# navallo/collision_avoidance

Measured on AMD Instinct MI355X. Metric: agent-steps/sec (whole node), 4096 arenas x 64 agents per GPU, higher is better.
Workload: dtype f32

## Files before the change

### collision_avoidance_amd/_lib.py

```python
import ctypes as C
import os

from . import build as _build

OBS_DIM = 64
MAX_NEIGHBORS, MAX_OBST_NEIGHBORS, MAX_AGENTS = 16, 16, 1024
DONE_XLESS, DONE_GOAL, DONE_REGOAL = 0, 1, 2
F_OBS, F_STATS, F_AUTORESET, F_NODONE, F_FREEZE = 1, 2, 4, 8, 16
SCN_CROWD, SCN_CIRCLE, SCN_DOORWAY, SCN_CONGESTED, SCN_INCOMING, SCN_BLOCKS, SCN_DEADLOCK, SCN_CROWD_SEPARATED = range(8)

(FLD_POS_X, FLD_POS_Y, FLD_VEL_X, FLD_VEL_Y, FLD_PREF_X, FLD_PREF_Y, FLD_GOAL_X, FLD_GOAL_Y,
 FLD_GOAL2_X, FLD_GOAL2_Y, FLD_REWARD, FLD_AGENT_DONE, FLD_ARRIVE_STEP, FLD_NB_COUNT, FLD_NB_IDX,
 FLD_OBST_COUNT, FLD_OBST_IDX, FLD_OBS, FLD_STEP_COUNT, FLD_ARENA_DONE, FLD_EPISODE,
 FLD_REGOAL_COUNT, FLD_ALAN_WEIGHTS, FLD_ALAN_TIMES, FLD_ALAN_ACTION, FLD_ARENA_STATS) = range(26)

EXPORTS = ("ca_create", "ca_destroy", "ca_last_error", "ca_set_stream", "ca_set_obstacles", "ca_init_scenario", "ca_set",
           "ca_get", "ca_field_ptr", "ca_bind_obs", "ca_reset", "ca_step", "ca_step_host", "ca_orca_step", "ca_observe", "ca_rollout",
           "ca_get_stats", "ca_reset_stats", "ca_sync", "ca_debug_math", "ca_profile", "ca_profile_read", "ca_launch_info",
           "ca_alan_configure", "ca_alan_step", "ca_alan_rollout", "ca_reset_masked", "ca_get_obstacles",
           "ca_set_obstacles_per_arena", "ca_get_obstacles_arena", "ca_solver_info", "ca_source_sha", "ca_host_alloc", "ca_host_free",
           "ca_step_packed", "ca_allow_obstacle_overflow", "ca_alan_configure_per_arena", "ca_alan_actions_arena")


class Config(C.Structure):
    _fields_ = [
        ("n_arenas", C.c_int32), ("n_agents", C.c_int32), ("arena_offset", C.c_int64),
        ("seed", C.c_uint64), ("reward_scale", C.c_double), ("time_step", C.c_float),
        ("neighbor_dist", C.c_float), ("max_neighbors", C.c_int32), ("time_horizon", C.c_float),
        ("time_horizon_obst", C.c_float), ("radius", C.c_float), ("max_speed", C.c_float),
        ("max_obst_neighbors", C.c_int32), ("max_step", C.c_int32), ("done_mode", C.c_int32),
        ("done_x_thresh", C.c_float), ("spawn_x0", C.c_float), ("spawn_x1", C.c_float),
        ("spawn_y0", C.c_float), ("spawn_y1", C.c_float), ("goal_x0", C.c_float),
        ("goal_x1", C.c_float), ("goal_y0", C.c_float), ("goal_y1", C.c_float),
    ]


class Stats(C.Structure):
    _fields_ = [("agent_steps", C.c_uint64), ("episodes", C.c_uint64), ("collisions", C.c_uint64),
                ("obst_collisions", C.c_uint64), ("goals_reached", C.c_uint64),
                ("obst_overflow", C.c_uint64), ("sum_reward", C.c_double)]

    def as_dict(self):
        return {k: getattr(self, k) for k, _ in self._fields_}


_lib = None


def lib_path():
    return _build.LIB_PATH


def load():
    global _lib
    if _lib is not None:
        return _lib
    path = lib_path()
    if not os.path.exists(path):
        raise RuntimeError("libcaenv.so is not built (%s); run `python -m collision_avoidance_amd.build` "
                           "-- the HIP extension is the only implementation of this path" % path)
    L = C.CDLL(path)
    vp, i32, u32, sz = C.c_void_p, C.c_int32, C.c_uint32, C.c_size_t
    L.ca_create.argtypes = [C.POINTER(Config), C.c_int, vp, C.POINTER(vp)]
    L.ca_destroy.argtypes = [vp]
    L.ca_last_error.argtypes = [vp]
    L.ca_last_error.restype = C.c_char_p
    L.ca_set_stream.argtypes = [vp, vp]
    L.ca_set_obstacles.argtypes = [vp, vp, vp, i32]
    L.ca_init_scenario.argtypes = [vp, i32]
    L.ca_get_obstacles.argtypes = [vp, vp, vp, vp, i32, C.POINTER(i32)]
    L.ca_set_obstacles_per_arena.argtypes = [vp, vp, vp, vp]
    L.ca_get_obstacles_arena.argtypes = [vp, i32, vp, vp, vp, i32, C.POINTER(i32)]
    L.ca_set.argtypes = [vp, i32, vp, sz, i32]
    L.ca_get.argtypes = [vp, i32, vp, sz, i32]
    L.ca_field_ptr.argtypes = [vp, i32, C.POINTER(vp), C.POINTER(sz)]
    L.ca_bind_obs.argtypes = [vp, vp, sz]
    L.ca_reset.argtypes = [vp, vp, vp, i32, u32]
    L.ca_reset_masked.argtypes = [vp, vp, i32, u32]
    L.ca_step.argtypes = [vp, vp, u32]
    L.ca_step_host.argtypes = [vp, vp, u32]
    L.ca_step_packed.argtypes = [vp, vp, u32, vp, sz]
    L.ca_host_alloc.argtypes = [vp, sz, C.POINTER(vp)]
    L.ca_host_free.argtypes = [vp, vp]
    L.ca_orca_step.argtypes = [vp, u32]
    L.ca_observe.argtypes = [vp]
    L.ca_rollout.argtypes = [vp, i32, u32]
    L.ca_alan_configure.argtypes = [vp, vp, i32, C.c_double, C.c_double, C.c_double]
    L.ca_alan_configure_per_arena.argtypes = [vp, vp, vp, C.c_double, C.c_double, C.c_double]
    L.ca_alan_actions_arena.argtypes = [vp, i32, vp, i32, C.POINTER(i32)]
    L.ca_alan_step.argtypes = [vp, vp, i32, u32]
    L.ca_alan_rollout.argtypes = [vp, i32, u32]
    L.ca_get_stats.argtypes = [vp, C.POINTER(Stats)]
    L.ca_reset_stats.argtypes = [vp]
    L.ca_sync.argtypes = [vp]
    L.ca_allow_obstacle_overflow.argtypes = [vp, i32]
    L.ca_debug_math.argtypes = [vp, i32, vp, vp, i32]
    L.ca_profile.argtypes = [vp, i32]
    L.ca_profile_read.argtypes = [vp, C.POINTER(i32), C.POINTER(C.c_float)]
    L.ca_launch_info.argtypes = [vp] + [C.POINTER(i32)] * 4
    L.ca_solver_info.argtypes = [vp, C.POINTER(i32), C.POINTER(i32)]
    L.ca_source_sha.argtypes = []
    L.ca_source_sha.restype = C.c_char_p
    for name in EXPORTS:
        if name not in ("ca_last_error", "ca_source_sha"):
            getattr(L, name).restype = C.c_int
    _lib = L
    return L


def check(L, handle, rc, what):
    if rc != 0:
        msg = L.ca_last_error(handle)
        raise RuntimeError("%s failed (%d): %s" % (what, rc, msg.decode() if msg else "?"))
```

### collision_avoidance_amd/csrc/ca_env.hip

```cpp
#include "../../include/ca_env.h"

#include <hip/hip_runtime.h>
#include <hip/hip_ext.h>

#include <algorithm>
#include <cmath>
#include <cstdarg>
#include <cstdlib>
#include <cstdio>
#include <cstring>
#include <string>
#include <vector>

#include "ca_kernels.h"

using namespace ca;

struct ca_env {
    ca_config cfg;
    int device = 0;
    hipStream_t stream = nullptr;
    bool own_stream = false;
    float *pos_x = nullptr, *pos_y = nullptr, *vel_x = nullptr, *vel_y = nullptr, *pref_x = nullptr,
          *pref_y = nullptr, *reward = nullptr, *orient_x = nullptr, *orient_y = nullptr;
    bool orient_valid = false;
    double *goal_x = nullptr, *goal_y = nullptr, *goal2_x = nullptr, *goal2_y = nullptr;
    int *agent_done = nullptr, *arrive_step = nullptr, *regoal_count = nullptr;
    unsigned short* counts = nullptr;
    void* nb_idx = nullptr;
    unsigned short* obst_idx = nullptr;
    int nidx16 = 0;
    int* cvt_buf = nullptr;
    size_t cvt_cap = 0;
    int *step_count = nullptr, *arena_done = nullptr, *episode = nullptr;
    unsigned long long* arena_stats = nullptr;
    unsigned long long* arena_steps = nullptr;
    float* obs = nullptr;
    bool obs_external = false;
    float* slab = nullptr;
    unsigned long long* dbg = nullptr;
    unsigned long long* dbg_obs = nullptr;
    float *tmp_x = nullptr, *tmp_y = nullptr;
    double *alan_w = nullptr, *alan_t = nullptr, *alan_dirs = nullptr, *alan_u = nullptr;
    int* alan_action = nullptr;
    AlanCold* d_alan = nullptr;
    bool alan_fused = false;
    bool alan_lane = false;
    int* mask_buf = nullptr;
    std::vector<std::pair<void*, size_t>> host_allocs;
    int n_actions = 0;
    double act_c[CA_ALAN_MAX_ACTIONS], act_s[CA_ALAN_MAX_ACTIONS];
    bool alan_per = false;
    double2* d_act_tab = nullptr;
    int* d_act_n = nullptr;
    std::vector<double> h_act_tab;
    std::vector<int> h_act_n;
    double alan_temp = 0.2, alan_window = 2.0, alan_dt = 1.0 / 60.0;
    ObstDev* d_obst = nullptr;
    std::vector<ObstDev> h_obst;
    std::vector<int> h_tab_off;
    int* d_tab_off = nullptr;
    StepCold* d_cold = nullptr;
    unsigned long long* ovf_host = nullptr;
    bool allow_overflow = false;
    int* d_order = nullptr;
    int P = 1, logP = 0, BS = 64, grid = 1, K = 0, S = 1;
    bool obs_dense_on = false;
    bool lists_trusted = true;
    int LS = 1, apb = 1, linv = 65536, dense = 0;
    struct { int reg_lines = -1, pair = -1, alan_fused = -1; } sw;
    int ST = 0, KT = 16;
    int SMX = 4;
    int max_edges = 0;
    int n_cus = 256;
    bool pair = false;
    size_t lds_p = 0;
    bool quad = false;
    bool quad_roll = false;
    int BSq = 64, grid_q = 1, SQ = 4;
    size_t lds_q = 0;
    size_t lds = 0;
    uint64_t steps_done = 0;
    float rays[32], oct[32];
    bool profiling = false;
    int prof_period = 0;
    struct Span { hipEvent_t t0, t1; int kind; int steps; };
    std::vector<Span> spans;
    std::vector<hipEvent_t> free_events;
    std::string err;
};

static thread_local std::string g_create_err;

static int fail(ca_env* e, int code, const char* fmt, ...) {
    char buf[512];
    va_list ap;
    va_start(ap, fmt);
    vsnprintf(buf, sizeof buf, fmt, ap);
    va_end(ap);
    if (e) e->err = buf;
    else g_create_err = buf;
    return code;
}
#define HIPCHK(e, call)                                                                         \
    do {                                                                                        \
        hipError_t _r = (call);                                                                 \
        if (_r != hipSuccess) return fail(e, CA_EHIP, "%s failed: %s", #call, hipGetErrorString(_r)); \
    } while (0)

static int overflow_status(ca_env* e, const char* where) {
    if (e->allow_overflow || !e->ovf_host) return CA_OK;
    const unsigned long long v = *(volatile unsigned long long*)e->ovf_host;
    if (!(v >> 63)) return CA_OK;
    return fail(e, CA_ERANGE, "%s: an obstacle-neighbour list overflowed: arena %lld, agent %d had %d%s obstacle edges in range but "
                "max_obst_neighbors=%d, so the farthest were dropped (RVO2 keeps every edge in range: collision_avoidence_env.py:249, "
                "301-318).  Raise max_obst_neighbors (at most %d), coarsen the world's polylines, or accept the truncation with "
                "ca_allow_obstacle_overflow(env, 1); ca_reset_stats clears this status", where,
                (long long)((v >> 20) & 0xFFFFFFFFFFull), (int)((v >> 8) & 0x7FF), (int)(v & 0xFF), (v & 0xFF) == 255 ? "+" : "",
                e->S, CA_MAX_OBST_NEIGHBORS);
}

enum { KIND_NBR = 0, KIND_STEP = 1, KIND_OBS = 2, KIND_RESET = 3 };
enum { CA_ROLLOUT_MAX_T = 256 };
static hipEvent_t prof_event(ca_env* e) {
    if (!e->free_events.empty()) { hipEvent_t ev = e->free_events.back(); e->free_events.pop_back(); return ev; }
    hipEvent_t ev = nullptr;
    if (hipEventCreate(&ev) != hipSuccess) return nullptr;
    return ev;
}
struct ProfScope {
    ca_env* e; hipEvent_t t0 = nullptr, t1 = nullptr; int kind; int steps;
    ProfScope(ca_env* env, int k, int n_steps = 1) : e(env), kind(k), steps(n_steps) {
        if (!e->profiling) return;
        t0 = prof_event(e);
        t1 = t0 ? prof_event(e) : nullptr;
        if (t0 && !t1) { e->free_events.push_back(t0); t0 = nullptr; }
    }
    ~ProfScope() {
        if (t0) e->spans.push_back({t0, t1, kind, steps});
    }
};
template <class... Args>
static void launch_k(const ProfScope& ps, void (*kernel)(Args...), dim3 grid, dim3 block, size_t lds, hipStream_t stream,
                     Args... args) {
    if (ps.t0) hipExtLaunchKernelGGL(kernel, grid, block, (uint32_t)lds, stream, ps.t0, ps.t1, 0, args...);
    else hipLaunchKernelGGL(kernel, grid, block, lds, stream, args...);
}

static size_t AN(const ca_env* e) { return (size_t)e->cfg.n_arenas * e->cfg.n_agents; }

struct FieldInfo {
    void* ptr;
    size_t bytes;
    bool writable;
};
static FieldInfo field_info(ca_env* e, int f) {
    const size_t an = AN(e), A = e->cfg.n_arenas;
    switch (f) {
        case CA_FLD_POS_X: return {e->pos_x, an * 4, true};
        case CA_FLD_POS_Y: return {e->pos_y, an * 4, true};
        case CA_FLD_VEL_X: return {e->vel_x, an * 4, true};
        case CA_FLD_VEL_Y: return {e->vel_y, an * 4, true};
        case CA_FLD_PREF_X: return {e->pref_x, an * 4, true};
        case CA_FLD_PREF_Y: return {e->pref_y, an * 4, true};
        case CA_FLD_GOAL_X: return {e->goal_x, an * 8, true};
        case CA_FLD_GOAL_Y: return {e->goal_y, an * 8, true};
        case CA_FLD_GOAL2_X: return {e->goal2_x, an * 8, true};
        case CA_FLD_GOAL2_Y: return {e->goal2_y, an * 8, true};
        case CA_FLD_REWARD: return {e->reward, an * 4, true};
        case CA_FLD_AGENT_DONE: return {e->agent_done, an * 4, true};
        case CA_FLD_ARRIVE_STEP: return {e->arrive_step, an * 4, true};
        case CA_FLD_NB_COUNT: return {e->counts, an * 4, true};
        case CA_FLD_NB_IDX: return {e->nb_idx, an * 4 * (size_t)(e->K > 0 ? e->K : 1), true};
        case CA_FLD_OBST_COUNT: return {e->counts, an * 4, true};
        case CA_FLD_OBST_IDX: return {e->obst_idx, an * 4 * (size_t)e->S, true};
        case CA_FLD_OBS: return {e->obs, an * CA_OBS_DIM * 4, false};
        case CA_FLD_STEP_COUNT: return {e->step_count, A * 4, true};
        case CA_FLD_ARENA_DONE: return {e->arena_done, A * 4, true};
        case CA_FLD_EPISODE: return {e->episode, A * 4, true};
        case CA_FLD_REGOAL_COUNT: return {e->regoal_count, an * 4, true};
        case CA_FLD_ALAN_WEIGHTS: return {e->alan_w, an * 8 * (size_t)e->n_actions, true};
        case CA_FLD_ALAN_TIMES: return {e->alan_t, an * 8 * (size_t)e->n_actions, true};
        case CA_FLD_ALAN_ACTION: return {e->alan_action, an * 4, true};
        case CA_FLD_ARENA_STATS: return {e->arena_stats, A * ST_STRIDE * 8, false};
        default: return {nullptr, 0, false};
    }
}

static void host_tables(ca_env* e) {
    const double nd = (double)e->cfg.neighbor_dist, r = (double)e->cfg.radius;
    for (int i = 0; i < 16; ++i) {
        const double th = i * (2.0 * M_PI / 16);
        e->rays[2 * i] = (float)(nd * std::cos(th));
        e->rays[2 * i + 1] = (float)(-nd * std::sin(th));
    }
    double first[2] = {r * std::cos(0.0), -r * std::sin(0.0)}, cur[2] = {first[0], first[1]};
    int k = 0;
    for (int i = 1; i < 8; ++i, ++k) {
        const double th = i * (2.0 * M_PI / 8);
        const double nx = r * std::cos(th), ny = -r * std::sin(th);
        e->oct[4 * k] = (float)cur[0]; e->oct[4 * k + 1] = (float)cur[1];
        e->oct[4 * k + 2] = (float)nx; e->oct[4 * k + 3] = (float)ny;
        cur[0] = nx; cur[1] = ny;
    }
    e->oct[4 * k] = (float)cur[0]; e->oct[4 * k + 1] = (float)cur[1];
    e->oct[4 * k + 2] = (float)first[0]; e->oct[4 * k + 3] = (float)first[1];
}

static void fill_cold(const ca_env* e, StepCold& c) {
    const ca_config& g = e->cfg;
    c.pos_x = e->pos_x; c.pos_y = e->pos_y; c.vel_x = e->vel_x; c.vel_y = e->vel_y;
    c.pref_x = e->pref_x; c.pref_y = e->pref_y; c.goal_x = e->goal_x; c.goal_y = e->goal_y;
    c.goal2_x = e->goal2_x; c.goal2_y = e->goal2_y; c.reward = e->reward;
    c.orient_x = e->orient_x; c.orient_y = e->orient_y;
    c.agent_done = e->agent_done; c.arrive_step = e->arrive_step; c.regoal_count = e->regoal_count;
    c.step_count = e->step_count; c.arena_done = e->arena_done; c.episode = e->episode;
    c.arena_stats = e->arena_stats; c.arena_steps = e->arena_steps; c.ovf_word = e->ovf_host;
    c.reward_scale = g.reward_scale; c.seed = g.seed; c.arena_offset = g.arena_offset;
    c.max_step = g.max_step; c.done_mode = g.done_mode; c.done_x_thresh = g.done_x_thresh;
    c.spawn_x0 = g.spawn_x0; c.spawn_x1 = g.spawn_x1; c.spawn_y0 = g.spawn_y0; c.spawn_y1 = g.spawn_y1;
    c.goal_x0 = g.goal_x0; c.goal_x1 = g.goal_x1; c.goal_y0 = g.goal_y0; c.goal_y1 = g.goal_y1;
}

static void fill_args(ca_env* e, StepArgs& a, const float* actions, uint32_t flags) {
    const ca_config& c = e->cfg;
    a.pos_x = e->pos_x; a.pos_y = e->pos_y; a.vel_x = e->vel_x; a.vel_y = e->vel_y;
    a.pref_x = e->pref_x; a.pref_y = e->pref_y; a.goal_x = e->goal_x; a.goal_y = e->goal_y;
    a.counts = e->counts; a.nb_idx = e->nb_idx; a.obst_idx = e->obst_idx;
    a.arena_done = e->arena_done; a.arena_stats = e->arena_stats; a.cold = e->d_cold;
    a.obst = e->d_obst; a.tab_off = e->d_tab_off; a.actions = actions; a.alan = nullptr; a.alan_u = nullptr;
#ifdef CA_STAMPS
    a.order = e->d_order;
#endif
    a.reset_px = nullptr; a.reset_py = nullptr; a.reset_mask = nullptr; a.dbg = e->dbg;
    a.n_obst = e->h_tab_off.empty() ? (int)e->h_obst.size() : 0; a.A = c.n_arenas; a.N = c.n_agents; a.P = e->P; a.logP = e->logP;
    a.K = e->K; a.S = e->S; a.flags = flags; a.a0 = 0; a.a1 = c.n_arenas; a.T = 1;
    a.LS = e->LS; a.apb = e->apb; a.linv = e->linv; a.dense = e->dense; a.nb_hint = e->lists_trusted ? 1 : 0;
    a.time_step = c.time_step; a.neighbor_dist = c.neighbor_dist; a.time_horizon = c.time_horizon;
    a.time_horizon_obst = c.time_horizon_obst; a.radius = c.radius; a.max_speed = c.max_speed;
}

struct SolveLaunch { const void* fn; dim3 grid, block; size_t lds; };
template <class F> static const void* fn_ptr(F* f) { return reinterpret_cast<const void*>(f); }
template <int KMAX, int ST, int SMX, bool ALAN, class... PER>
static const void* step_fn_for(int BS) {
    if constexpr (ALAN) {
        return BS == 64 ? fn_ptr(&step_kernel<KMAX, 64, ST, SMX, true, PER...>) : fn_ptr(&step_kernel<KMAX, 128, ST, SMX, true, PER...>);
    } else {
        switch (BS) {
            case 64: return fn_ptr(&step_kernel<KMAX, 64, ST, SMX>);
            case 128: return fn_ptr(&step_kernel<KMAX, 128, ST, SMX>);
            case 256: return fn_ptr(&step_kernel<KMAX, 256, ST, SMX>);
            case 512: return fn_ptr(&step_kernel<KMAX, 512, ST, SMX>);
            default: return fn_ptr(&step_kernel<KMAX, 1024, ST, SMX>);
        }
    }
}
template <int KMAX>
static const void* pair_fn_for(int BS) {
    return BS == 256 ? fn_ptr(&pair_kernel<KMAX, 256>) : fn_ptr(&pair_kernel<KMAX, 512>);
}
template <int KMAX, int SQ, bool ALAN, class... PER>
static const void* quad_fn_for(int BS) {
    switch (BS) {
        case 64: return fn_ptr(&quad_kernel<KMAX, 64, SQ, ALAN, PER...>);
        case 128: return fn_ptr(&quad_kernel<KMAX, 128, SQ, ALAN, PER...>);
        case 256: return fn_ptr(&quad_kernel<KMAX, 256, SQ, ALAN, PER...>);
        default: return fn_ptr(&quad_kernel<KMAX, 512, SQ, ALAN, PER...>);
    }
}
template <bool ALAN, class... PER>
static const void* lane_fn_for(const ca_env* e) {
    if (e->ST > 0 && e->SMX > 4) return e->KT == 5 ? step_fn_for<5, 4, 16, ALAN, PER...>(e->BS) : step_fn_for<10, 4, 16, ALAN, PER...>(e->BS);
    if (e->ST > 0) return e->KT == 5 ? step_fn_for<5, 4, 4, ALAN, PER...>(e->BS) : step_fn_for<10, 4, 4, ALAN, PER...>(e->BS);
    if (e->KT == 5) return step_fn_for<5, 0, SMAX, ALAN, PER...>(e->BS);
    if constexpr (!ALAN) { if (e->KT == 16) return step_fn_for<16, 0, SMAX, false>(e->BS); }
    return step_fn_for<10, 0, SMAX, ALAN, PER...>(e->BS);
}
template <bool ALAN, class... PER>
static const void* quad_fn_for(const ca_env* e) {
    if (e->SQ > 4) return e->KT == 5 ? quad_fn_for<5, 16, ALAN, PER...>(e->BSq) : quad_fn_for<10, 16, ALAN, PER...>(e->BSq);
    return e->KT == 5 ? quad_fn_for<5, 4, ALAN, PER...>(e->BSq) : quad_fn_for<10, 4, ALAN, PER...>(e->BSq);
}
static SolveLaunch solve_launch(const ca_env* e, bool alan, bool rollout) {
    const bool per = alan && e->alan_per;
    if (e->quad || (rollout && e->quad_roll) || (alan && !e->alan_lane)) {
        const void* f = per ? quad_fn_for<true, AlanArenaSets>(e) : (alan ? quad_fn_for<true>(e) : quad_fn_for<false>(e));
        return {f, dim3(e->grid_q), dim3(e->BSq), alan ? quad_lds_bytes(e->BSq, e->KT, e->SQ, e->n_actions) : e->lds_q};
    }
    if (e->pair)
        return {e->KT == 5 ? pair_fn_for<5>(e->BS) : pair_fn_for<10>(e->BS), dim3(e->grid), dim3(2 * e->BS), e->lds_p};
    const void* f = per ? lane_fn_for<true, AlanArenaSets>(e) : (alan ? lane_fn_for<true>(e) : lane_fn_for<false>(e));
    return {f, dim3(e->grid), dim3(e->BS), e->lds};
}
static hipError_t allow_lds(const SolveLaunch& s) {
    return s.lds > 48 * 1024 ? hipFuncSetAttribute(s.fn, hipFuncAttributeMaxDynamicSharedMemorySize, (int)s.lds) : hipSuccess;
}
static hipError_t launch_step(ca_env* e, const StepArgs& a) {
    const SolveLaunch s = solve_launch(e, a.alan != nullptr, a.T > 1);
    if (!(a.flags & CA_F_FREEZE)) e->lists_trusted = true;
    ProfScope ps(e, KIND_STEP, a.T > 1 ? a.T : 1);
    StepArgs arg = a;
    void* params[] = {&arg};
    if (ps.t0) return hipExtLaunchKernel(s.fn, s.grid, s.block, params, s.lds, e->stream, ps.t0, ps.t1, 0);
    return hipLaunchKernel(s.fn, s.grid, s.block, params, s.lds, e->stream);
}

typedef void (*obs_fn_t)(const ObsArgs);
static obs_fn_t obs_fn(int obs_bs, bool w16, bool dense = false) {
    if (dense) return obs_kernel<256, false, true>;
    switch (obs_bs) {
        case 1024: return w16 ? obs_kernel<1024, true> : obs_kernel<1024, false>;
        case 512: return w16 ? obs_kernel<512, true> : obs_kernel<512, false>;
        case 128: return w16 ? obs_kernel<128, true> : obs_kernel<128, false>;
        case 64: return w16 ? obs_kernel<64, true> : obs_kernel<64, false>;
        default: return w16 ? obs_kernel<256, true> : obs_kernel<256, false>;
    }
}

static bool obs_dense(const ca_env* e) { return e->obs_dense_on; }
static int obs_nstage(const ca_env* e) { return obs_dense(e) ? 16 + 2 * e->cfg.n_agents : e->cfg.n_agents; }

static hipError_t launch_obs(ca_env* e) {
    if (!e->orient_valid) {
        StepArgs a;
        fill_args(e, a, nullptr, 0);
        const unsigned an = (unsigned)AN(e);
        hipLaunchKernelGGL(orient_kernel, dim3((an + 255) / 256), dim3(256), 0, e->stream, a);
        hipError_t r = hipGetLastError();
        if (r != hipSuccess) return r;
        e->orient_valid = true;
    }
    ObsArgs o;
    o.pos_x = e->pos_x; o.pos_y = e->pos_y; o.vel_x = e->vel_x; o.vel_y = e->vel_y;
    o.orient_x = e->orient_x; o.orient_y = e->orient_y; o.counts = e->counts; o.nb_idx = e->nb_idx;
    o.obst_idx = e->obst_idx; o.obst = e->d_obst; o.tab_off = e->d_tab_off;
    o.obs = e->obs;
    o.A = e->cfg.n_arenas; o.N = e->cfg.n_agents; o.S = e->S;
    o.K = e->K > 0 ? e->K : 1;
    const int obs_bs = obs_block_threads(o.N), apb = obs_bs / 16;
    o.bpa = (o.N + apb - 1) / apb;
    o.paircap = 16 * (e->K + e->S);
    o.a0 = 0; o.dbg = e->dbg_obs;
    o.dense = obs_dense(e) ? 1 : 0;
    o.nstage_max = obs_nstage(e);
    o.xcd = (o.A % 8 == 0 && !o.dense) ? 1 : 0;
    o.radius = e->cfg.radius;
    memcpy(o.rays, e->rays, sizeof o.rays);
    memcpy(o.oct, e->oct, sizeof o.oct);
    const dim3 grid(o.dense ? (unsigned)(((size_t)o.A * o.N + apb - 1) / apb) : (unsigned)((size_t)o.A * o.bpa)), block(obs_bs);
    const size_t lds = obs_lds_bytes(o.nstage_max, obs_bs, o.paircap);
    ProfScope ps(e, KIND_OBS);
    launch_k(ps, obs_fn(obs_bs, e->nidx16 != 0, o.dense != 0), grid, block, lds, e->stream, o);
    return hipGetLastError();
}

static hipError_t launch_reset(ca_env* e, const StepArgs& a) {
    const unsigned an = (unsigned)AN(e);
    {
        ProfScope ps(e, KIND_RESET);
        launch_k(ps, reset_kernel, dim3((an + 255) / 256), dim3(256), 0, e->stream, a);
    }
    hipError_t r = hipGetLastError();
    if (r != hipSuccess) return r;
    {
        ProfScope ps(e, KIND_RESET);
        launch_k(ps, reset_arena_kernel, dim3((e->cfg.n_arenas + 255) / 256), dim3(256), 0, e->stream, a);
    }
    return hipGetLastError();
}

static void split_crossing_edges(std::vector<ObstDev>& tab) {
    struct Side { int left, right; };
    auto sides = [&](int split, int edge, float* a, float* b) {
        const V2 s1 = mk(tab[split].px, tab[split].py), s2 = mk(tab[tab[split].next].px, tab[tab[split].next].py);
        *a = leftOf(s1, s2, mk(tab[edge].px, tab[edge].py));
        *b = leftOf(s1, s2, mk(tab[tab[edge].next].px, tab[tab[edge].next].py));
    };
    auto worse_or_equal = [](Side x, Side y) {
        const int xm = x.left > x.right ? x.left : x.right, xn = x.left < x.right ? x.left : x.right;
        const int ym = y.left > y.right ? y.left : y.right, yn = y.left < y.right ? y.left : y.right;
        return xm > ym || (xm == ym && xn >= yn);
    };
    std::vector<std::vector<int>> work(1);
    for (int i = 0; i < (int)tab.size(); ++i) work[0].push_back(i);
    while (!work.empty()) {
        const std::vector<int> edges = std::move(work.back());
        work.pop_back();
        const int n = (int)edges.size();
        if (n == 0) continue;
        int pick = 0;
        Side best = {n, n};
        for (int i = 0; i < n; ++i) {
            Side c = {0, 0};
            for (int j = 0; j < n; ++j) {
                if (j == i) continue;
                float a, b;
                sides(edges[i], edges[j], &a, &b);
                if (a >= -EPS && b >= -EPS) ++c.left;
                else if (a <= EPS && b <= EPS) ++c.right;
                else { ++c.left; ++c.right; }
                if (worse_or_equal(c, best)) break;
            }
            if (!worse_or_equal(c, best)) { best = c; pick = i; }
        }
        std::vector<int> lhs, rhs;
        const int sp = edges[pick];
        const V2 s1 = mk(tab[sp].px, tab[sp].py), s2 = mk(tab[tab[sp].next].px, tab[tab[sp].next].py);
        for (int j = 0; j < n; ++j) {
            if (j == pick) continue;
            const int e1 = edges[j], e2 = tab[e1].next;
            float a, b;
            sides(sp, e1, &a, &b);
            if (a >= -EPS && b >= -EPS) { lhs.push_back(e1); continue; }
            if (a <= EPS && b <= EPS) { rhs.push_back(e1); continue; }
            const V2 p1 = mk(tab[e1].px, tab[e1].py), p2 = mk(tab[e2].px, tab[e2].py);
            const float t = det(s2 - s1, p1 - s1) / det(s2 - s1, p1 - p2);
            const V2 cut = p1 + t * (p2 - p1);
            ObstDev o;
            memset(&o, 0, sizeof o);
            o.px = cut.x; o.py = cut.y; o.ux = tab[e1].ux; o.uy = tab[e1].uy;
            o.prev = e1; o.next = e2; o.convex = 1;
            const int id = (int)tab.size();
            tab.push_back(o);
            tab[e1].next = id; tab[e2].prev = id;
            if (a > 0.0f) { lhs.push_back(e1); rhs.push_back(id); }
            else { rhs.push_back(e1); lhs.push_back(id); }
        }
        work.push_back(std::move(rhs));
        work.push_back(std::move(lhs));
    }
}

template <class T>
static hipError_t dalloc(ca_env* e, T** p, size_t n, bool zero = true) {
    hipError_t r = hipMalloc((void**)p, n * sizeof(T));
    if (r != hipSuccess || !zero) return r;
    return hipMemsetAsync(*p, 0, n * sizeof(T), e->stream);
}
static hipError_t upload(ca_env* e, void* dst, const void* src, size_t bytes) {
    hipError_t r = hipMemcpyAsync(dst, src, bytes, hipMemcpyHostToDevice, e->stream);
    return r != hipSuccess ? r : hipStreamSynchronize(e->stream);
}
static hipError_t download(ca_env* e, void* dst, const void* src, size_t bytes) {
    hipError_t r = hipMemcpyAsync(dst, src, bytes, hipMemcpyDeviceToHost, e->stream);
    return r != hipSuccess ? r : hipStreamSynchronize(e->stream);
}

static size_t lds_static_bytes(const ca_env* e) {
    return (size_t)e->BS * 8 +
           (e->BS >= 1024 ? (size_t)e->BS * 2 + 16 + 1024 + 1028 : (e->BS >= 256 ? (size_t)e->BS * 2 + (size_t)e->BS * 8 + 16 + 4096 + 4100 : 0)) + 64;
}

static void pick_variant(ca_env* e) {
    const bool allow = e->sw.reg_lines != 0, force = e->sw.reg_lines == 1;
    e->KT = e->K <= 5 ? 5 : (e->K <= 10 ? 10 : 16);
    const size_t table_per_wg = step_lds_bytes(e->BS, e->K, e->S, 0, e->KT) + lds_static_bytes(e);
    const bool table_fits = table_per_wg <= 160 * 1024;
    const bool small_world = e->max_edges <= 16;
    const bool table_resident = table_fits && (long)e->grid <= (long)e->n_cus * (long)((160 * 1024) / table_per_wg);
    if (allow && e->K <= 10 && e->S <= 4) { e->ST = 4; e->SMX = 4; }
    else if (allow && e->K <= 10 && (small_world || force || !table_resident)) { e->ST = 4; e->SMX = 16; }
    else { e->ST = 0; e->SMX = 16; }
    e->lds = step_lds_bytes(e->BS, e->K, e->S, e->ST, e->KT);
    e->pair = e->sw.pair != 0 && e->ST > 0 && e->SMX == 4 && (e->BS == 256 || e->BS == 512) && e->K > 0;
    e->lds_p = pair_lds_bytes(e->BS, e->KT);
}

static const size_t LDS_PER_CU = 160 * 1024;
static hipError_t apply_variant_attributes(ca_env* e, bool* misfit) {
    const SolveLaunch plain = solve_launch(e, false, false);
    *misfit = !e->pair && e->lds + lds_static_bytes(e) > LDS_PER_CU;
    hipError_t r = hipSuccess;
    if (e->pair) {
        hipFuncAttributes fa;
        r = hipFuncGetAttributes(&fa, plain.fn);
        *misfit = r == hipSuccess && fa.sharedSizeBytes + plain.lds > LDS_PER_CU;
    }
    if (r != hipSuccess || *misfit) return r;
    r = allow_lds(plain);
    if (r == hipSuccess) r = allow_lds(solve_launch(e, false, true));
    return r;
}

static int alan_pick(ca_env* e) {
    e->alan_fused = e->alan_lane = false;
    if (e->n_actions <= 0) return CA_OK;
    const size_t lq = quad_lds_bytes(e->BSq, e->KT, e->SQ, e->n_actions);
    const bool on = e->sw.alan_fused != 0;
    e->alan_fused = on && (e->quad || e->quad_roll) && lq <= 64 * 1024;
    e->alan_lane = on && !e->quad && !e->pair && e->BS <= 128 && e->K <= 10 &&
                   e->n_actions <= (e->ST > 0 ? 4 + e->KT : 2 * (e->K + e->S));
    if (e->alan_fused) HIPCHK(e, allow_lds(solve_launch(e, true, true)));
    if (e->alan_lane) HIPCHK(e, allow_lds(solve_launch(e, true, false)));
    return CA_OK;
}

extern "C" {

const char* ca_last_error(const ca_env* env) { return env ? env->err.c_str() : g_create_err.c_str(); }

int ca_create(const ca_config* cfg, int device, void* stream, ca_env** out) {
    if (!cfg || !out) return fail(nullptr, CA_EINVAL, "ca_create: null argument");
    *out = nullptr;
    if (cfg->n_arenas <= 0 || cfg->n_agents <= 0 || cfg->n_agents > CA_MAX_AGENTS)
        return fail(nullptr, CA_ERANGE, "ca_create: n_arenas=%d n_agents=%d out of range (agents 1..%d)",
                    cfg->n_arenas, cfg->n_agents, CA_MAX_AGENTS);
    if (cfg->max_neighbors < 0 || cfg->max_neighbors > CA_MAX_NEIGHBORS)
        return fail(nullptr, CA_ERANGE, "ca_create: max_neighbors=%d out of range 0..%d", cfg->max_neighbors,
                    CA_MAX_NEIGHBORS);
    if (cfg->max_obst_neighbors < 1 || cfg->max_obst_neighbors > CA_MAX_OBST_NEIGHBORS)
        return fail(nullptr, CA_ERANGE, "ca_create: max_obst_neighbors=%d out of range 1..%d",
                    cfg->max_obst_neighbors, CA_MAX_OBST_NEIGHBORS);
    if (cfg->done_mode < 0 || cfg->done_mode > 2) return fail(nullptr, CA_EINVAL, "ca_create: bad done_mode");
    {
        const struct { const char* name; float v, lo, hi; } rng[] = {
            {"time_step", cfg->time_step, CA_MIN_TIME_STEP, CA_MAX_TIME_STEP}, {"neighbor_dist", cfg->neighbor_dist, CA_MIN_LENGTH, CA_MAX_LENGTH},
            {"time_horizon", cfg->time_horizon, CA_MIN_LENGTH, CA_MAX_LENGTH}, {"time_horizon_obst", cfg->time_horizon_obst, CA_MIN_LENGTH, CA_MAX_LENGTH},
            {"radius", cfg->radius, CA_MIN_LENGTH, CA_MAX_LENGTH}, {"max_speed", cfg->max_speed, CA_MIN_LENGTH, CA_MAX_LENGTH}};
        for (const auto& q : rng)
            if (!(q.v >= q.lo && q.v <= q.hi))
                return fail(nullptr, CA_ERANGE, "ca_create: %s=%g outside the supported range [%g, %g]", q.name, (double)q.v, (double)q.lo, (double)q.hi);
        const float box[] = {cfg->spawn_x0, cfg->spawn_x1, cfg->spawn_y0, cfg->spawn_y1, cfg->goal_x0, cfg->goal_x1, cfg->goal_y0, cfg->goal_y1,
                             cfg->done_x_thresh};
        for (float v : box)
            if (!(fabsf(v) <= CA_MAX_COORD)) return fail(nullptr, CA_ERANGE, "ca_create: a spawn / goal box coordinate (%g) is beyond %g or not a number", (double)v, (double)CA_MAX_COORD);
    }
    if ((size_t)cfg->n_arenas * cfg->n_agents > (size_t)1 << 30)
        return fail(nullptr, CA_ERANGE, "ca_create: more than 2^30 agents on one handle");
    int ndev = 0;
    if (hipGetDeviceCount(&ndev) != hipSuccess || ndev <= 0)
        return fail(nullptr, CA_ENODEV, "ca_create: no HIP device (this library has no CPU path)");
    if (device < 0 || device >= ndev) return fail(nullptr, CA_ENODEV, "ca_create: device %d of %d", device, ndev);
    ca_env* e = new ca_env();
    e->cfg = *cfg;
    e->device = device;
    hipError_t r = hipSetDevice(device);
    if (r == hipSuccess) {
        if (stream) e->stream = (hipStream_t)stream;
        else { r = hipStreamCreateWithFlags(&e->stream, hipStreamNonBlocking); e->own_stream = true; }
    }
    {
        auto digit = [](const char* name) { const char* v = getenv(name); return (v && v[0] >= '0' && v[0] <= '9') ? v[0] - '0' : -1; };
        e->sw.reg_lines = digit("CA_REG_LINES"); e->sw.pair = digit("CA_PAIR"); e->sw.alan_fused = digit("CA_ALAN_FUSED");
    }
    int P = 1, logP = 0;
    while (P < cfg->n_agents) { P <<= 1; ++logP; }
    e->P = P; e->logP = logP;
    e->BS = P > 64 ? P : 64;
    e->LS = P; e->apb = e->BS / P; e->linv = 65536 / P; e->dense = 0;
    e->grid = (cfg->n_arenas + e->apb - 1) / e->apb;
    {
        const char* v = getenv("CA_OBS_DENSE");
        e->obs_dense_on = cfg->n_agents < 16 && !(v && v[0] == '0');
    }
    {
        const char* v = getenv("CA_DENSE");
        const int N = cfg->n_agents;
        if (!(v && v[0] == '0') && e->BS == 64 && P < 64 && 64 / N > 64 / P) {
            const int linv = (65536 + N - 1) / N;
            bool exact = true;
            for (int t = 0; t < 64; ++t) exact = exact && ((t * linv) >> 16) == t / N;
            if (exact) {
                e->LS = N; e->apb = 64 / N; e->linv = linv; e->dense = 1;
                e->grid = (cfg->n_arenas + e->apb - 1) / e->apb;
            }
        }
    }
    e->K = cfg->max_neighbors;
    e->S = cfg->max_obst_neighbors;
    {
        int cus = 0;
        if (hipDeviceGetAttribute(&cus, hipDeviceAttributeMultiprocessorCount, device) == hipSuccess && cus > 0) e->n_cus = cus;
    }
    pick_variant(e);
    {
        const char* v = getenv("CA_QUAD");
        e->SQ = e->S <= 4 ? 4 : 16;
        const bool fits = e->K <= 10 && 4 * P <= ((e->SQ == 16 && e->KT == 10) ? 256 : 512);
        const long lane_waves = (long)((cfg->n_arenas + e->BS / P - 1) / (e->BS / P)) * (e->BS / 64);
        e->quad = fits && (v ? v[0] == '1' : lane_waves < 1024);
        e->quad_roll = fits && (v ? v[0] == '1' : lane_waves <= 1024);
        e->BSq = 4 * P > 64 ? 4 * P : 64;
        const int apbq = (e->BSq / 4) / P;
        e->grid_q = (cfg->n_arenas + apbq - 1) / apbq;
        e->lds_q = quad_lds_bytes(e->BSq, e->KT, e->SQ);
    }
    if (!e->pair && e->lds + lds_static_bytes(e) > LDS_PER_CU) {
        fail(nullptr, CA_ERANGE, "ca_create: the solve kernel would need %zu B of LDS (> 160 KiB) for n_agents=%d, "
             "max_neighbors=%d, max_obst_neighbors=%d: arenas above 256 agents need max_neighbors <= 10 "
             "(register-line variant)", e->lds + lds_static_bytes(e), cfg->n_agents, e->K, e->S);
        if (e->own_stream && e->stream) hipStreamDestroy(e->stream);
        delete e;
        return CA_ERANGE;
    }
    host_tables(e);
    const size_t an = AN(e), A = cfg->n_arenas;
    float** f32s[] = {&e->pos_x, &e->pos_y, &e->vel_x, &e->vel_y, &e->pref_x, &e->pref_y,
                      &e->tmp_x, &e->tmp_y, &e->orient_x, &e->orient_y};
    for (auto p : f32s) if (r == hipSuccess) r = dalloc(e, p, an);
    double** f64s[] = {&e->goal_x, &e->goal_y, &e->goal2_x, &e->goal2_y};
    for (auto p : f64s) if (r == hipSuccess) r = dalloc(e, p, an);
    int** i32s[] = {&e->agent_done, &e->arrive_step, &e->regoal_count};
    for (auto p : i32s) if (r == hipSuccess) r = dalloc(e, p, an);
    e->nidx16 = CA_NBW16(e->BS) ? 1 : 0;
    if (r == hipSuccess) r = dalloc(e, &e->counts, an);
    if (r == hipSuccess) r = dalloc(e, reinterpret_cast<unsigned char**>(&e->nb_idx),
                                    an * (size_t)(e->K > 0 ? e->K : 1) * (e->nidx16 ? 2 : 1));
    if (r == hipSuccess) r = dalloc(e, &e->obst_idx, an * (size_t)e->S);
    if (r == hipSuccess) r = dalloc(e, &e->slab, an * CA_OBS_DIM + an + 2 * A);
    if (r == hipSuccess) {
        e->obs = e->slab; e->reward = e->slab + an * CA_OBS_DIM;
        e->arena_done = reinterpret_cast<int*>(e->reward + an); e->step_count = e->arena_done + A;
    }
    if (r == hipSuccess) r = dalloc(e, &e->episode, A);
    if (r == hipSuccess) r = dalloc(e, &e->arena_stats, A * ST_STRIDE);
    if (r == hipSuccess) r = dalloc(e, &e->arena_steps, A);
    if (r == hipSuccess) r = dalloc(e, &e->d_obst, (size_t)1);
#ifdef CA_STAMPS
    if (r == hipSuccess) r = dalloc(e, &e->dbg, (size_t)std::max(e->grid * (2 * e->BS / 64), e->grid_q * (e->BSq / 64)) * 16);
    if (r == hipSuccess) r = dalloc(e, &e->dbg_obs, (size_t)cfg->n_arenas * ((cfg->n_agents + 15) / 16 + 16) * 4 * 16);
#endif
    bool lds_misfit = false;
    if (r == hipSuccess) r = apply_variant_attributes(e, &lds_misfit);
    if (r == hipSuccess) {
        const int obs_bs = obs_block_threads(cfg->n_agents);
        const size_t ol = obs_lds_bytes(obs_nstage(e), obs_bs, 16 * (e->K + e->S));
        if (ol > 48 * 1024) {
            r = hipFuncSetAttribute(reinterpret_cast<const void*>(obs_fn(obs_bs, e->nidx16 != 0, obs_dense(e))),
                                    hipFuncAttributeMaxDynamicSharedMemorySize, (int)ol);
        }
    }
    if (r == hipSuccess) {
        r = hipHostMalloc((void**)&e->ovf_host, sizeof(unsigned long long), hipHostMallocDefault);
        if (r == hipSuccess) *e->ovf_host = 0ull;
    }
    if (r == hipSuccess) r = hipMalloc((void**)&e->d_cold, sizeof(StepCold));
    if (r == hipSuccess) {
        StepCold hc;
        fill_cold(e, hc);
        r = upload(e, e->d_cold, &hc, sizeof hc);
    }
    if (r == hipSuccess) r = hipStreamSynchronize(e->stream);
    if (r == hipSuccess && lds_misfit) {
        fail(nullptr, CA_ERANGE, "ca_create: the solve kernel for n_agents=%d, max_neighbors=%d, max_obst_neighbors=%d does not fit the "
             "160 KiB of LDS of a CU", cfg->n_agents, e->K, e->S);
        ca_destroy(e);
        return CA_ERANGE;
    }
    if (r != hipSuccess) {
        fail(nullptr, CA_EHIP, "ca_create: %s", hipGetErrorString(r));
        ca_destroy(e);
        return CA_EHIP;
    }
    *out = e;
    return CA_OK;
}

int ca_destroy(ca_env* e) {
    if (!e) return CA_OK;
    hipSetDevice(e->device);
    if (e->stream) hipStreamSynchronize(e->stream);
    void* bufs[] = {e->pos_x, e->pos_y, e->vel_x, e->vel_y, e->pref_x, e->pref_y, e->goal_x, e->goal_y,
                    e->goal2_x, e->goal2_y, e->slab, e->tmp_x, e->tmp_y, e->orient_x, e->orient_y,
                    e->agent_done, e->arrive_step,
                    e->regoal_count, e->counts, e->nb_idx, e->obst_idx, e->cvt_buf, e->d_tab_off, e->d_cold, e->d_order,
                    e->episode, e->arena_stats, e->arena_steps, e->d_obst, e->dbg, e->dbg_obs,
                    e->alan_w, e->alan_t, e->alan_dirs, e->alan_u, e->alan_action, e->d_alan, e->mask_buf,
                    e->d_act_tab, e->d_act_n};
    for (void* b : bufs) if (b) hipFree(b);
    for (const auto& h : e->host_allocs) hipHostFree(h.first);
    if (e->ovf_host) hipHostFree(e->ovf_host);
    for (const ca_env::Span& sp : e->spans) { hipEventDestroy(sp.t0); hipEventDestroy(sp.t1); }
    for (hipEvent_t ev : e->free_events) hipEventDestroy(ev);
    if (e->own_stream && e->stream) hipStreamDestroy(e->stream);
    delete e;
    return CA_OK;
}

int ca_set_stream(ca_env* e, void* stream) {
    if (!e) return CA_EINVAL;
    HIPCHK(e, hipSetDevice(e->device));
    HIPCHK(e, hipStreamSynchronize(e->stream));
    if (e->own_stream && e->stream) HIPCHK(e, hipStreamDestroy(e->stream));
    e->stream = (hipStream_t)stream;
    e->own_stream = false;
    return CA_OK;
}

static int build_table(ca_env* e, const float* verts_xy, const int32_t* poly_sizes, int n_poly, std::vector<ObstDev>& tab) {
    size_t off = 0;
    for (int pi = 0; pi < n_poly; ++pi) {
        const int n = poly_sizes[pi];
        if (n < 2) return fail(e, CA_EINVAL, "ca_set_obstacles: polygon %d has %d vertices (need >= 2)", pi, n);
        const int base = (int)tab.size();
        for (int i = 0; i < n; ++i) {
            const int in = (i == n - 1) ? 0 : i + 1, ip = (i == 0) ? n - 1 : i - 1;
            const V2 pt = mk(verts_xy[2 * (off + i)], verts_xy[2 * (off + i) + 1]);
            const V2 pn = mk(verts_xy[2 * (off + in)], verts_xy[2 * (off + in) + 1]);
            const V2 pp = mk(verts_xy[2 * (off + ip)], verts_xy[2 * (off + ip) + 1]);
            if (!(fabsf(pt.x) <= CA_MAX_COORD && fabsf(pt.y) <= CA_MAX_COORD))
                return fail(e, CA_ERANGE, "ca_set_obstacles: polygon %d vertex %d = (%g, %g) is beyond %g or not a number", pi, i,
                            (double)pt.x, (double)pt.y, (double)CA_MAX_COORD);
            if (pn.x == pt.x && pn.y == pt.y)
                return fail(e, CA_EINVAL, "ca_set_obstacles: polygon %d has an edge of length zero (vertex %d twice)", pi, i);
            if (absSq(pn - pt) < CA_MIN_EDGE * CA_MIN_EDGE)
                return fail(e, CA_ERANGE, "ca_set_obstacles: polygon %d edge %d is shorter than %g", pi, i, (double)CA_MIN_EDGE);
            const V2 u = normalize(pn - pt);
            ObstDev o;
            memset(&o, 0, sizeof o);
            o.px = pt.x; o.py = pt.y; o.ux = u.x; o.uy = u.y;
            o.next = base + in; o.prev = base + ip;
            o.convex = (n == 2) ? 1 : (leftOf(pp, pt, pn) >= 0.0f ? 1 : 0);
            tab.push_back(o);
        }
        off += n;
    }
    split_crossing_edges(tab);
    for (ObstDev& o : tab) {
        const ObstDev& nx = tab[o.next];
        const ObstDev& pv = tab[o.prev];
        o.qx = nx.px; o.qy = nx.py; o.qux = nx.ux; o.quy = nx.uy; o.qconvex = nx.convex;
        o.pux = pv.ux; o.puy = pv.uy;
    }
    return CA_OK;
}

__global__ void clear_obst_counts_kernel(unsigned short* counts, size_t n) {
    const size_t q = (size_t)blockIdx.x * blockDim.x + threadIdx.x;
    if (q < n) counts[q] &= 0x00FFu;
}

static int install_tables(ca_env* e, std::vector<ObstDev>& all, std::vector<int>& offs) {
    HIPCHK(e, hipSetDevice(e->device));
    HIPCHK(e, hipStreamSynchronize(e->stream));
    ObstDev* n_obst = nullptr;
    int* n_off = nullptr;
    hipError_t r = hipMalloc((void**)&n_obst, (all.size() + 1) * sizeof(ObstDev));
    if (r == hipSuccess && !all.empty()) r = upload(e, n_obst, all.data(), all.size() * sizeof(ObstDev));
    if (r == hipSuccess && !offs.empty()) {
        r = hipMalloc((void**)&n_off, offs.size() * sizeof(int));
        if (r == hipSuccess) r = upload(e, n_off, offs.data(), offs.size() * sizeof(int));
    }
    if (r == hipSuccess) {
        const size_t an = AN(e);
        hipLaunchKernelGGL(clear_obst_counts_kernel, dim3((unsigned)((an + 255) / 256)), dim3(256), 0, e->stream, e->counts, an);
        r = hipGetLastError();
        if (r == hipSuccess) r = hipStreamSynchronize(e->stream);
    }
    if (r != hipSuccess) {
        if (n_obst) hipFree(n_obst);
        if (n_off) hipFree(n_off);
        return fail(e, CA_EHIP, "ca_set_obstacles: %s (the previous tables stay installed)", hipGetErrorString(r));
    }
    int me = 0;
    if (offs.empty()) me = (int)all.size();
    else for (size_t a = 0; a + 1 < offs.size(); ++a) me = std::max(me, offs[a + 1] - offs[a]);
    struct { int ST, SMX, KT, max_edges; bool pair; size_t lds, lds_p; } old_v = {e->ST, e->SMX, e->KT, e->max_edges, e->pair, e->lds, e->lds_p};
    e->max_edges = me;
    pick_variant(e);
    bool misfit = false;
    const hipError_t ra = apply_variant_attributes(e, &misfit);
    if (misfit || ra != hipSuccess) {
        e->ST = old_v.ST; e->SMX = old_v.SMX; e->KT = old_v.KT; e->max_edges = old_v.max_edges; e->pair = old_v.pair;
        e->lds = old_v.lds; e->lds_p = old_v.lds_p;
        bool dummy = false;
        (void)apply_variant_attributes(e, &dummy);
        hipFree(n_obst);
        if (n_off) hipFree(n_off);
        if (misfit)
            return fail(e, CA_ERANGE, "ca_set_obstacles: the solve kernel this world selects does not fit the 160 KiB of LDS of a CU "
                        "(n_agents=%d, max_neighbors=%d, max_obst_neighbors=%d); the previous tables stay installed", e->cfg.n_agents, e->K, e->S);
        return fail(e, CA_EHIP, "ca_set_obstacles: %s (the previous tables stay installed)", hipGetErrorString(ra));
    }
    if (e->d_obst) hipFree(e->d_obst);
    if (e->d_tab_off) hipFree(e->d_tab_off);
    e->d_obst = n_obst;
    e->d_tab_off = n_off;
    e->h_obst.swap(all);
    e->h_tab_off.swap(offs);
    return alan_pick(e);
}

int ca_set_obstacles(ca_env* e, const float* verts_xy, const int32_t* poly_sizes, int32_t n_poly) {
    if (!e || n_poly < 0 || (n_poly > 0 && (!verts_xy || !poly_sizes))) return fail(e, CA_EINVAL, "ca_set_obstacles: bad argument");
    std::vector<ObstDev> tab;
    const int rc = build_table(e, verts_xy, poly_sizes, n_poly, tab);
    if (rc) return rc;
    if (tab.size() > 65536) return fail(e, CA_ERANGE, "ca_set_obstacles: %zu edges (at most 65536)", tab.size());
    std::vector<int> none;
    return install_tables(e, tab, none);
}

int ca_set_obstacles_per_arena(ca_env* e, const float* verts_xy, const int32_t* poly_sizes, const int32_t* n_poly) {
    if (!e || !n_poly) return fail(e, CA_EINVAL, "ca_set_obstacles_per_arena: null argument");
    const int A = e->cfg.n_arenas;
    std::vector<ObstDev> all;
    std::vector<int> offs(1, 0);
    size_t voff = 0, poff = 0;
    for (int a = 0; a < A; ++a) {
        if (n_poly[a] < 0 || (n_poly[a] > 0 && (!verts_xy || !poly_sizes)))
            return fail(e, CA_EINVAL, "ca_set_obstacles_per_arena: bad argument for arena %d", a);
        std::vector<ObstDev> tab;
        const int rc = build_table(e, verts_xy ? verts_xy + 2 * voff : nullptr, poly_sizes ? poly_sizes + poff : nullptr,
                                   n_poly[a], tab);
        if (rc) return rc;
        for (int k = 0; k < n_poly[a]; ++k) voff += (size_t)poly_sizes[poff + k];
        poff += (size_t)n_poly[a];
        if (tab.size() > 65536) return fail(e, CA_ERANGE, "ca_set_obstacles_per_arena: arena %d has %zu edges (at most 65536)", a, tab.size());
        all.insert(all.end(), tab.begin(), tab.end());
        if (all.size() > (size_t)0x7FFFFFFF) return fail(e, CA_ERANGE, "ca_set_obstacles_per_arena: too many edges");
        offs.push_back((int)all.size());
    }
    return install_tables(e, all, offs);
}

static int get_table(ca_env* e, int arena, float* verts_xy, int32_t* next, int32_t* convex, int32_t cap, int32_t* n_out) {
    const bool per = !e->h_tab_off.empty();
    const int t0 = per ? e->h_tab_off[arena] : 0;
    const int n = per ? e->h_tab_off[arena + 1] - t0 : (int)e->h_obst.size();
    *n_out = n;
    for (int i = 0; i < n && i < cap; ++i) {
        const ObstDev& o = e->h_obst[t0 + i];
        if (verts_xy) { verts_xy[2 * i] = o.px; verts_xy[2 * i + 1] = o.py; }
        if (next) next[i] = o.next;
        if (convex) convex[i] = o.convex;
    }
    return CA_OK;
}

int ca_get_obstacles(ca_env* e, float* verts_xy, int32_t* next, int32_t* convex, int32_t cap, int32_t* n_out) {
    if (!e || !n_out) return fail(e, CA_EINVAL, "ca_get_obstacles: null argument");
    return get_table(e, 0, verts_xy, next, convex, cap, n_out);
}

int ca_get_obstacles_arena(ca_env* e, int32_t arena, float* verts_xy, int32_t* next, int32_t* convex, int32_t cap,
                           int32_t* n_out) {
    if (!e || !n_out) return fail(e, CA_EINVAL, "ca_get_obstacles_arena: null argument");
    if (arena < 0 || arena >= e->cfg.n_arenas) return fail(e, CA_ERANGE, "ca_get_obstacles_arena: arena %d of %d", arena, e->cfg.n_arenas);
    return get_table(e, arena, verts_xy, next, convex, cap, n_out);
}

}

static void host_scenario(const ca_env* e, int scenario, int An, std::vector<float>& px, std::vector<float>& py, std::vector<float>& vx,
                          std::vector<float>& vy, std::vector<float>& fx, std::vector<float>& fy, std::vector<double>& gx,
                          std::vector<double>& gy, std::vector<double>& g2x, std::vector<double>& g2y) {
    const ca_config& c = e->cfg;
    const int A = An, N = c.n_agents;
    const size_t an = (size_t)An * N;
    px.assign(an, 0.0f); py.assign(an, 0.0f); vx.assign(an, 0.0f); vy.assign(an, 0.0f); fx.assign(an, 0.0f); fy.assign(an, 0.0f);
    gx.assign(an, 0.0); gy.assign(an, 0.0); g2x.assign(an, 0.0); g2y.assign(an, 0.0);
    const double r = (double)c.radius;
    for (int a = 0; a < A; ++a) {
        const int64_t g = c.arena_offset + a;
        double theta = 0.0;
        for (int i = 0; i < N; ++i) {
            const size_t q = (size_t)a * N + i;
            double u0, u1, s, cs;
            rng2(c.seed, g, i, RNG_HEADING, 0, &u0, &u1);
            sincos64(uniform64(0.0, 2.0 * M_PI, u0), &s, &cs);
            vx[q] = (float)cs; vy[q] = (float)s;
            if (scenario == CA_SCN_CROWD || scenario == CA_SCN_CROWD_SEPARATED) {
                const double E = std::sqrt(2.0 * r * N) * 2.0;
                const int tries = scenario == CA_SCN_CROWD_SEPARATED ? 64 : 1;
                const float minSq = sqr(c.radius + c.radius);
                for (int t = 0; t < tries; ++t) {
                    rng2(c.seed, g, i, RNG_POS, (uint32_t)t, &u0, &u1);
                    px[q] = (float)uniform64(0.0, E, u0); py[q] = (float)uniform64(0.0, E, u1);
                    bool clear = true;
                    for (int j = 0; j < i && clear; ++j)
                        clear = !(absSq(mk(px[q], py[q]) - mk(px[q - i + j], py[q - i + j])) < minSq);
                    if (clear) break;
                }
                rng2(c.seed, g, i, RNG_GOAL, 0, &u0, &u1);
                gx[q] = uniform64(0.0, E, u0); gy[q] = uniform64(0.0, E, u1);
                g2x[q] = gx[q]; g2y[q] = gy[q];
            } else if (scenario == CA_SCN_CIRCLE) {
                const double R = (r * 3 * N) / (2.0 * M_PI);
                const double E = 2.0 * R + 4.0 * r;
                px[q] = (float)(E / 2 + R * std::cos(theta)); py[q] = (float)(E / 2 + R * std::sin(theta));
                gx[q] = E / 2 + R * std::cos(theta + M_PI);
                gy[q] = E / 2 + R * std::sin(theta + M_PI);
                g2x[q] = gx[q]; g2y[q] = gy[q];
                theta += (2.0 * M_PI) / N;
            } else if (scenario >= CA_SCN_CONGESTED) {
                const double E = (scenario == CA_SCN_CONGESTED) ? std::sqrt(2 * r * N) * 3
                               : (scenario == CA_SCN_BLOCKS) ? 3 * r * N : std::sqrt(2 * r * N) * 10;
                double x = 0, y = 0, tx = 0, ty = 0, t2x = 0, t2y = 0;
                if (scenario == CA_SCN_CONGESTED) {
                    rng2(c.seed, g, i, RNG_POS, 0, &u0, &u1);
                    x = uniform64(E * 0.2, E, u0); y = uniform64(0.0, E, u1);
                    tx = 0.1 * E - 1.0; ty = E / 2; t2x = 0.1 * E - E; t2y = E / 2;
                } else if (scenario == CA_SCN_INCOMING) {
                    if (i == 0) {
                        x = 0.1 * E; y = E / 2; tx = t2x = 0.9 * E; ty = t2y = E / 2;
                    } else {
                        const double len = std::sqrt((double)(N - 1)), x_inc = 3 * r, y_inc = 2.1 * r;
                        const double y_start = E / 2 - ((y_inc * len) / 2);
                        double x_pos = 0.8 * E, y_pos = y_start;
                        for (int k = 1; k < i; ++k) {
                            y_pos += y_inc;
                            if (y_pos > y_start + y_inc * len) { x_pos += x_inc; y_pos = y_start; }
                        }
                        x = x_pos; y = y_pos; tx = t2x = x_pos - 0.7 * E; ty = t2y = y_pos;
                    }
                } else if (scenario == CA_SCN_BLOCKS) {
                    double y_pos = 1.5 * r;
                    for (int k = 0; k < i; ++k) y_pos += 3 * r;
                    x = 1.5 * r; y = y_pos; tx = t2x = E - 1.5 * r; ty = t2y = y_pos;
                } else {
                    const int half = N / 2;
                    if (i < half) {
                        double pos_x = 0.2 * E;
                        for (int k = 0; k < i; ++k) pos_x += -3 * r;
                        x = pos_x; tx = 0.9 * E; t2x = 0.9 * E + E;
                    } else {
                        double pos_x = 0.8 * E;
                        for (int k = half; k < i; ++k) pos_x += 3 * r;
                        x = pos_x; tx = 0.1 * E; t2x = 0.1 * E - E;
                    }
                    y = E / 2; ty = t2y = E / 2;
                }
                px[q] = (float)x; py[q] = (float)y; gx[q] = tx; gy[q] = ty;
                g2x[q] = t2x; g2y[q] = t2y;
            } else {
                const double E = 10.0;
                rng2(c.seed, g, i, RNG_POS, 0, &u0, &u1);
                px[q] = (float)uniform64(E * 0.5, E, u0); py[q] = (float)uniform64(0.0, E, u1);
                gx[q] = 1.0; gy[q] = 5.0; g2x[q] = -10.0; g2y[q] = 5.0;
            }
            double dx, dy;
            pref_dir64(px[q], py[q], gx[q], gy[q], &dx, &dy);
            fx[q] = (float)dx; fy[q] = (float)dy;
        }
    }
}

struct InitArgs {
    float *pos_x, *pos_y, *vel_x, *vel_y, *pref_x, *pref_y;
    double *goal_x, *goal_y, *goal2_x, *goal2_y;
    const float *tpx, *tpy;
    const double *tgx, *tgy, *tg2x, *tg2y;
    double x0, x1, y0, y1;
    double ge;
    uint64_t seed;
    int64_t arena_offset;
    int A, N, pos_rng, goal_rng;
};
__global__ void init_scenario_kernel(const InitArgs p) {
    const size_t q = (size_t)blockIdx.x * blockDim.x + threadIdx.x;
    if (q >= (size_t)p.A * p.N) return;
    const int a = (int)(q / p.N), i = (int)(q - (size_t)a * p.N);
    const int64_t g = p.arena_offset + a;
    double u0, u1, s, cs;
    rng2(p.seed, g, i, RNG_HEADING, 0, &u0, &u1);
    sincos64(uniform64(0.0, 2.0 * M_PI, u0), &s, &cs);
    p.vel_x[q] = (float)cs; p.vel_y[q] = (float)s;
    float px = p.tpx[i], py = p.tpy[i];
    double gx = p.tgx[i], gy = p.tgy[i], g2x = p.tg2x[i], g2y = p.tg2y[i];
    if (p.pos_rng) {
        rng2(p.seed, g, i, RNG_POS, 0, &u0, &u1);
        px = (float)uniform64(p.x0, p.x1, u0); py = (float)uniform64(p.y0, p.y1, u1);
    }
    if (p.goal_rng) {
        rng2(p.seed, g, i, RNG_GOAL, 0, &u0, &u1);
        gx = uniform64(0.0, p.ge, u0); gy = uniform64(0.0, p.ge, u1);
        g2x = gx; g2y = gy;
    }
    double dx, dy;
    pref_dir64(px, py, gx, gy, &dx, &dy);
    p.pos_x[q] = px; p.pos_y[q] = py; p.pref_x[q] = (float)dx; p.pref_y[q] = (float)dy;
    p.goal_x[q] = gx; p.goal_y[q] = gy; p.goal2_x[q] = g2x; p.goal2_y[q] = g2y;
}

extern "C" {

int ca_init_scenario(ca_env* e, int32_t scenario) {
    if (!e) return CA_EINVAL;
    if (scenario < 0 || scenario > CA_SCN_CROWD_SEPARATED)
        return fail(e, CA_EINVAL, "ca_init_scenario: unknown scenario %d", scenario);
    const ca_config& c = e->cfg;
    const int A = c.n_arenas, N = c.n_agents;
    const size_t an = AN(e);
    const bool on_host = scenario == CA_SCN_CROWD_SEPARATED;
    std::vector<float> px, py, vx, vy, fx, fy;
    std::vector<double> gx, gy, g2x, g2y;
    host_scenario(e, scenario, on_host ? A : 1, px, py, vx, vy, fx, fy, gx, gy, g2x, g2y);
    HIPCHK(e, hipSetDevice(e->device));
    hipStream_t st = e->stream;
    if (on_host) {
        struct { float* d; std::vector<float>* h; } up[] = {{e->pos_x, &px}, {e->pos_y, &py}, {e->vel_x, &vx},
            {e->vel_y, &vy}, {e->pref_x, &fx}, {e->pref_y, &fy}};
        struct { double* d; std::vector<double>* h; } upd[] = {{e->goal_x, &gx}, {e->goal_y, &gy},
            {e->goal2_x, &g2x}, {e->goal2_y, &g2y}};
        for (auto& u : up) HIPCHK(e, hipMemcpyAsync(u.d, u.h->data(), an * 4, hipMemcpyHostToDevice, st));
        for (auto& u : upd) HIPCHK(e, hipMemcpyAsync(u.d, u.h->data(), an * 8, hipMemcpyHostToDevice, st));
    } else {
        char* tab = nullptr;
        const size_t nb = (size_t)N * (2 * 4 + 4 * 8);
        HIPCHK(e, hipMalloc((void**)&tab, nb));
        std::vector<char> h(nb);
        memcpy(h.data(), px.data(), (size_t)N * 4); memcpy(h.data() + (size_t)N * 4, py.data(), (size_t)N * 4);
        memcpy(h.data() + (size_t)N * 8, gx.data(), (size_t)N * 8); memcpy(h.data() + (size_t)N * 16, gy.data(), (size_t)N * 8);
        memcpy(h.data() + (size_t)N * 24, g2x.data(), (size_t)N * 8); memcpy(h.data() + (size_t)N * 32, g2y.data(), (size_t)N * 8);
        hipError_t r = hipMemcpyAsync(tab, h.data(), nb, hipMemcpyHostToDevice, st);
        if (r == hipSuccess) {
            InitArgs ia;
            ia.pos_x = e->pos_x; ia.pos_y = e->pos_y; ia.vel_x = e->vel_x; ia.vel_y = e->vel_y; ia.pref_x = e->pref_x; ia.pref_y = e->pref_y;
            ia.goal_x = e->goal_x; ia.goal_y = e->goal_y; ia.goal2_x = e->goal2_x; ia.goal2_y = e->goal2_y;
            ia.tpx = (const float*)tab; ia.tpy = (const float*)(tab + (size_t)N * 4);
            ia.tgx = (const double*)(tab + (size_t)N * 8); ia.tgy = (const double*)(tab + (size_t)N * 16);
            ia.tg2x = (const double*)(tab + (size_t)N * 24); ia.tg2y = (const double*)(tab + (size_t)N * 32);
            const double r2 = (double)c.radius;
            ia.pos_rng = (scenario == CA_SCN_CROWD || scenario == CA_SCN_CONGESTED || scenario == CA_SCN_DOORWAY) ? 1 : 0;
            ia.goal_rng = scenario == CA_SCN_CROWD ? 1 : 0;
            ia.x0 = 0.0; ia.x1 = 0.0; ia.y0 = 0.0; ia.y1 = 0.0; ia.ge = 0.0;
            if (scenario == CA_SCN_CROWD) { const double E = std::sqrt(2.0 * r2 * N) * 2.0; ia.x1 = E; ia.y1 = E; ia.ge = E; }
            else if (scenario == CA_SCN_CONGESTED) { const double E = std::sqrt(2 * r2 * N) * 3; ia.x0 = E * 0.2; ia.x1 = E; ia.y1 = E; }
            else if (scenario == CA_SCN_DOORWAY) { const double E = 10.0; ia.x0 = E * 0.5; ia.x1 = E; ia.y1 = E; }
            ia.seed = c.seed; ia.arena_offset = c.arena_offset; ia.A = A; ia.N = N;
            hipLaunchKernelGGL(init_scenario_kernel, dim3((unsigned)((an + 255) / 256)), dim3(256), 0, st, ia);
            r = hipGetLastError();
        }
        if (r == hipSuccess) r = hipStreamSynchronize(st);
        hipFree(tab);
        if (r != hipSuccess) return fail(e, CA_EHIP, "ca_init_scenario: %s", hipGetErrorString(r));
    }
    HIPCHK(e, hipMemsetAsync(e->agent_done, 0, an * 4, st));
    HIPCHK(e, hipMemsetAsync(e->arrive_step, 0xff, an * 4, st));
    HIPCHK(e, hipMemsetAsync(e->regoal_count, 0, an * 4, st));
    HIPCHK(e, hipMemsetAsync(e->counts, 0, an * 2, st));
    HIPCHK(e, hipMemsetAsync(e->step_count, 0, (size_t)A * 4, st));
    HIPCHK(e, hipMemsetAsync(e->arena_done, 0, (size_t)A * 4, st));
    HIPCHK(e, hipMemsetAsync(e->episode, 0, (size_t)A * 4, st));
    HIPCHK(e, hipMemsetAsync(e->obs, 0, an * CA_OBS_DIM * 4, st));
    HIPCHK(e, hipStreamSynchronize(st));
    e->orient_valid = false;
    return CA_OK;
}

__global__ void unpack_list_kernel(const void* src, int kind, int w16, int* dst, size_t n) {
    const size_t q = (size_t)blockIdx.x * blockDim.x + threadIdx.x;
    if (q >= n) return;
    if (kind == 0) dst[q] = (int)(reinterpret_cast<const unsigned short*>(src)[q] & 0xFFu);
    else if (kind == 1) dst[q] = (int)(reinterpret_cast<const unsigned short*>(src)[q] >> 8);
    else dst[q] = w16 ? ld_idx_t<true>(src, q) : ld_idx_t<false>(src, q);
}
__global__ void pack_list_kernel(const int* src, int kind, int w16, void* dst, size_t n) {
    const size_t q = (size_t)blockIdx.x * blockDim.x + threadIdx.x;
    if (q >= n) return;
    unsigned short* c = reinterpret_cast<unsigned short*>(dst);
    if (kind == 0) c[q] = (unsigned short)((c[q] & 0xFF00u) | ((unsigned)src[q] & 0xFFu));
    else if (kind == 1) c[q] = (unsigned short)((c[q] & 0x00FFu) | (((unsigned)src[q] & 0xFFu) << 8));
    else if (w16) st_idx_t<true>(dst, q, src[q]);
    else st_idx_t<false>(dst, q, src[q]);
}
static bool packed_field(int f) {
    return f == CA_FLD_NB_COUNT || f == CA_FLD_OBST_COUNT || f == CA_FLD_NB_IDX || f == CA_FLD_OBST_IDX;
}
static int packed_kind(int f) { return f == CA_FLD_NB_COUNT ? 0 : (f == CA_FLD_OBST_COUNT ? 1 : 2); }
static int cvt_reserve(ca_env* e, size_t elems) {
    if (e->cvt_cap >= elems) return CA_OK;
    HIPCHK(e, hipStreamSynchronize(e->stream));
    if (e->cvt_buf) HIPCHK(e, hipFree(e->cvt_buf));
    e->cvt_buf = nullptr; e->cvt_cap = 0;
    HIPCHK(e, hipMalloc((void**)&e->cvt_buf, elems * sizeof(int)));
    e->cvt_cap = elems;
    return CA_OK;
}

int ca_set(ca_env* e, int32_t field, const void* src, size_t bytes, int32_t src_is_device) {
    if (!e || !src) return fail(e, CA_EINVAL, "ca_set: null argument");
    const FieldInfo fi = field_info(e, field);
    if (!fi.ptr) return fail(e, CA_EINVAL, "ca_set: unknown field %d", field);
    if (!fi.writable) return fail(e, CA_EINVAL, "ca_set: field %d is read-only", field);
    if (bytes != fi.bytes) return fail(e, CA_ESIZE, "ca_set: field %d holds %zu bytes, got %zu", field, fi.bytes, bytes);
    HIPCHK(e, hipSetDevice(e->device));
    if (packed_field(field)) {
        e->lists_trusted = false;
        const size_t n = bytes / 4;
        const int rc = cvt_reserve(e, n);
        if (rc) return rc;
        HIPCHK(e, hipMemcpyAsync(e->cvt_buf, src, bytes, src_is_device ? hipMemcpyDeviceToDevice : hipMemcpyHostToDevice, e->stream));
        hipLaunchKernelGGL(pack_list_kernel, dim3((unsigned)((n + 255) / 256)), dim3(256), 0, e->stream, e->cvt_buf,
                           packed_kind(field), field == CA_FLD_NB_IDX ? e->nidx16 : 1, fi.ptr, n);
        HIPCHK(e, hipGetLastError());
        HIPCHK(e, hipStreamSynchronize(e->stream));
        return CA_OK;
    }
    HIPCHK(e, hipMemcpyAsync(fi.ptr, src, bytes, src_is_device ? hipMemcpyDeviceToDevice : hipMemcpyHostToDevice, e->stream));
    if (!src_is_device) HIPCHK(e, hipStreamSynchronize(e->stream));
    if (field == CA_FLD_POS_X || field == CA_FLD_POS_Y || field == CA_FLD_GOAL_X || field == CA_FLD_GOAL_Y)
        e->orient_valid = false;
    return CA_OK;
}

int ca_get(ca_env* e, int32_t field, void* dst, size_t bytes, int32_t dst_is_device) {
    if (!e || !dst) return fail(e, CA_EINVAL, "ca_get: null argument");
    const FieldInfo fi = field_info(e, field);
    if (!fi.ptr) return fail(e, CA_EINVAL, "ca_get: unknown field %d", field);
    if (bytes != fi.bytes) return fail(e, CA_ESIZE, "ca_get: field %d holds %zu bytes, got %zu", field, fi.bytes, bytes);
    HIPCHK(e, hipSetDevice(e->device));
    if (packed_field(field)) {
        const size_t n = bytes / 4;
        const int rc = cvt_reserve(e, n);
        if (rc) return rc;
        hipLaunchKernelGGL(unpack_list_kernel, dim3((unsigned)((n + 255) / 256)), dim3(256), 0, e->stream, fi.ptr,
                           packed_kind(field), field == CA_FLD_NB_IDX ? e->nidx16 : 1, e->cvt_buf, n);
        HIPCHK(e, hipGetLastError());
        HIPCHK(e, hipMemcpyAsync(dst, e->cvt_buf, bytes, dst_is_device ? hipMemcpyDeviceToDevice : hipMemcpyDeviceToHost, e->stream));
        HIPCHK(e, hipStreamSynchronize(e->stream));
        return CA_OK;
    }
    HIPCHK(e, hipMemcpyAsync(dst, fi.ptr, bytes, dst_is_device ? hipMemcpyDeviceToDevice : hipMemcpyDeviceToHost, e->stream));
    if (!dst_is_device) HIPCHK(e, hipStreamSynchronize(e->stream));
    return CA_OK;
}

int ca_field_ptr(ca_env* e, int32_t field, void** dev_ptr, size_t* bytes) {
    if (!e || !dev_ptr) return fail(e, CA_EINVAL, "ca_field_ptr: null argument");
    const FieldInfo fi = field_info(e, field);
    if (!fi.ptr) return fail(e, CA_EINVAL, "ca_field_ptr: unknown field %d", field);
    if (packed_field(field))
        return fail(e, CA_EINVAL, "ca_field_ptr: field %d is stored packed (u8/u16); read it through ca_get", field);
    *dev_ptr = fi.ptr;
    if (bytes) *bytes = fi.bytes;
    return CA_OK;
}

int ca_bind_obs(ca_env* e, void* dev_ptr, size_t bytes) {
    if (!e || !dev_ptr) return fail(e, CA_EINVAL, "ca_bind_obs: null argument");
    if (bytes != AN(e) * CA_OBS_DIM * 4)
        return fail(e, CA_ESIZE, "ca_bind_obs: need %zu bytes, got %zu", AN(e) * CA_OBS_DIM * 4, bytes);
    if (((uintptr_t)dev_ptr & 15) != 0) return fail(e, CA_EINVAL, "ca_bind_obs: buffer must be 16-byte aligned");
    HIPCHK(e, hipSetDevice(e->device));
    HIPCHK(e, hipStreamSynchronize(e->stream));
    e->obs = (float*)dev_ptr;
    e->obs_external = true;
    return CA_OK;
}

int ca_reset(ca_env* e, const float* pos_x, const float* pos_y, int32_t pos_is_device, uint32_t flags) {
    if (!e) return CA_EINVAL;
    if ((pos_x == nullptr) != (pos_y == nullptr)) return fail(e, CA_EINVAL, "ca_reset: pos_x and pos_y go together");
    HIPCHK(e, hipSetDevice(e->device));
    StepArgs a;
    fill_args(e, a, nullptr, flags);
    if (pos_x) {
        if (pos_is_device) { a.reset_px = pos_x; a.reset_py = pos_y; }
        else {
            HIPCHK(e, hipMemcpyAsync(e->tmp_x, pos_x, AN(e) * 4, hipMemcpyHostToDevice, e->stream));
            HIPCHK(e, hipMemcpyAsync(e->tmp_y, pos_y, AN(e) * 4, hipMemcpyHostToDevice, e->stream));
            HIPCHK(e, hipStreamSynchronize(e->stream));
            a.reset_px = e->tmp_x; a.reset_py = e->tmp_y;
        }
    }
    HIPCHK(e, launch_reset(e, a));
    HIPCHK(e, hipGetLastError());
    e->orient_valid = true;
    if (flags & CA_F_OBS) HIPCHK(e, launch_obs(e));
    return CA_OK;
}

int ca_reset_masked(ca_env* e, const int32_t* mask, int32_t mask_is_device, uint32_t flags) {
    if (!e || !mask) return fail(e, CA_EINVAL, "ca_reset_masked: null argument");
    HIPCHK(e, hipSetDevice(e->device));
    const int A = e->cfg.n_arenas;
    if (!mask_is_device) {
        if (!e->mask_buf) HIPCHK(e, dalloc(e, &e->mask_buf, (size_t)A, false));
        HIPCHK(e, upload(e, e->mask_buf, mask, (size_t)A * 4));
        mask = e->mask_buf;
    }
    StepArgs a;
    fill_args(e, a, nullptr, flags);
    a.reset_mask = mask;
    HIPCHK(e, launch_reset(e, a));
    HIPCHK(e, hipGetLastError());
    if (flags & CA_F_OBS) HIPCHK(e, launch_obs(e));
    return CA_OK;
}

static int do_step(ca_env* e, const float* actions, uint32_t flags) {
    { const int rs = overflow_status(e, "step"); if (rs) return rs; }
    if (e->prof_period > 1) e->profiling = (e->steps_done % (uint64_t)e->prof_period) == 0;
    StepArgs a;
    fill_args(e, a, actions, flags);
    HIPCHK(e, launch_step(e, a));
    e->orient_valid = true;
    if (flags & CA_F_OBS) HIPCHK(e, launch_obs(e));
    e->steps_done += 1;
    return CA_OK;
}

int ca_step(ca_env* e, const float* actions, uint32_t flags) {
    if (!e) return CA_EINVAL;
    if (!actions) return fail(e, CA_EINVAL, "ca_step: actions is null (use ca_orca_step for the ORCA-only step)");
    if (flags & CA_F_NODONE) return fail(e, CA_EINVAL, "ca_step: CA_F_NODONE applies to ca_orca_step only");
    HIPCHK(e, hipSetDevice(e->device));
    return do_step(e, actions, flags);
}

int ca_step_host(ca_env* e, const float* actions_host, uint32_t flags) {
    if (!e) return CA_EINVAL;
    if (!actions_host) return fail(e, CA_EINVAL, "ca_step_host: actions is null");
    if (flags & CA_F_NODONE) return fail(e, CA_EINVAL, "ca_step_host: CA_F_NODONE applies to ca_orca_step only");
    HIPCHK(e, hipSetDevice(e->device));
    HIPCHK(e, hipMemcpyAsync(e->tmp_x, actions_host, AN(e) * 4, hipMemcpyHostToDevice, e->stream));
    HIPCHK(e, hipStreamSynchronize(e->stream));
    return do_step(e, e->tmp_x, flags);
}

int ca_step_packed(ca_env* e, const float* actions_host, uint32_t flags, void* out_host, size_t out_bytes) {
    if (!e || !out_host) return fail(e, CA_EINVAL, "ca_step_packed: null argument");
    const size_t an = AN(e), A = (size_t)e->cfg.n_arenas;
    const size_t obs_b = an * CA_OBS_DIM * 4, rest_b = an * 4 + 2 * A * 4;
    if (out_bytes != obs_b + rest_b) return fail(e, CA_ESIZE, "ca_step_packed: need %zu bytes, got %zu", obs_b + rest_b, out_bytes);
    if (actions_host && (flags & CA_F_NODONE)) return fail(e, CA_EINVAL, "ca_step_packed: CA_F_NODONE applies to the ORCA-only step");
    HIPCHK(e, hipSetDevice(e->device));
    const float* act = nullptr;
    if (actions_host) {
        bool mapped = false;
        for (const auto& h : e->host_allocs)
            if ((const char*)actions_host >= (const char*)h.first && (const char*)actions_host + an * 4 <= (const char*)h.first + h.second) { mapped = true; break; }
        if (mapped) act = actions_host;
        else {
            HIPCHK(e, hipMemcpyAsync(e->tmp_x, actions_host, an * 4, hipMemcpyHostToDevice, e->stream));
            act = e->tmp_x;
        }
    }
    const int rc = do_step(e, act, flags);
    if (rc) return rc;
    char* out = (char*)out_host;
    if (!e->obs_external) {
        HIPCHK(e, hipMemcpyAsync(out, e->slab, obs_b + rest_b, hipMemcpyDeviceToHost, e->stream));
    } else {
        HIPCHK(e, hipMemcpyAsync(out, e->obs, obs_b, hipMemcpyDeviceToHost, e->stream));
        HIPCHK(e, hipMemcpyAsync(out + obs_b, e->reward, rest_b, hipMemcpyDeviceToHost, e->stream));
    }
    HIPCHK(e, hipStreamSynchronize(e->stream));
    return overflow_status(e, "ca_step_packed");
}

int ca_orca_step(ca_env* e, uint32_t flags) {
    if (!e) return CA_EINVAL;
    HIPCHK(e, hipSetDevice(e->device));
    return do_step(e, nullptr, flags);
}

static void alan_unit(double x, double y, double* c, double* s) {
    const double len = std::sqrt(x * x + y * y);
    *c = len == 0.0 ? 1.0 : x / len;
    *s = len == 0.0 ? 0.0 : y / len;
}

static int alan_install(ca_env* e, int nA, double temp, double timewindow, double time_step) {
    for (double** b : {&e->alan_w, &e->alan_t, &e->alan_dirs, &e->alan_u}) { if (*b) hipFree(*b); *b = nullptr; }
    if (e->alan_action) { hipFree(e->alan_action); e->alan_action = nullptr; }
    const size_t an = AN(e);
    HIPCHK(e, dalloc(e, &e->alan_w, an * (size_t)nA));
    HIPCHK(e, dalloc(e, &e->alan_t, an * (size_t)nA));
    HIPCHK(e, dalloc(e, &e->alan_dirs, an * 4));
    HIPCHK(e, dalloc(e, &e->alan_u, an));
    HIPCHK(e, dalloc(e, &e->alan_action, an));
    if (e->alan_per) {
        const size_t A = (size_t)e->cfg.n_arenas;
        if (!e->d_act_tab) HIPCHK(e, hipMalloc((void**)&e->d_act_tab, A * CA_ALAN_MAX_ACTIONS * sizeof(double2)));
        if (!e->d_act_n) HIPCHK(e, hipMalloc((void**)&e->d_act_n, A * sizeof(int)));
        HIPCHK(e, hipMemcpyAsync(e->d_act_tab, e->h_act_tab.data(), A * CA_ALAN_MAX_ACTIONS * sizeof(double2),
                                 hipMemcpyHostToDevice, e->stream));
        HIPCHK(e, hipMemcpyAsync(e->d_act_n, e->h_act_n.data(), A * sizeof(int), hipMemcpyHostToDevice, e->stream));
    }
    HIPCHK(e, hipStreamSynchronize(e->stream));
    e->n_actions = nA;
    e->alan_temp = temp; e->alan_window = timewindow; e->alan_dt = time_step;
    {
        if (!e->d_alan) HIPCHK(e, hipMalloc((void**)&e->d_alan, sizeof(AlanCold)));
        AlanCold h;
        memset(&h, 0, sizeof h);
        h.w = e->alan_w; h.t = e->alan_t; h.action = e->alan_action; h.reward = e->reward;
        memcpy(h.act_c, e->act_c, sizeof h.act_c); memcpy(h.act_s, e->act_s, sizeof h.act_s);
        h.temp = temp; h.window = timewindow; h.dt = time_step; h.reward_scale = e->cfg.reward_scale; h.nA = nA;
        h.tab = e->alan_per ? e->d_act_tab : nullptr;
        h.tab_n = e->alan_per ? e->d_act_n : nullptr;
        HIPCHK(e, upload(e, e->d_alan, &h, sizeof h));
    }
    return alan_pick(e);
}

int ca_alan_configure(ca_env* e, const double* actions_xy, int32_t n_actions, double temp, double timewindow,
                      double time_step) {
    if (!e || !actions_xy) return fail(e, CA_EINVAL, "ca_alan_configure: null argument");
    if (n_actions < 1 || n_actions > CA_ALAN_MAX_ACTIONS)
        return fail(e, CA_ERANGE, "ca_alan_configure: n_actions=%d out of range 1..%d", n_actions, CA_ALAN_MAX_ACTIONS);
    if (!(temp > 0.0) || !(timewindow > 0.0) || !(time_step > 0.0))
        return fail(e, CA_EINVAL, "ca_alan_configure: temp, timewindow and time_step must be positive");
    HIPCHK(e, hipSetDevice(e->device));
    HIPCHK(e, hipStreamSynchronize(e->stream));
    e->n_actions = 0;
    for (int k = 0; k < n_actions; ++k) alan_unit(actions_xy[2 * k], actions_xy[2 * k + 1], &e->act_c[k], &e->act_s[k]);
    e->alan_per = false;
    return alan_install(e, n_actions, temp, timewindow, time_step);
}

int ca_alan_configure_per_arena(ca_env* e, const double* actions_xy, const int32_t* n_actions, double temp, double timewindow,
                                double time_step) {
    if (!e || !actions_xy || !n_actions) return fail(e, CA_EINVAL, "ca_alan_configure_per_arena: null argument");
    const int A = e->cfg.n_arenas;
    int nmax = 0;
    for (int a = 0; a < A; ++a) {
        if (n_actions[a] < 1 || n_actions[a] > CA_ALAN_MAX_ACTIONS)
            return fail(e, CA_ERANGE, "ca_alan_configure_per_arena: n_actions[%d]=%d out of range 1..%d", a, n_actions[a],
                        CA_ALAN_MAX_ACTIONS);
        nmax = n_actions[a] > nmax ? n_actions[a] : nmax;
    }
    if (!(temp > 0.0) || !(timewindow > 0.0) || !(time_step > 0.0))
        return fail(e, CA_EINVAL, "ca_alan_configure_per_arena: temp, timewindow and time_step must be positive");
    HIPCHK(e, hipSetDevice(e->device));
    HIPCHK(e, hipStreamSynchronize(e->stream));
    e->n_actions = 0;
    e->h_act_tab.assign((size_t)A * CA_ALAN_MAX_ACTIONS * 2, 0.0);
    e->h_act_n.assign(n_actions, n_actions + A);
    size_t off = 0;
    for (int a = 0; a < A; ++a)
        for (int k = 0; k < n_actions[a]; ++k, ++off) {
            double* cs = &e->h_act_tab[((size_t)a * CA_ALAN_MAX_ACTIONS + k) * 2];
            alan_unit(actions_xy[2 * off], actions_xy[2 * off + 1], cs, cs + 1);
        }
    e->alan_per = true;
    return alan_install(e, nmax, temp, timewindow, time_step);
}

int ca_alan_actions_arena(ca_env* e, int32_t arena, double* cs_xy, int32_t cap, int32_t* n_out) {
    if (!e || !n_out) return fail(e, CA_EINVAL, "ca_alan_actions_arena: null argument");
    if (arena < 0 || arena >= e->cfg.n_arenas)
        return fail(e, CA_ERANGE, "ca_alan_actions_arena: arena %d of %d", arena, e->cfg.n_arenas);
    if (e->n_actions <= 0) return fail(e, CA_EINVAL, "ca_alan_actions_arena: call ca_alan_configure first");
    const int n = e->alan_per ? e->h_act_n[arena] : e->n_actions;
    *n_out = n;
    if (!cs_xy) return CA_OK;
    for (int k = 0; k < n && k < cap; ++k) {
        if (e->alan_per) {
            cs_xy[2 * k] = e->h_act_tab[((size_t)arena * CA_ALAN_MAX_ACTIONS + k) * 2];
            cs_xy[2 * k + 1] = e->h_act_tab[((size_t)arena * CA_ALAN_MAX_ACTIONS + k) * 2 + 1];
        } else {
            cs_xy[2 * k] = e->act_c[k]; cs_xy[2 * k + 1] = e->act_s[k];
        }
    }
    return CA_OK;
}

int ca_alan_step(ca_env* e, const double* u, int32_t u_is_device, uint32_t flags) {
    if (!e) return CA_EINVAL;
    if (e->n_actions <= 0) return fail(e, CA_EINVAL, "ca_alan_step: call ca_alan_configure first");
    if (flags & (CA_F_AUTORESET | CA_F_NODONE))
        return fail(e, CA_EINVAL, "ca_alan_step: CA_F_AUTORESET / CA_F_NODONE do not apply (ALAN:106-123)");
    HIPCHK(e, hipSetDevice(e->device));
    { const int rs = overflow_status(e, "ca_alan_step"); if (rs) return rs; }
    if (u && !u_is_device) {
        HIPCHK(e, hipMemcpyAsync(e->alan_u, u, AN(e) * 8, hipMemcpyHostToDevice, e->stream));
        HIPCHK(e, hipStreamSynchronize(e->stream));
        u = e->alan_u;
    }
    if (e->prof_period > 1) e->profiling = (e->steps_done % (uint64_t)e->prof_period) == 0;
    if ((e->alan_fused && e->quad) || e->alan_lane) {
        StepArgs a;
        fill_args(e, a, nullptr, flags);
        a.alan = e->d_alan; a.alan_u = u;
        HIPCHK(e, launch_step(e, a));
        e->orient_valid = true;
        if (flags & CA_F_OBS) HIPCHK(e, launch_obs(e));
        e->steps_done += 1;
        return CA_OK;
    }
    const ca_config& c = e->cfg;
    AlanArgs p;
    p.pos_x = e->pos_x; p.pos_y = e->pos_y; p.vel_x = e->vel_x; p.vel_y = e->vel_y;
    p.goal_x = e->goal_x; p.goal_y = e->goal_y; p.pref_x = e->pref_x; p.pref_y = e->pref_y; p.reward = e->reward;
    p.w = e->alan_w; p.t = e->alan_t; p.action = e->alan_action; p.dirs = e->alan_dirs; p.u = u;
    p.step_count = e->step_count; p.arena_done = e->arena_done; p.episode = e->episode; p.arena_stats = e->arena_stats;
    memcpy(p.act_c, e->act_c, sizeof p.act_c);
    memcpy(p.act_s, e->act_s, sizeof p.act_s);
    p.tab = e->alan_per ? e->d_act_tab : nullptr; p.tab_n = e->alan_per ? e->d_act_n : nullptr;
    p.temp = e->alan_temp; p.window = e->alan_window; p.dt = e->alan_dt; p.reward_scale = c.reward_scale;
    p.seed = c.seed; p.arena_offset = c.arena_offset; p.A = c.n_arenas; p.N = c.n_agents; p.nA = e->n_actions;
    p.flags = flags;
    const dim3 grid((unsigned)((AN(e) + ALAN_BS - 1) / ALAN_BS)), block(ALAN_BS);
    {
        ProfScope ps(e, KIND_RESET);
        if (e->alan_per) launch_k(ps, alan_select_kernel<2>, grid, block, (size_t)e->n_actions * ALAN_BS * 8, e->stream, p);
        else launch_k(ps, alan_select_kernel<1>, grid, block, (size_t)e->n_actions * ALAN_BS * 8, e->stream, p);
    }
    HIPCHK(e, hipGetLastError());
    StepArgs a;
    fill_args(e, a, nullptr, flags);
    HIPCHK(e, launch_step(e, a));
    {
        ProfScope ps(e, KIND_RESET);
        if (e->alan_per) launch_k(ps, alan_update_kernel<2>, grid, block, 0, e->stream, p);
        else launch_k(ps, alan_update_kernel<1>, grid, block, 0, e->stream, p);
    }
    HIPCHK(e, hipGetLastError());
    e->orient_valid = true;
    if (flags & CA_F_OBS) HIPCHK(e, launch_obs(e));
    e->steps_done += 1;
    return CA_OK;
}

int ca_alan_rollout(ca_env* e, int32_t steps, uint32_t flags) {
    if (!e || steps < 0) return fail(e, CA_EINVAL, "ca_alan_rollout: bad argument");
    { const int rs = overflow_status(e, "ca_alan_rollout"); if (rs) return rs; }
    if (e->n_actions > 0 && e->alan_fused && e->quad_roll && !(flags & (CA_F_OBS | CA_F_AUTORESET | CA_F_NODONE)) && steps > 1) {
        HIPCHK(e, hipSetDevice(e->device));
        StepArgs a;
        fill_args(e, a, nullptr, flags);
        a.alan = e->d_alan;
        for (int done = 0; done < steps; done += CA_ROLLOUT_MAX_T) {
            if (e->prof_period > 1) e->profiling = (e->steps_done / (uint64_t)CA_ROLLOUT_MAX_T) % (uint64_t)e->prof_period == 0;
            a.T = steps - done < CA_ROLLOUT_MAX_T ? steps - done : CA_ROLLOUT_MAX_T;
            if (a.T == 1 && !e->quad) {
                const int rc = ca_alan_step(e, nullptr, 0, flags);
                if (rc) return rc;
                continue;
            }
            HIPCHK(e, launch_step(e, a));
            e->steps_done += (uint64_t)a.T;
        }
        e->orient_valid = true;
        return CA_OK;
    }
    for (int s = 0; s < steps; ++s) {
        const int rc = ca_alan_step(e, nullptr, 0, flags);
        if (rc) return rc;
    }
    return CA_OK;
}

int ca_observe(ca_env* e) {
    if (!e) return CA_EINVAL;
    HIPCHK(e, hipSetDevice(e->device));
    HIPCHK(e, launch_obs(e));
    return CA_OK;
}

int ca_rollout(ca_env* e, int32_t steps, uint32_t flags) {
    if (!e || steps < 0) return fail(e, CA_EINVAL, "ca_rollout: bad argument");
    HIPCHK(e, hipSetDevice(e->device));
    { const int rs = overflow_status(e, "ca_rollout"); if (rs) return rs; }
    if (e->quad_roll && !(flags & CA_F_OBS) && steps > 1) {
        StepArgs a;
        fill_args(e, a, nullptr, flags);
        for (int done = 0; done < steps; done += CA_ROLLOUT_MAX_T) {
            if (e->prof_period > 1) e->profiling = (e->steps_done / (uint64_t)CA_ROLLOUT_MAX_T) % (uint64_t)e->prof_period == 0;
            a.T = steps - done < CA_ROLLOUT_MAX_T ? steps - done : CA_ROLLOUT_MAX_T;
            HIPCHK(e, launch_step(e, a));
            e->steps_done += (uint64_t)a.T;
        }
        e->orient_valid = true;
        return CA_OK;
    }
    for (int s = 0; s < steps; ++s) {
        const int rc = do_step(e, nullptr, flags);
        if (rc) return rc;
    }
    return CA_OK;
}

int ca_sync(ca_env* e) {
    if (!e) return CA_EINVAL;
    HIPCHK(e, hipSetDevice(e->device));
    HIPCHK(e, hipStreamSynchronize(e->stream));
    return overflow_status(e, "ca_sync");
}

int ca_allow_obstacle_overflow(ca_env* e, int32_t allow) {
    if (!e) return CA_EINVAL;
    e->allow_overflow = allow != 0;
    return CA_OK;
}

int ca_get_stats(ca_env* e, ca_stats* out) {
    if (!e || !out) return fail(e, CA_EINVAL, "ca_get_stats: null argument");
    HIPCHK(e, hipSetDevice(e->device));
    const size_t A = e->cfg.n_arenas;
    std::vector<unsigned long long> h(A * ST_STRIDE);
    HIPCHK(e, hipMemcpyAsync(h.data(), e->arena_stats, h.size() * 8, hipMemcpyDeviceToHost, e->stream));
    HIPCHK(e, hipStreamSynchronize(e->stream));
    ca_stats s;
    memset(&s, 0, sizeof s);
    for (size_t a = 0; a < A; ++a) {
        const unsigned long long* r = &h[a * ST_STRIDE];
        s.episodes += r[ST_EPISODES]; s.collisions += r[ST_COLL]; s.obst_collisions += r[ST_OBST_COLL];
        s.goals_reached += r[ST_GOALS]; s.obst_overflow += r[ST_OVERFLOW];
        double d;
        memcpy(&d, &r[ST_SUMREW], 8);
        s.sum_reward += d;
    }
    std::vector<unsigned long long> hs(A);
    HIPCHK(e, hipMemcpyAsync(hs.data(), e->arena_steps, A * 8, hipMemcpyDeviceToHost, e->stream));
    HIPCHK(e, hipStreamSynchronize(e->stream));
    unsigned long long arena_steps = 0;
    for (size_t a = 0; a < A; ++a) arena_steps += hs[a];
    s.agent_steps = arena_steps * (uint64_t)e->cfg.n_agents;
    *out = s;
    return CA_OK;
}

int ca_reset_stats(ca_env* e) {
    if (!e) return CA_EINVAL;
    HIPCHK(e, hipSetDevice(e->device));
    HIPCHK(e, hipMemsetAsync(e->arena_stats, 0, (size_t)e->cfg.n_arenas * ST_STRIDE * 8, e->stream));
    HIPCHK(e, hipMemsetAsync(e->arena_steps, 0, (size_t)e->cfg.n_arenas * 8, e->stream));
    e->steps_done = 0;
    if (e->ovf_host && (*(volatile unsigned long long*)e->ovf_host >> 63)) {
        HIPCHK(e, hipStreamSynchronize(e->stream));
        *(volatile unsigned long long*)e->ovf_host = 0ull;
    }
    return CA_OK;
}

int ca_debug_math(ca_env* e, int32_t op, const void* in, void* out, int32_t n) {
    if (!e || !in || !out || n <= 0 || op < 0 || op > 7) return fail(e, CA_EINVAL, "ca_debug_math: bad argument");
    static const size_t in_b[] = {4, 8, 8, 16, 16, 8, 8, 4}, out_b[] = {4, 4, 16, 16, 16, 8, 4, 4};
    HIPCHK(e, hipSetDevice(e->device));
    void *di = nullptr, *dout = nullptr;
    HIPCHK(e, hipMalloc(&di, in_b[op] * n));
    HIPCHK(e, hipMalloc(&dout, out_b[op] * n));
    HIPCHK(e, upload(e, di, in, in_b[op] * n));
    hipLaunchKernelGGL(debug_math_kernel, dim3((n + 255) / 256), dim3(256), 0, e->stream, op, di, dout, n, e->cfg.seed);
    HIPCHK(e, hipGetLastError());
    HIPCHK(e, download(e, out, dout, out_b[op] * n));
    hipFree(di);
    hipFree(dout);
    return CA_OK;
}

#ifdef CA_STAMPS
int ca_debug_set_order(ca_env* e, const int32_t* order) {
    if (!e) return CA_EINVAL;
    HIPCHK(e, hipSetDevice(e->device));
    HIPCHK(e, hipStreamSynchronize(e->stream));
    if (e->d_order) { HIPCHK(e, hipFree(e->d_order)); e->d_order = nullptr; }
    if (!order) return CA_OK;
    std::vector<char> seen((size_t)e->grid, 0);
    for (int b = 0; b < e->grid; ++b) {
        if (order[b] < 0 || order[b] >= e->grid || seen[order[b]]) return fail(e, CA_EINVAL, "ca_debug_set_order: not a permutation");
        seen[order[b]] = 1;
    }
    HIPCHK(e, hipMalloc((void**)&e->d_order, (size_t)e->grid * sizeof(int)));
    HIPCHK(e, upload(e, e->d_order, order, (size_t)e->grid * sizeof(int)));
    return CA_OK;
}

__global__ void debug_clock_kernel(unsigned long long* out) {
    const unsigned long long t0 = __builtin_amdgcn_s_memrealtime();
    __builtin_amdgcn_s_waitcnt(0xC07F);
    if (threadIdx.x == 0) out[0] = t0;
    __builtin_amdgcn_sched_barrier(0);
    const unsigned long long t1 = __builtin_amdgcn_s_memrealtime();
    __builtin_amdgcn_s_waitcnt(0xC07F);
    if (threadIdx.x == 0) out[1] = t1;
}
__global__ void debug_empty_kernel(unsigned long long* dbg, int waves_per_block) {
    extern __shared__ float4 smem4[];
    const unsigned long long t0 = __builtin_amdgcn_s_memrealtime();
    __builtin_amdgcn_s_waitcnt(0xC07F);
    if (threadIdx.x == 4096) smem4[0] = make_float4(0.f, 0.f, 0.f, 0.f);
    __builtin_amdgcn_sched_barrier(0);
    const unsigned long long t1 = __builtin_amdgcn_s_memrealtime();
    __builtin_amdgcn_s_waitcnt(0xC07F);
    if ((threadIdx.x & 63) == 0) {
        unsigned long long* r = dbg + ((size_t)blockIdx.x * waves_per_block + (threadIdx.x >> 6)) * 16;
        r[12] = t0; r[11] = t1;
    }
}
static unsigned long long* g_dbg_clock = nullptr;
int ca_debug_clock(ca_env* e, int32_t slot) {
    if (!e || slot < 0 || slot >= 64) return fail(e, CA_EINVAL, "ca_debug_clock: bad argument");
    HIPCHK(e, hipSetDevice(e->device));
    if (!g_dbg_clock) HIPCHK(e, hipMalloc((void**)&g_dbg_clock, 64 * 2 * 8));
    hipLaunchKernelGGL(debug_clock_kernel, dim3(1), dim3(64), 0, e->stream, g_dbg_clock + 2 * slot);
    return CA_OK;
}
int ca_debug_clock_read(ca_env* e, unsigned long long* out, int32_t n_slots) {
    if (!e || !g_dbg_clock || n_slots > 64) return fail(e, CA_EINVAL, "ca_debug_clock_read: bad argument");
    HIPCHK(e, download(e, out, g_dbg_clock, (size_t)n_slots * 2 * 8));
    return CA_OK;
}
int ca_debug_empty(ca_env* e) {
    if (!e || !e->dbg) return fail(e, CA_EINVAL, "ca_debug_empty: not a CA_STAMPS build");
    HIPCHK(e, hipSetDevice(e->device));
    ProfScope ps(e, KIND_RESET);
    launch_k(ps, debug_empty_kernel, dim3(e->grid), dim3(e->BS), (size_t)e->lds, e->stream, e->dbg, e->BS / 64);
    return CA_OK;
}

int ca_debug_stamps(ca_env* e, unsigned long long* out, int32_t max_waves, int32_t* n_waves) {
    if (!e || !e->dbg) return fail(e, CA_EINVAL, "ca_debug_stamps: not a CA_STAMPS build");
    const bool obs = max_waves < 0;
    if (obs) max_waves = -max_waves;
    const int nw = obs ? e->cfg.n_arenas * ((e->cfg.n_agents + 15) / 16) * 4 : (e->quad ? e->grid_q * (e->BSq / 64) : e->grid * ((e->pair ? 2 : 1) * e->BS / 64));
    if (n_waves) *n_waves = nw;
    const int n = nw < max_waves ? nw : max_waves;
    HIPCHK(e, hipSetDevice(e->device));
    HIPCHK(e, download(e, out, obs ? e->dbg_obs : e->dbg, (size_t)n * 16 * 8));
    return CA_OK;
}
#endif

int ca_host_alloc(ca_env* e, size_t bytes, void** out) {
    if (!e || !out || bytes == 0) return fail(e, CA_EINVAL, "ca_host_alloc: bad argument");
    *out = nullptr;
    HIPCHK(e, hipSetDevice(e->device));
    void* p = nullptr;
    HIPCHK(e, hipHostMalloc(&p, bytes, hipHostMallocDefault));
    e->host_allocs.push_back({p, bytes});
    *out = p;
    return CA_OK;
}
int ca_host_free(ca_env* e, void* p) {
    if (!e || !p) return fail(e, CA_EINVAL, "ca_host_free: bad argument");
    for (size_t k = 0; k < e->host_allocs.size(); ++k)
        if (e->host_allocs[k].first == p) {
            e->host_allocs.erase(e->host_allocs.begin() + k);
            HIPCHK(e, hipHostFree(p));
            return CA_OK;
        }
    return fail(e, CA_EINVAL, "ca_host_free: not a buffer of this handle");
}

int ca_profile(ca_env* e, int32_t period) {
    if (!e || period < 0) return fail(e, CA_EINVAL, "ca_profile: bad argument");
    e->prof_period = period;
    e->profiling = period == 1;
    if (period > 0) {
        HIPCHK(e, hipSetDevice(e->device));
        while (e->free_events.size() < 256) {
            hipEvent_t ev = nullptr;
            if (hipEventCreate(&ev) != hipSuccess) break;
            e->free_events.push_back(ev);
        }
    }
    return CA_OK;
}

int ca_profile_read(ca_env* e, int32_t counts[4], float mean_ms[4]) {
    if (!e || !counts || !mean_ms) return fail(e, CA_EINVAL, "ca_profile_read: null argument");
    HIPCHK(e, hipSetDevice(e->device));
    HIPCHK(e, hipStreamSynchronize(e->stream));
    double sum[4] = {0, 0, 0, 0};
    for (int k = 0; k < 4; ++k) counts[k] = 0;
    for (const ca_env::Span& sp : e->spans) {
        float ms = 0.0f;
        if (hipEventElapsedTime(&ms, sp.t0, sp.t1) == hipSuccess) { sum[sp.kind] += ms / (sp.steps > 0 ? sp.steps : 1); counts[sp.kind] += 1; }
        e->free_events.push_back(sp.t0);
        e->free_events.push_back(sp.t1);
    }
    e->spans.clear();
    for (int k = 0; k < 4; ++k) mean_ms[k] = counts[k] ? (float)(sum[k] / counts[k]) : 0.0f;
    return CA_OK;
}

int ca_launch_info(ca_env* e, int32_t* block, int32_t* grid, int32_t* lds_bytes, int32_t* obs_grid) {
    if (!e) return CA_EINVAL;
    const SolveLaunch s = solve_launch(e, false, false);
    if (block) *block = (int32_t)s.block.x;
    if (grid) *grid = (int32_t)s.grid.x;
    if (lds_bytes) *lds_bytes = (int32_t)s.lds;
    if (obs_grid) {
        const int apb = obs_block_threads(e->cfg.n_agents) / 16;
        *obs_grid = obs_dense(e) ? (int32_t)(((size_t)e->cfg.n_arenas * e->cfg.n_agents + apb - 1) / apb)
                                 : (int32_t)((size_t)e->cfg.n_arenas * ((e->cfg.n_agents + apb - 1) / apb));
    }
    return CA_OK;
}

#ifndef CA_SRC_SHA
#define CA_SRC_SHA "unknown"
#endif
const char* ca_source_sha(void) { return CA_SRC_SHA; }

int ca_solver_info(ca_env* e, int32_t* lanes_per_agent, int32_t* rollout_one_launch) {
    if (!e) return CA_EINVAL;
    if (lanes_per_agent) *lanes_per_agent = e->quad ? 4 : (e->pair ? 2 : 1);
    if (rollout_one_launch) *rollout_one_launch = e->quad_roll ? 1 : 0;
    return CA_OK;
}

}
```

### collision_avoidance_amd/csrc/ca_obs.h

```cpp
#pragma once
#include "ca_common.h"

namespace ca {

struct ObsArgs {
    const float *pos_x, *pos_y, *vel_x, *vel_y, *orient_x, *orient_y;
    const unsigned short* counts;
    const void* nb_idx;
    const unsigned short* obst_idx;
    const ObstDev* obst;
    const int* tab_off;
    float* obs;
    int A, N, K, S, bpa;
    int nstage_max;
    int paircap;
    int a0;
    int xcd;
    int dense;
    unsigned long long* dbg;
    float radius;
    float rays[32];
    float oct[32];
};

#ifdef CA_STAMPS
#define CA_OSTAMP(k)                                                                       \
    do {                                                                                   \
        __builtin_amdgcn_sched_barrier(0);                                                 \
        const unsigned long long _t = CA_STAMP_CLOCK();                                    \
        __builtin_amdgcn_s_waitcnt(0xC07F);                                                \
        if ((threadIdx.x & 63) == 0 && p.dbg)                                              \
            p.dbg[((size_t)blockIdx.x * (blockDim.x >> 6) + (threadIdx.x >> 6)) * 16 + (k)] = _t; \
        __builtin_amdgcn_sched_barrier(0);                                                 \
    } while (0)
#else
#define CA_OSTAMP(k) do { } while (0)
#endif

__host__ __device__ inline size_t obs_lds_bytes(int nstage_max, int obs_bs, int paircap) {
    const size_t apb = obs_bs / 16;
    return (size_t)nstage_max * 16 + 2 * apb * 16 * 8 + apb * 16 + apb * 16 * 4 + apb * 16 * 4 + 64 * 4 + 2 * apb * 4 + apb * (size_t)paircap * 2;
}
#ifndef CA_OBS_BS_MAX
#define CA_OBS_BS_MAX 256
#endif
__host__ __device__ inline int obs_block_threads(int N) {
    const int want = N > 32 ? 1024 : (N > 16 ? 512 : 256);
    return want < CA_OBS_BS_MAX ? want : CA_OBS_BS_MAX;
}

struct SegGeom {
    float s02x, s02y;
    float s32x, s32y;
    float t_numer;
    float r1x, r1y, r2x, r2y;
};

__device__ __forceinline__ float ray_dial(float x, float y) {
    const float yy = -y;
    const float ax = fabsf(x), ay = fabsf(yy);
    const float mx = fmaxf(ax, ay), mn = fminf(ax, ay);
    const float a = mn * __builtin_amdgcn_rcpf(mx);
    const float s = a * a;
    float r = a * (0.99997726f + s * (-0.33262347f + s * (0.19354346f + s * (-0.11643287f +
              s * (0.05265332f + s * -0.01172120f)))));
    r = (ay > ax) ? 1.57079632679f - r : r;
    r = (x < 0.0f) ? 3.14159265359f - r : r;
    r = (yy < 0.0f) ? -r : r;
    const float u = r * 2.54647908947f;
    return (u < 0.0f) ? u + 16.0f : u;
}

template <int OBS_BS, bool NW16, bool DENSE = false>
__global__ __launch_bounds__(OBS_BS) void obs_kernel(const ObsArgs p) {
    constexpr int OBS_APB = OBS_BS / 16;
    extern __shared__ float4 smem4[];
    const int tid = threadIdx.x;
    const int g = tid >> 4, r = tid & 15;
    const int N = p.N, K = p.K, S = p.S;
    const int PAIRCAP = p.paircap;
    int bid = blockIdx.x;
    if (p.xcd) { const int x = bid & 7, idx = bid >> 3, q8 = idx / p.bpa; bid = (x + 8 * q8) * p.bpa + (idx - q8 * p.bpa); }
    int a, i, a_lo, nstage;
    bool active;
    if constexpr (DENSE) {
        const int first = bid * OBS_APB, gi = first + g;
        active = gi < p.A * N;
        const int ga = active ? gi : p.A * N - 1;
        a = p.a0 + ga / N; i = ga - (ga / N) * N;
        a_lo = p.a0 + first / N;
        const int last = min(first + OBS_APB - 1, p.A * N - 1);
        nstage = (last / N - first / N + 1) * N;
    } else {
        const int ab = bid / p.bpa;
        a = p.a0 + ab;
        i = (bid - ab * p.bpa) * OBS_APB + g;
        active = i < N;
        a_lo = a; nstage = N;
    }
    const int abase = DENSE ? (a - a_lo) * N : 0;
    const size_t q = (size_t)a * N + (active ? i : 0);
    const size_t aoff = (size_t)a * N;
    const unsigned ii = active ? (unsigned)i : 0u;
    const ObstDev* tab = p.obst + (p.tab_off ? p.tab_off[a] : 0);

    const int NST = p.nstage_max;
    float* s_px = reinterpret_cast<float*>(smem4);
    float* s_py = s_px + NST;
    float* s_vx = s_py + NST;
    float* s_vy = s_vx + NST;
    unsigned long long* s_key = reinterpret_cast<unsigned long long*>(s_vy + NST);
    float2* s_rel = reinterpret_cast<float2*>(s_key + OBS_APB * 16);
    float4* s_frame = reinterpret_cast<float4*>(s_rel + OBS_APB * 16);
    int* s_nb = reinterpret_cast<int*>(s_frame + OBS_APB);
    int* s_ob = s_nb + OBS_APB * 16;
    float* s_rays = reinterpret_cast<float*>(s_ob + OBS_APB * 16);
    float* s_oct = s_rays + 32;
    int* s_cnt = reinterpret_cast<int*>(s_oct + 32);
    int* s_cnt2 = s_cnt + OBS_APB;
    unsigned short* s_pair = reinterpret_cast<unsigned short*>(s_cnt2 + OBS_APB);
    const int SPAIRS = 16 * S;
    CA_OSTAMP(0);
    if (tid < 32) { s_rays[tid] = p.rays[tid]; s_oct[tid] = p.oct[tid]; }

    constexpr bool GATHER = NW16;
    const float* gpx = p.pos_x + (size_t)a * N;
    const float* gpy = p.pos_y + (size_t)a * N;
    const float* gvx = p.vel_x + (size_t)a * N;
    const float* gvy = p.vel_y + (size_t)a * N;
    if constexpr (!GATHER) {
        if constexpr (DENSE) {
            for (int t = tid; t < nstage; t += OBS_BS) {
                const size_t qa = (size_t)a_lo * N + t;
                s_px[t] = p.pos_x[qa]; s_py[t] = p.pos_y[qa]; s_vx[t] = p.vel_x[qa]; s_vy[t] = p.vel_y[qa];
            }
        } else {
            for (unsigned t = tid; t < (unsigned)nstage; t += OBS_BS) {
                s_px[t] = (p.pos_x + aoff)[t]; s_py[t] = (p.pos_y + aoff)[t]; s_vx[t] = (p.vel_x + aoff)[t]; s_vy[t] = (p.vel_y + aoff)[t];
            }
        }
    }
    int nn = 0, ns = 0;
    float c = 1.0f, s = 0.0f;
    if (active) {
        if constexpr (DENSE) {
            const int cnts = p.counts[q];
            nn = cnts & 0xFF; ns = cnts >> 8;
            c = p.orient_x[q]; s = -p.orient_y[q];
            if (r < nn) s_nb[g * 16 + r] = abase + ld_idx_t<NW16>(p.nb_idx, ((size_t)a * K + r) * N + i);
            if (r < ns) s_ob[g * 16 + r] = (int)p.obst_idx[((size_t)a * S + r) * N + i];
        } else {
            const int cnts = (p.counts + aoff)[ii];
            nn = cnts & 0xFF; ns = cnts >> 8;
            c = (p.orient_x + aoff)[ii]; s = -(p.orient_y + aoff)[ii];
            const unsigned li = (unsigned)r * (unsigned)N + ii;
            const char* nbase = (const char*)p.nb_idx + aoff * (size_t)K * (NW16 ? 2 : 1);
            if (r < nn) s_nb[g * 16 + r] = ld_idx_t<NW16>(nbase, li);
            if (r < ns) s_ob[g * 16 + r] = (int)(p.obst_idx + aoff * (size_t)S)[li];
        }
    }
    s_key[g * 16 + r] = ~0ull;
    if (r == 0) { s_cnt[g] = 0; s_cnt2[g] = 0; }
    CA_OSTAMP(1);
    __syncthreads();
    CA_OSTAMP(2);

    const int M = 8 * nn + ns;
    float mx = 0.0f, my = 0.0f;
    if (M > 0) { mx = GATHER ? gpx[i] : s_px[abase + i]; my = GATHER ? gpy[i] : s_py[abase + i]; }
    if (r == 0) s_frame[g] = make_float4(c, s, mx, my);
    {
        const int k = r;
        int i0 = 0, w = 0;
        if (k < nn) {
            const int nb = s_nb[g * 16 + k];
            const float rx = (GATHER ? gpx[nb] : s_px[nb]) - mx, ry = (GATHER ? gpy[nb] : s_py[nb]) - my;
            s_rel[g * 16 + k] = make_float2(rx, ry);
            const float d2 = rx * rx + ry * ry, R = p.radius;
            const float ax = c * rx - s * ry, ay = s * rx + c * ry;
            const bool all = !(d2 > 1.0404f * R * R);
            const float ua = ray_dial(ax, ay);
            const float t = R * __builtin_amdgcn_rsqf(d2);
            const float t2 = t * t;
            const float hw = t * (1.0f + t2 * (0.16666667f + t2 * (0.075f + t2 * 0.32914f))) * 2.54647908947f + 0.002f;
            int i1 = (int)floorf(ua + hw);
            i0 = (int)ceilf(ua - hw);
            if (all || i1 - i0 >= 15) { i0 = 0; i1 = 15; }
            w = max(i1 - i0 + 1, 0);
        }
        const int incl = wave_prefix_sum(w);
        int base = 0;
        if ((tid & 63) == 63) base = atomicAdd(&s_cnt[0], incl);
        base = __builtin_amdgcn_readlane(base, 63) + (incl - w);
        const unsigned short hd = (unsigned short)((g << 8) | (k << 4));
#pragma unroll
        for (int t2 = 0; t2 < 4; ++t2)
            if (t2 < w) s_pair[base + t2] = (unsigned short)(hd | ((i0 + t2) & 15));
        if (__builtin_expect(__ballot(w > 4) != 0ull, 0)) {
#pragma clang loop vectorize(disable) unroll(disable)
            for (int t2 = 4; t2 < w; ++t2) s_pair[base + t2] = (unsigned short)(hd | ((i0 + t2) & 15));
        }
    }
    {
        const float dx = s_rays[2 * r], dy = s_rays[2 * r + 1];
        int cnt2 = 0;
        for (int sidx = 0; sidx < ns; ++sidx) {
            const ObstDev o1 = load_obst(tab, s_ob[g * 16 + sidx]);
            const float x1 = o1.px - mx, y1 = o1.py - my, x2 = o1.qx - mx, y2 = o1.qy - my;
            const float ax = c * x1 - s * y1, ay = s * x1 + c * y1;
            const float bx = c * x2 - s * y2, by = s * x2 + c * y2;
            const float c2 = dx * ay - dy * ax, c3 = dx * by - dy * bx;
            const float f2 = dx * ax + dy * ay, f3 = dx * bx + dy * by;
            const float tolE = 1e-5f * p.rays[0] * (fabsf(ax) + fabsf(ay) + fabsf(bx) + fabsf(by) + 1.0f);
            const bool keep = !(c2 > tolE && c3 > tolE) && !(c2 < -tolE && c3 < -tolE) && (fmaxf(f2, f3) >= -tolE);
            const unsigned grp = (unsigned)(__ballot(keep) >> (threadIdx.x & 48)) & 0xFFFFu;
            if (keep)
                s_pair[OBS_APB * PAIRCAP - 1 - (g * SPAIRS + cnt2 + __popc(grp & ((1u << r) - 1u)))] =
                    (unsigned short)(((nn + sidx) << 4) | r);
            cnt2 += __popc(grp);
        }
        if (r == 0) s_cnt2[g] = cnt2;
    }
    CA_OSTAMP(3);
    __syncthreads();
    CA_OSTAMP(4);
    auto build = [&](int m, SegGeom& sg, float& velx, float& vely, bool want_vel) {
        float x1, y1, x2, y2, vx = 0.0f, vy = 0.0f;
        if (m < 8 * nn) {
            const int k = m >> 3, e = m & 7;
            const float2 rel = s_rel[g * 16 + k];
            const float rx = rel.x, ry = rel.y;
            const float4 oc = reinterpret_cast<const float4*>(s_oct)[e];
            x1 = oc.x + rx; y1 = oc.y + ry;
            x2 = oc.z + rx; y2 = oc.w + ry;
            if (want_vel) { const int nb = s_nb[g * 16 + k]; vx = GATHER ? gvx[nb] : s_vx[nb]; vy = GATHER ? gvy[nb] : s_vy[nb]; }
        } else {
            const ObstDev o1 = load_obst(tab, s_ob[g * 16 + (m - 8 * nn)]);
            x1 = o1.px - mx; y1 = o1.py - my;
            x2 = o1.qx - mx; y2 = o1.qy - my;
        }
        sg.r1x = c * x1 - s * y1; sg.r1y = s * x1 + c * y1;
        sg.r2x = c * x2 - s * y2; sg.r2y = s * x2 + c * y2;
        sg.s32x = sg.r2x - sg.r1x; sg.s32y = sg.r2y - sg.r1y;
        sg.s02x = 0.0f - sg.r1x; sg.s02y = 0.0f - sg.r1y;
        sg.t_numer = sg.s32x * sg.s02y - sg.s32y * sg.s02x;
        if (want_vel) {
            const float lvx = x1 + vx, lvy = y1 + vy;
            const float rvx = c * lvx - s * lvy, rvy = s * lvx + c * lvy;
            velx = rvx - sg.r1x; vely = rvy - sg.r1y;
        }
    };
    auto build_nb = [&](const float2& fr, float rx, float ry, int e, SegGeom& sg) {
        const float4 oc = reinterpret_cast<const float4*>(s_oct)[e];
        const float x1 = oc.x + rx, y1 = oc.y + ry, x2 = oc.z + rx, y2 = oc.w + ry;
        sg.r1x = fr.x * x1 - fr.y * y1; sg.r1y = fr.y * x1 + fr.x * y1;
        sg.r2x = fr.x * x2 - fr.y * y2; sg.r2y = fr.y * x2 + fr.x * y2;
        sg.s32x = sg.r2x - sg.r1x; sg.s32y = sg.r2y - sg.r1y;
        sg.s02x = 0.0f - sg.r1x; sg.s02y = 0.0f - sg.r1y;
        sg.t_numer = sg.s32x * sg.s02y - sg.s32y * sg.s02x;
    };
    auto hit = [&](const SegGeom& sg, float s10x, float s10y, float& d, float& hx, float& hy) -> bool {
        const float denom = s10x * sg.s32y - sg.s32x * s10y;
        if (denom == 0.0f) return false;
        const bool dpos = denom > 0.0f;
        const float s_numer = s10x * sg.s02y - s10y * sg.s02x;
        if ((s_numer < 0.0f) == dpos) return false;
        if ((sg.t_numer < 0.0f) == dpos) return false;
        if (((s_numer > denom) == dpos) || ((sg.t_numer > denom) == dpos)) return false;
        const float t = div_ir(sg.t_numer, denom);
        hx = 0.0f + t * s10x; hy = 0.0f + t * s10y;
        d = sqrt_ir(hx * hx + hy * hy);
        return true;
    };

    auto accept_nb = [&](const SegGeom& sg, float s10x, float s10y, float& denom) -> bool {
        denom = s10x * sg.s32y - sg.s32x * s10y;
        const float s_numer = s10x * sg.s02y - s10y * sg.s02x;
        const bool dpos = denom > 0.0f;
        return (denom != 0.0f) && ((s_numer < 0.0f) != dpos) && ((sg.t_numer < 0.0f) != dpos) &&
               ((s_numer > denom) != dpos) && ((sg.t_numer > denom) != dpos);
    };
    auto hit_dist = [&](float t_numer, float denom, float s10x, float s10y) -> float {
        const float t = div_ir(t_numer, denom);
        const float hx = 0.0f + t * s10x, hy = 0.0f + t * s10y;
        return sqrt_ir(hx * hx + hy * hy);
    };

    const float tol = 2e-5f * p.rays[0] * (p.rays[0] + 2.0f * p.radius + 1.0f);
    auto merge = [&](int ga, int ray, float best, int best_m) {
        if (best_m >= 0)
            atomicMin(&s_key[ga * 16 + ray], ((unsigned long long)__float_as_uint(best) << 32) | (unsigned)best_m);
    };
    const int ntot = s_cnt[0];
    for (int pi = tid; pi < ntot; pi += OBS_BS) {
        const int pr = s_pair[pi];
        const int ga = pr >> 8, k = (pr >> 4) & 15, ray = pr & 15;
        const float2 fr = *reinterpret_cast<const float2*>(&s_frame[ga]);
        const float2 rel = s_rel[pr >> 4];
        const float s10x = s_rays[2 * ray] - 0.0f, s10y = s_rays[2 * ray + 1] - 0.0f;
        float best = __int_as_float(0x7f800000);
        int best_m = -1;
        const float rx = rel.x, ry = rel.y;
        const float wx = fr.x * s10x + fr.y * s10y, wy = fr.x * s10y - fr.y * s10x;
        const float wb = wx * ry - wy * rx;
        const float R = p.radius, Rh = 0.70710678f * R;
        const float c0 = R * wy, c2 = R * wx, c1 = Rh * (wx + wy), c3 = Rh * (wy - wx);
        const float cr[8] = {wb - c0, wb - c1, wb - c2, wb + c3, wb + c0, wb + c1, wb + c2, wb - c3};
        unsigned acc = 0;
#pragma unroll
        for (int e = 0; e < 8; ++e) {
            const float ca = cr[e], cb = cr[(e + 1) & 7];
            const bool same_side = (ca > tol && cb > tol) || (ca < -tol && cb < -tol);
            acc |= same_side ? 0u : (1u << e);
        }
        while (acc) {
            const int e1 = __ffs(acc) - 1;
            acc &= acc - 1;
            const bool two = acc != 0;
            const int e2 = two ? __ffs(acc) - 1 : e1;
            acc &= acc - 1;
            SegGeom g1, g2;
            build_nb(fr, rx, ry, e1, g1);
            build_nb(fr, rx, ry, e2, g2);
            float dn1, dn2;
            const bool ok1 = accept_nb(g1, s10x, s10y, dn1), ok2 = accept_nb(g2, s10x, s10y, dn2) && two;
            const float lhs = fabsf(g1.t_numer) * fabsf(dn2), rhs = fabsf(g2.t_numer) * fabsf(dn1);
            const bool first = ok1 && (!ok2 || lhs < rhs);
            const float tnw = first ? g1.t_numer : g2.t_numer, dnw = first ? dn1 : dn2;
            const int ew = first ? e1 : e2;
            const bool sure = fminf(lhs, rhs) < 0.99999f * fmaxf(lhs, rhs) && fmaxf(lhs, rhs) > 1e-30f &&
                              fabsf(tnw) > 1e-12f * fabsf(dnw);
            if (ok1 && ok2 && !sure) {
                const float d1 = hit_dist(g1.t_numer, dn1, s10x, s10y), d2 = hit_dist(g2.t_numer, dn2, s10x, s10y);
                if (d1 < best) { best = d1; best_m = 8 * k + e1; }
                if (d2 < best) { best = d2; best_m = 8 * k + e2; }
            } else {
                const float dw = hit_dist(tnw, dnw, s10x, s10y);
                if ((ok1 || ok2) && dw < best) { best = dw; best_m = 8 * k + ew; }
            }
        }
        merge(ga, ray, best, best_m);
    }
    const int no = s_cnt2[g];
    for (int pi = r; pi < no; pi += 16) {
        const int pr = s_pair[OBS_APB * PAIRCAP - 1 - (g * SPAIRS + pi)];
        const int k = pr >> 4, ray = pr & 15;
        const float s10x = s_rays[2 * ray] - 0.0f, s10y = s_rays[2 * ray + 1] - 0.0f;
        SegGeom sg;
        float dum0, dum1, d, hx, hy;
        const int m = 8 * nn + (k - nn);
        build(m, sg, dum0, dum1, false);
        if (hit(sg, s10x, s10y, d, hx, hy)) merge(g, ray, d, m);
    }
    CA_OSTAMP(5);
    __syncthreads();
    CA_OSTAMP(6);
    if (!active) return;
    const unsigned long long key = s_key[g * 16 + r];
    float bx = 0.0f, by = 0.0f, vx = 0.0f, vy = 0.0f;
    if (key != ~0ull) {
        SegGeom sg;
        float wx, wy;
        build((int)(unsigned)key, sg, wx, wy, true);
        const float s10x = s_rays[2 * r] - 0.0f, s10y = s_rays[2 * r + 1] - 0.0f;
        const float t = div_ir(sg.t_numer, s10x * sg.s32y - sg.s32x * s10y);
        bx = 0.0f + t * s10x; by = 0.0f + t * s10y;
        if (!(bx == 0.0f && by == 0.0f)) { vx = wx; vy = wy; }
    }
    CA_OSTAMP(7);
    {
        typedef float v4f __attribute__((ext_vector_type(4)));
        const v4f out = {bx, by, vx, vy};
        if constexpr (DENSE) __builtin_nontemporal_store(out, reinterpret_cast<v4f*>(p.obs) + (q * 16 + r));
        else __builtin_nontemporal_store(out, (reinterpret_cast<v4f*>(p.obs) + aoff * 16) + (ii * 16u + (unsigned)r));
    }
    CA_OSTAMP(8);
}

}
```

### collision_avoidance_amd/vec_env.py

```python
import ctypes as C

import numpy as np

from . import _lib, scenarios

try:
    import torch
except Exception:
    torch = None

_I32_FIELDS = {_lib.FLD_AGENT_DONE, _lib.FLD_ARRIVE_STEP, _lib.FLD_NB_COUNT, _lib.FLD_NB_IDX,
               _lib.FLD_OBST_COUNT, _lib.FLD_OBST_IDX, _lib.FLD_STEP_COUNT, _lib.FLD_ARENA_DONE,
               _lib.FLD_EPISODE, _lib.FLD_REGOAL_COUNT, _lib.FLD_ALAN_ACTION}
_ARENA_FIELDS = {_lib.FLD_STEP_COUNT, _lib.FLD_ARENA_DONE, _lib.FLD_EPISODE}
_F64_FIELDS = {_lib.FLD_GOAL_X, _lib.FLD_GOAL_Y, _lib.FLD_GOAL2_X, _lib.FLD_GOAL2_Y, _lib.FLD_ALAN_WEIGHTS,
               _lib.FLD_ALAN_TIMES}


def _ptr(a):
    return a.ctypes.data_as(C.c_void_p)


class VecCollisionAvoidanceEnv:

    def __init__(self, n_arenas, n_agents, scenario="crowd", params=None, device=0, seed=0,
                 arena_offset=0, max_obst_neighbors=None, use_torch=None, obstacles="scenario", allow_obst_overflow=False):
        self.L = _lib.load()
        self.A, self.N = int(n_arenas), int(n_agents)
        p = scenarios.env_params()
        if params:
            p.update(params)
        worlds = None
        if obstacles == "scenario":
            worlds = scenarios.obstacle_worlds(scenario, self.A, n_agents, p["radius"], seed, arena_offset) \
                if scenario is not None else None
            polys = scenarios.obstacles(scenario, n_agents, p["radius"]) if scenario is not None and worlds is None else []
        elif isinstance(obstacles, dict) and "per_arena" in obstacles:
            worlds, polys = list(obstacles["per_arena"]), []
        else:
            polys = list(obstacles or [])
        n_edges = max(sum(len(q) for q in w) for w in worlds) if worlds else sum(len(q) for q in polys)
        if max_obst_neighbors is None:
            max_obst_neighbors = max(1, min(_lib.MAX_OBST_NEIGHBORS, n_edges))
        self.cfg = _lib.Config(n_arenas=self.A, n_agents=self.N, arena_offset=arena_offset, seed=seed,
                               max_obst_neighbors=max_obst_neighbors, **p)
        self.K, self.S = self.cfg.max_neighbors, self.cfg.max_obst_neighbors
        self.device = int(device)
        self.use_torch = (torch is not None and torch.cuda.is_available()) if use_torch is None else bool(use_torch)
        h = C.c_void_p()
        rc = self.L.ca_create(C.byref(self.cfg), self.device, None, C.byref(h))
        _lib.check(self.L, None, rc, "ca_create")
        self.h = h
        if allow_obst_overflow:
            self._call("ca_allow_obstacle_overflow", self.h, 1)
        if self.use_torch:
            torch.cuda.set_device(self.device)
            self._call("ca_set_stream", self.h, C.c_void_p(torch.cuda.current_stream(self.device).cuda_stream))
        self._obs_t = None
        self.n_actions = 0
        if self.use_torch:
            dev = torch.device("cuda", self.device)
            self._obs_t = torch.zeros((self.A, self.N, _lib.OBS_DIM), dtype=torch.float32, device=dev)
            self._call("ca_bind_obs", self.h, C.c_void_p(self._obs_t.data_ptr()), self._obs_t.numel() * 4)
            self._rew_t = self.field_tensor(_lib.FLD_REWARD)
            self._done_t = self.field_tensor(_lib.FLD_ARENA_DONE)
            self._act_t = torch.zeros((self.A, self.N), dtype=torch.float32, device=dev)
        if worlds is not None:
            self.set_obstacles_per_arena(worlds)
        else:
            self.set_obstacles(polys)
        if scenario is not None:
            self.init_scenario(scenario)

    def _call(self, name, *args):
        rc = getattr(self.L, name)(*args)
        _lib.check(self.L, self.h, rc, name)

    def close(self):
        self.__dict__.pop("_host_bufs", None); self.__dict__.pop("_packed", None); self.__dict__.pop("_packed_act", None)
        for arr in self.__dict__.pop("_host_arrays", []):
            try:
                arr.flags.writeable = False
            except Exception:
                pass
        if getattr(self, "h", None):
            self.L.ca_destroy(self.h)
            self.h = None

    def __del__(self):
        try:
            self.close()
        except Exception:
            pass

    def _shape_dtype(self, field):
        if field == _lib.FLD_ARENA_STATS:
            return (self.A, 8), np.uint64
        dt = np.int32 if field in _I32_FIELDS else (np.float64 if field in _F64_FIELDS else np.float32)
        if field in _ARENA_FIELDS:
            return (self.A,), dt
        if field == _lib.FLD_NB_IDX:
            return (self.A, max(self.K, 1), self.N), dt
        if field == _lib.FLD_OBST_IDX:
            return (self.A, self.S, self.N), dt
        if field == _lib.FLD_OBS:
            return (self.A, self.N, _lib.OBS_DIM), dt
        if field in (_lib.FLD_ALAN_WEIGHTS, _lib.FLD_ALAN_TIMES):
            return (self.A, self.n_actions, self.N), dt
        return (self.A, self.N), dt

    def get(self, field, out=None):
        shape, dt = self._shape_dtype(field)
        if out is not None and field in (_lib.FLD_ALAN_WEIGHTS, _lib.FLD_ALAN_TIMES):
            raise ValueError("get: out= is not supported for the ALAN weights / times (they are returned transposed, [A, N, n_actions])")
        if out is None:
            out = np.empty(shape, dt)
        elif out.shape != tuple(shape) or out.dtype != np.dtype(dt) or not out.flags["C_CONTIGUOUS"]:
            raise ValueError("get: out must be a C-contiguous %s array of shape %s" % (np.dtype(dt).name, tuple(shape)))
        self._call("ca_get", self.h, field, _ptr(out), out.nbytes, 0)
        if field in (_lib.FLD_ALAN_WEIGHTS, _lib.FLD_ALAN_TIMES):
            return np.ascontiguousarray(np.transpose(out, (0, 2, 1)))
        return out

    def host_array(self, shape, dtype):
        n = int(np.prod(shape)) * np.dtype(dtype).itemsize
        ptr = C.c_void_p()
        self._call("ca_host_alloc", self.h, max(n, 1), C.byref(ptr))
        buf = (C.c_char * max(n, 1)).from_address(ptr.value)
        arr = np.frombuffer(buf, dtype=dtype, count=int(np.prod(shape))).reshape(shape)
        self.__dict__.setdefault("_host_arrays", []).append(arr)
        return arr

    def host_buffer(self, field):
        bufs = self.__dict__.setdefault("_host_bufs", {})
        if field not in bufs:
            shape, dt = self._shape_dtype(field)
            bufs[field] = self.host_array(shape, dt)
        return bufs[field]

    def step_packed(self, actions=None, with_obs=True, stats=False, autoreset=False, no_done=False):
        an, A = self.A * self.N, self.A
        if "_packed" not in self.__dict__:
            words = an * _lib.OBS_DIM + an + 2 * A
            raw = self.host_array((words,), np.float32)
            self._packed = (raw, raw[:an * _lib.OBS_DIM].reshape(A, self.N, _lib.OBS_DIM), raw[an * _lib.OBS_DIM:an * _lib.OBS_DIM + an].reshape(A, self.N),
                            raw[an * _lib.OBS_DIM + an:an * _lib.OBS_DIM + an + A].view(np.int32), raw[an * _lib.OBS_DIM + an + A:].view(np.int32))
            self._packed_act = self.host_array((A, self.N), np.float32)
        raw, obs, rew, done, steps = self._packed
        flags = (_lib.F_OBS if with_obs else 0) | (_lib.F_STATS if stats else 0) | (_lib.F_AUTORESET if autoreset else 0) | \
                (_lib.F_NODONE if no_done else 0)
        act_ptr = None
        if actions is not None:
            if torch is not None and isinstance(actions, torch.Tensor):
                actions = actions.detach().cpu().numpy()
            self._packed_act[...] = np.asarray(actions, np.float32).reshape(A, self.N)
            act_ptr = self._packed_act.ctypes.data
        self._call("ca_step_packed", self.h, act_ptr, flags, raw.ctypes.data, raw.nbytes)
        return obs, rew, done, steps

    def set(self, field, arr):
        shape, dt = self._shape_dtype(field)
        if field in (_lib.FLD_ALAN_WEIGHTS, _lib.FLD_ALAN_TIMES):
            arr = np.transpose(np.asarray(arr, dt).reshape(self.A, self.N, self.n_actions), (0, 2, 1))
        a = np.ascontiguousarray(np.asarray(arr, dt).reshape(shape))
        self._call("ca_set", self.h, field, _ptr(a), a.nbytes, 0)

    _STATE_FIELDS = ("POS_X", "POS_Y", "VEL_X", "VEL_Y", "PREF_X", "PREF_Y", "GOAL_X", "GOAL_Y", "GOAL2_X", "GOAL2_Y",
                     "AGENT_DONE", "ARRIVE_STEP", "NB_COUNT", "NB_IDX", "OBST_COUNT", "OBST_IDX", "STEP_COUNT", "ARENA_DONE",
                     "EPISODE", "REGOAL_COUNT", "REWARD")

    def get_state(self):
        st = {name: self.get(getattr(_lib, "FLD_" + name)) for name in self._STATE_FIELDS}
        if self.n_actions > 0:
            st["ALAN_WEIGHTS"] = self.get(_lib.FLD_ALAN_WEIGHTS)
            st["ALAN_TIMES"] = self.get(_lib.FLD_ALAN_TIMES)
            st["ALAN_ACTION"] = self.get(_lib.FLD_ALAN_ACTION)
        st["_shape"] = np.array([self.A, self.N, self.K, self.S, self.n_actions], np.int64)
        return st

    def set_state(self, st):
        shape = [int(v) for v in np.asarray(st["_shape"]).reshape(-1)]
        if shape != [self.A, self.N, self.K, self.S, self.n_actions]:
            raise ValueError("set_state: the state is of an environment of shape %s, this one is %s"
                             % (shape, [self.A, self.N, self.K, self.S, self.n_actions]))
        optional = ("REWARD", "ALAN_ACTION")
        need = [n for n in self._STATE_FIELDS if n not in optional] + (["ALAN_WEIGHTS", "ALAN_TIMES"] if self.n_actions > 0 else [])
        missing = [n for n in need if n not in st]
        if missing:
            raise KeyError("set_state: the snapshot lacks %s" % ", ".join(missing))
        for name in self._STATE_FIELDS:
            if name in st:
                self.set(getattr(_lib, "FLD_" + name), st[name])
        if self.n_actions > 0:
            self.set(_lib.FLD_ALAN_WEIGHTS, st["ALAN_WEIGHTS"])
            self.set(_lib.FLD_ALAN_TIMES, st["ALAN_TIMES"])
            if "ALAN_ACTION" in st:
                self.set(_lib.FLD_ALAN_ACTION, st["ALAN_ACTION"])

    def field_tensor(self, field):
        if torch is None:
            raise RuntimeError("field_tensor needs PyTorch")
        shape, dt = self._shape_dtype(field)
        ptr, nbytes = C.c_void_p(), C.c_size_t()
        self._call("ca_field_ptr", self.h, field, C.byref(ptr), C.byref(nbytes))

        class _View(object):
            pass
        v = _View()
        v.__cuda_array_interface__ = {"shape": tuple(shape), "typestr": np.dtype(dt).str, "data": (int(ptr.value), False),
                                      "version": 2, "strides": None}
        t = torch.as_tensor(v, device=torch.device("cuda", self.device))
        assert t.numel() * t.element_size() == nbytes.value
        return t

    def neighbor_lists(self):
        return self.get(_lib.FLD_NB_COUNT), np.transpose(self.get(_lib.FLD_NB_IDX), (0, 2, 1))[:, :, :self.K]

    def obstacle_neighbor_lists(self):
        return self.get(_lib.FLD_OBST_COUNT), np.transpose(self.get(_lib.FLD_OBST_IDX), (0, 2, 1))

    def set_obstacles(self, polys):
        polys = [np.asarray(q, np.float32).reshape(-1, 2) for q in polys]
        verts = np.ascontiguousarray(np.concatenate(polys) if polys else np.zeros((0, 2), np.float32))
        sizes = np.asarray([len(q) for q in polys], np.int32)
        self._call("ca_set_obstacles", self.h, _ptr(verts), _ptr(sizes), len(polys))

    def set_obstacles_per_arena(self, worlds):
        if len(worlds) != self.A:
            raise ValueError("set_obstacles_per_arena: %d worlds for %d arenas" % (len(worlds), self.A))
        polys = [np.asarray(q, np.float32).reshape(-1, 2) for w in worlds for q in w]
        verts = np.ascontiguousarray(np.concatenate(polys) if polys else np.zeros((0, 2), np.float32))
        sizes = np.asarray([len(q) for q in polys], np.int32)
        counts = np.asarray([len(w) for w in worlds], np.int32)
        self._call("ca_set_obstacles_per_arena", self.h, _ptr(verts), _ptr(sizes), _ptr(counts))

    def obstacle_table(self, arena=0):
        n = C.c_int32()
        self._call("ca_get_obstacles_arena", self.h, int(arena), None, None, None, 0, C.byref(n))
        verts, nxt, cvx = np.zeros((n.value, 2), np.float32), np.zeros(n.value, np.int32), np.zeros(n.value, np.int32)
        self._call("ca_get_obstacles_arena", self.h, int(arena), _ptr(verts), _ptr(nxt), _ptr(cvx), n.value, C.byref(n))
        return dict(verts=verts, next=nxt, convex=cvx)

    def init_scenario(self, scenario):
        sid = scenarios.SCENARIO_IDS[scenario] if isinstance(scenario, str) else int(scenario)
        self._call("ca_init_scenario", self.h, sid)

    def sync(self):
        self._call("ca_sync", self.h)

    def stats(self):
        s = _lib.Stats()
        self._call("ca_get_stats", self.h, C.byref(s))
        return s.as_dict()

    def reset_stats(self):
        self._call("ca_reset_stats", self.h)

    def profile(self, period=1):
        self._call("ca_profile", self.h, int(period))

    def profile_read(self):
        n = (C.c_int32 * 4)()
        ms = (C.c_float * 4)()
        self._call("ca_profile_read", self.h, n, ms)
        return {k: (n[i], ms[i]) for i, k in enumerate(("nbr_kernel", "step_kernel", "obs_kernel", "reset_kernels"))}

    def launch_info(self):
        v = [C.c_int32() for _ in range(4)]
        self._call("ca_launch_info", self.h, *[C.byref(x) for x in v])
        lanes, roll = C.c_int32(), C.c_int32()
        self._call("ca_solver_info", self.h, C.byref(lanes), C.byref(roll))
        return dict(block=v[0].value, grid=v[1].value, lds_bytes=v[2].value, obs_grid=v[3].value,
                    lanes_per_agent=lanes.value, rollout_one_launch=roll.value)

    def _on_device(self, t, dtype):
        if not t.is_cuda:
            return t.detach().to(dtype=dtype).contiguous().numpy(), False
        dev = torch.device("cuda", self.device)
        t = t.detach().to(device=dev, dtype=dtype).contiguous()
        if not self.use_torch:
            torch.cuda.current_stream(self.device).synchronize()
        return t, True

    def _obs_out(self):
        return self._obs_t if self.use_torch else self.get(_lib.FLD_OBS)

    def reset(self, pos_x=None, pos_y=None, with_obs=True):
        flags = _lib.F_OBS if with_obs else 0
        if pos_x is None:
            self._call("ca_reset", self.h, None, None, 0, flags)
        elif torch is not None and isinstance(pos_x, torch.Tensor) and pos_x.is_cuda and \
                isinstance(pos_y, torch.Tensor) and pos_y.is_cuda:
            px, _ = self._on_device(pos_x, torch.float32)
            py, _ = self._on_device(pos_y, torch.float32)
            if px.numel() != self.A * self.N or py.numel() != self.A * self.N:
                raise ValueError("reset: pos_x / pos_y must hold %d x %d values" % (self.A, self.N))
            self._call("ca_reset", self.h, C.c_void_p(px.data_ptr()), C.c_void_p(py.data_ptr()), 1, flags)
            self.sync()
        else:
            if torch is not None and isinstance(pos_x, torch.Tensor):
                pos_x = pos_x.detach().cpu().numpy()
            if torch is not None and isinstance(pos_y, torch.Tensor):
                pos_y = pos_y.detach().cpu().numpy()
            px = np.ascontiguousarray(np.asarray(pos_x, np.float32).reshape(self.A, self.N))
            py = np.ascontiguousarray(np.asarray(pos_y, np.float32).reshape(self.A, self.N))
            self._call("ca_reset", self.h, _ptr(px), _ptr(py), 0, flags)
        return self._obs_out() if with_obs else None

    def reset_masked(self, mask, with_obs=True):
        flags = _lib.F_OBS if with_obs else 0
        on_dev = False
        if torch is not None and isinstance(mask, torch.Tensor):
            mask, on_dev = self._on_device(mask, torch.int32)
        if on_dev:
            if mask.numel() != self.A:
                raise ValueError("reset_masked: mask must hold %d values" % self.A)
            self._call("ca_reset_masked", self.h, C.c_void_p(mask.data_ptr()), 1, flags)
            self.sync()
        else:
            m = np.ascontiguousarray(np.asarray(mask, np.int32).reshape(self.A))
            self._call("ca_reset_masked", self.h, _ptr(m), 0, flags)
        return self._obs_out() if with_obs else None

    def arena_stats(self):
        r = self.get(_lib.FLD_ARENA_STATS)
        return dict(episodes=r[:, 0], collisions=r[:, 1], obst_collisions=r[:, 2], goals_reached=r[:, 3],
                    obst_overflow=r[:, 4], sum_reward=r[:, 5].copy().view(np.float64), frozen_steps=r[:, 6],
                    last_episode_steps=(r[:, 7] >> np.uint64(32)).astype(np.int64),
                    last_episode_arrived=(r[:, 7] & np.uint64(0xFFFFFFFF)).astype(np.int64))

    def step(self, actions, with_obs=True, stats=False, autoreset=False, copy=True):
        flags = (_lib.F_OBS if with_obs else 0) | (_lib.F_STATS if stats else 0) | \
                (_lib.F_AUTORESET if autoreset else 0)
        if self.use_torch:
            if not isinstance(actions, torch.Tensor):
                actions = torch.as_tensor(np.asarray(actions, np.float32).reshape(self.A, self.N))
            if actions.is_cuda and actions.dtype == torch.float32 and actions.is_contiguous() and \
                    actions.numel() == self.A * self.N and actions.device.index == self.device:
                src = actions
            else:
                self._act_t.copy_(actions.reshape(self.A, self.N), non_blocking=True)
                src = self._act_t
            self._call("ca_step", self.h, C.c_void_p(src.data_ptr()), flags)
            return (self._obs_t if with_obs else None), self._rew_t, self._done_t, {}
        a = np.ascontiguousarray(np.asarray(actions, np.float32).reshape(self.A, self.N))
        self._call("ca_step_host", self.h, _ptr(a), flags)
        if not copy:
            return (self.get(_lib.FLD_OBS, self.host_buffer(_lib.FLD_OBS)) if with_obs else None), \
                self.get(_lib.FLD_REWARD, self.host_buffer(_lib.FLD_REWARD)), \
                self.get(_lib.FLD_ARENA_DONE, self.host_buffer(_lib.FLD_ARENA_DONE)), {}
        return (self.get(_lib.FLD_OBS) if with_obs else None), self.get(_lib.FLD_REWARD), \
            self.get(_lib.FLD_ARENA_DONE), {}

    def orca_step(self, with_obs=False, stats=False, no_done=False, autoreset=False, freeze=False):
        flags = (_lib.F_OBS if with_obs else 0) | (_lib.F_STATS if stats else 0) | \
                (_lib.F_NODONE if no_done else 0) | (_lib.F_AUTORESET if autoreset else 0) | \
                (_lib.F_FREEZE if freeze else 0)
        self._call("ca_orca_step", self.h, flags)
        return self._obs_out() if with_obs else None

    def observe(self):
        self._call("ca_observe", self.h)
        return self._obs_out()

    def rollout(self, steps, with_obs=False, stats=False, autoreset=False, freeze=False):
        flags = (_lib.F_OBS if with_obs else 0) | (_lib.F_STATS if stats else 0) | \
                (_lib.F_AUTORESET if autoreset else 0) | (_lib.F_FREEZE if freeze else 0)
        self._call("ca_rollout", self.h, int(steps), flags)

    def alan_configure(self, actions, temp=0.2, timewindow=2.0, time_step=1 / 60.):
        a = np.ascontiguousarray(np.asarray(actions, np.float64).reshape(-1, 2))
        self._call("ca_alan_configure", self.h, _ptr(a), a.shape[0], float(temp), float(timewindow), float(time_step))
        self.n_actions = a.shape[0]

    def alan_configure_per_arena(self, action_sets, temp=0.2, timewindow=2.0, time_step=1 / 60.):
        if len(action_sets) != self.A:
            raise ValueError("alan_configure_per_arena: %d action sets for %d arenas" % (len(action_sets), self.A))
        sets = [np.asarray(acts, np.float64).reshape(-1, 2) for acts in action_sets]
        n = np.ascontiguousarray([s.shape[0] for s in sets], np.int32)
        xy = np.ascontiguousarray(np.concatenate(sets, 0) if n.sum() else np.zeros((0, 2)), np.float64)
        self._call("ca_alan_configure_per_arena", self.h, _ptr(xy), _ptr(n), float(temp), float(timewindow), float(time_step))
        self.n_actions = int(n.max())

    def alan_actions(self, arena):
        cnt = C.c_int32(0)
        self._call("ca_alan_actions_arena", self.h, int(arena), None, 0, C.byref(cnt))
        out = np.zeros((max(cnt.value, 1), 2), np.float64)
        self._call("ca_alan_actions_arena", self.h, int(arena), _ptr(out), cnt.value, C.byref(cnt))
        return out[:cnt.value]

    def alan_step(self, u=None, with_obs=False, stats=False, freeze=False):
        flags = (_lib.F_OBS if with_obs else 0) | (_lib.F_STATS if stats else 0) | (_lib.F_FREEZE if freeze else 0)
        if u is None:
            self._call("ca_alan_step", self.h, None, 0, flags)
        elif torch is not None and isinstance(u, torch.Tensor) and u.is_cuda:
            ud, _ = self._on_device(u, torch.float64)
            if ud.numel() != self.A * self.N:
                raise ValueError("alan_step: u must hold %d x %d values" % (self.A, self.N))
            self._call("ca_alan_step", self.h, C.c_void_p(ud.data_ptr()), 1, flags)
            self.sync()
        else:
            if torch is not None and isinstance(u, torch.Tensor):
                u = u.detach().numpy()
            uh = np.ascontiguousarray(np.asarray(u, np.float64).reshape(self.A, self.N))
            self._call("ca_alan_step", self.h, _ptr(uh), 0, flags)
        return self._obs_out() if with_obs else None

    def alan_rollout(self, steps, stats=False, freeze=True):
        flags = (_lib.F_STATS if stats else 0) | (_lib.F_FREEZE if freeze else 0)
        self._call("ca_alan_rollout", self.h, int(steps), flags)

    def state(self):
        names = dict(pos_x=_lib.FLD_POS_X, pos_y=_lib.FLD_POS_Y, vel_x=_lib.FLD_VEL_X, vel_y=_lib.FLD_VEL_Y,
                     pref_x=_lib.FLD_PREF_X, pref_y=_lib.FLD_PREF_Y, goal_x=_lib.FLD_GOAL_X,
                     goal_y=_lib.FLD_GOAL_Y, agent_done=_lib.FLD_AGENT_DONE,
                     step_count=_lib.FLD_STEP_COUNT, arena_done=_lib.FLD_ARENA_DONE)
        return {k: self.get(v) for k, v in names.items()}
```

### include/ca_env.h

```cpp
#ifndef CA_ENV_H
#define CA_ENV_H

#include <stddef.h>
#include <stdint.h>

#ifdef __cplusplus
extern "C" {
#endif

#define CA_OBS_DIM 64
#define CA_N_RAYS 16
#define CA_MAX_NEIGHBORS 16
#define CA_MAX_OBST_NEIGHBORS 16
#define CA_MAX_AGENTS 1024

#define CA_OK 0
#define CA_EINVAL (-1)
#define CA_ENODEV (-2)
#define CA_EHIP (-3)
#define CA_ESIZE (-4)
#define CA_ERANGE (-5)

#define CA_DONE_XLESS 0
#define CA_DONE_GOAL 1
#define CA_DONE_REGOAL 2

#define CA_F_OBS 1u
#define CA_F_STATS 2u
#define CA_F_AUTORESET 4u
#define CA_F_NODONE 8u
#define CA_F_FREEZE 16u
#define CA_ALAN_MAX_ACTIONS 32

#define CA_SCN_CROWD 0
#define CA_SCN_CIRCLE 1
#define CA_SCN_DOORWAY 2
#define CA_SCN_CONGESTED 3
#define CA_SCN_INCOMING 4
#define CA_SCN_BLOCKS 5
#define CA_SCN_DEADLOCK 6
#define CA_SCN_CROWD_SEPARATED 7

enum ca_field {
    CA_FLD_POS_X = 0, CA_FLD_POS_Y, CA_FLD_VEL_X, CA_FLD_VEL_Y, CA_FLD_PREF_X, CA_FLD_PREF_Y,
    CA_FLD_GOAL_X, CA_FLD_GOAL_Y, CA_FLD_GOAL2_X, CA_FLD_GOAL2_Y,
    CA_FLD_REWARD,
    CA_FLD_AGENT_DONE,
    CA_FLD_ARRIVE_STEP,
    CA_FLD_NB_COUNT,
    CA_FLD_NB_IDX,
    CA_FLD_OBST_COUNT,
    CA_FLD_OBST_IDX,
    CA_FLD_OBS,
    CA_FLD_STEP_COUNT,
    CA_FLD_ARENA_DONE,
    CA_FLD_EPISODE,
    CA_FLD_REGOAL_COUNT,
    CA_FLD_ALAN_WEIGHTS,
    CA_FLD_ALAN_TIMES,
    CA_FLD_ALAN_ACTION,
    CA_FLD_ARENA_STATS,
    CA_FLD__COUNT
};

#define CA_MIN_LENGTH 1e-3f
#define CA_MAX_LENGTH 1e3f
#define CA_MIN_TIME_STEP 1e-4f
#define CA_MAX_TIME_STEP 10.0f
#define CA_MAX_COORD 1e5f
#define CA_MIN_EDGE 1e-4f

typedef struct ca_config {
    int32_t n_arenas;
    int32_t n_agents;
    int64_t arena_offset;
    uint64_t seed;
    double reward_scale;
    float time_step;
    float neighbor_dist;
    int32_t max_neighbors;
    float time_horizon;
    float time_horizon_obst;
    float radius;
    float max_speed;
    int32_t max_obst_neighbors;
    int32_t max_step;
    int32_t done_mode;
    float done_x_thresh;
    float spawn_x0, spawn_x1, spawn_y0, spawn_y1;
    float goal_x0, goal_x1, goal_y0, goal_y1;
} ca_config;

typedef struct ca_stats {
    uint64_t agent_steps;
    uint64_t episodes;
    uint64_t collisions;
    uint64_t obst_collisions;
    uint64_t goals_reached;
    uint64_t obst_overflow;
    double sum_reward;
} ca_stats;

typedef struct ca_env ca_env;

int ca_create(const ca_config* cfg, int device, void* stream, ca_env** out);
int ca_destroy(ca_env* env);
const char* ca_last_error(const ca_env* env);
int ca_set_stream(ca_env* env, void* stream);

int ca_set_obstacles(ca_env* env, const float* verts_xy, const int32_t* poly_sizes, int32_t n_poly);
int ca_get_obstacles(ca_env* env, float* verts_xy, int32_t* next, int32_t* convex, int32_t cap, int32_t* n_out);
int ca_set_obstacles_per_arena(ca_env* env, const float* verts_xy, const int32_t* poly_sizes, const int32_t* n_poly);
int ca_get_obstacles_arena(ca_env* env, int32_t arena, float* verts_xy, int32_t* next, int32_t* convex, int32_t cap,
                           int32_t* n_out);

int ca_init_scenario(ca_env* env, int32_t scenario);

int ca_set(ca_env* env, int32_t field, const void* src, size_t bytes, int32_t src_is_device);
int ca_get(ca_env* env, int32_t field, void* dst, size_t bytes, int32_t dst_is_device);
int ca_host_alloc(ca_env* env, size_t bytes, void** out);
int ca_host_free(ca_env* env, void* p);
int ca_field_ptr(ca_env* env, int32_t field, void** dev_ptr, size_t* bytes);
int ca_bind_obs(ca_env* env, void* dev_ptr, size_t bytes);

int ca_reset(ca_env* env, const float* pos_x, const float* pos_y, int32_t pos_is_device, uint32_t flags);

int ca_reset_masked(ca_env* env, const int32_t* mask, int32_t mask_is_device, uint32_t flags);

int ca_step(ca_env* env, const float* actions, uint32_t flags);
int ca_step_host(ca_env* env, const float* actions_host, uint32_t flags);
int ca_step_packed(ca_env* env, const float* actions_host, uint32_t flags, void* out_host, size_t out_bytes);
int ca_orca_step(ca_env* env, uint32_t flags);
int ca_observe(ca_env* env);
int ca_rollout(ca_env* env, int32_t steps, uint32_t flags);

int ca_alan_configure(ca_env* env, const double* actions_xy, int32_t n_actions, double temp, double timewindow,
                      double time_step);
int ca_alan_configure_per_arena(ca_env* env, const double* actions_xy, const int32_t* n_actions, double temp,
                                double timewindow, double time_step);
int ca_alan_actions_arena(ca_env* env, int32_t arena, double* cs_xy, int32_t cap, int32_t* n_out);
int ca_alan_step(ca_env* env, const double* u, int32_t u_is_device, uint32_t flags);
int ca_alan_rollout(ca_env* env, int32_t steps, uint32_t flags);

int ca_allow_obstacle_overflow(ca_env* env, int32_t allow);

int ca_get_stats(ca_env* env, ca_stats* out);
int ca_reset_stats(ca_env* env);
int ca_sync(ca_env* env);

int ca_debug_math(ca_env* env, int32_t op, const void* in, void* out, int32_t n);

int ca_profile(ca_env* env, int32_t period);
int ca_profile_read(ca_env* env, int32_t counts[4], float mean_ms[4]);

int ca_launch_info(ca_env* env, int32_t* block, int32_t* grid, int32_t* lds_bytes, int32_t* obs_grid);
int ca_solver_info(ca_env* env, int32_t* lanes_per_agent, int32_t* rollout_one_launch);
const char* ca_source_sha(void);

#ifdef __cplusplus
}
#endif
#endif
```

Before: 2.419 billion.

## Add four-lanes-per-agent observation kernel for mid-size arenas

Adds obs_kernel4, which maps each agent to 4 lanes instead of 16. It uses a compacted work list of (agent, neighbor, ray) pairs stored in LDS and processes them block-wide, with atomicMin merges per ray. The kernel is enabled by default for 17-64 agents without 16-bit neighbor indices. Shared device helpers are factored out of the old kernel, and the old kernel is pinned to 256-thread blocks. The aim is less lane waste and higher occupancy in the observation pass, at the cost of extra synchronisation and LDS atomics.

```diff
diff --git a/collision_avoidance_amd/_lib.py b/collision_avoidance_amd/_lib.py
--- a/collision_avoidance_amd/_lib.py
+++ b/collision_avoidance_amd/_lib.py
@@ -19,7 +19,7 @@
            "ca_get_stats", "ca_reset_stats", "ca_sync", "ca_debug_math", "ca_profile", "ca_profile_read", "ca_launch_info",
            "ca_alan_configure", "ca_alan_step", "ca_alan_rollout", "ca_reset_masked", "ca_get_obstacles",
            "ca_set_obstacles_per_arena", "ca_get_obstacles_arena", "ca_solver_info", "ca_source_sha", "ca_host_alloc", "ca_host_free",
-           "ca_step_packed", "ca_allow_obstacle_overflow", "ca_alan_configure_per_arena", "ca_alan_actions_arena")
+           "ca_step_packed", "ca_allow_obstacle_overflow", "ca_alan_configure_per_arena", "ca_alan_actions_arena", "ca_obs_info")
 
 
 class Config(C.Structure):
@@ -99,6 +99,7 @@
     L.ca_profile_read.argtypes = [vp, C.POINTER(i32), C.POINTER(C.c_float)]
     L.ca_launch_info.argtypes = [vp] + [C.POINTER(i32)] * 4
     L.ca_solver_info.argtypes = [vp, C.POINTER(i32), C.POINTER(i32)]
+    L.ca_obs_info.argtypes = [vp] + [C.POINTER(i32)] * 3
     L.ca_source_sha.argtypes = []
     L.ca_source_sha.restype = C.c_char_p
     for name in EXPORTS:
diff --git a/collision_avoidance_amd/csrc/ca_env.hip b/collision_avoidance_amd/csrc/ca_env.hip
--- a/collision_avoidance_amd/csrc/ca_env.hip
+++ b/collision_avoidance_amd/csrc/ca_env.hip
@@ -66,6 +66,7 @@
     int* d_order = nullptr;
     int P = 1, logP = 0, BS = 64, grid = 1, K = 0, S = 1;
     bool obs_dense_on = false;
+    bool obs_four_on = false;
     bool lists_trusted = true;
     int LS = 1, apb = 1, linv = 65536, dense = 0;
     struct { int reg_lines = -1, pair = -1, alan_fused = -1; } sw;
@@ -307,19 +308,34 @@
 }
 
 typedef void (*obs_fn_t)(const ObsArgs);
-static obs_fn_t obs_fn(int obs_bs, bool w16, bool dense = false) {
+static obs_fn_t obs_fn(bool four, bool w16, bool dense) {
+    if (four) return obs_kernel4;
     if (dense) return obs_kernel<256, false, true>;
-    switch (obs_bs) {
-        case 1024: return w16 ? obs_kernel<1024, true> : obs_kernel<1024, false>;
-        case 512: return w16 ? obs_kernel<512, true> : obs_kernel<512, false>;
-        case 128: return w16 ? obs_kernel<128, true> : obs_kernel<128, false>;
-        case 64: return w16 ? obs_kernel<64, true> : obs_kernel<64, false>;
-        default: return w16 ? obs_kernel<256, true> : obs_kernel<256, false>;
-    }
+    return w16 ? obs_kernel<256, true> : obs_kernel<256, false>;
 }
 
 static bool obs_dense(const ca_env* e) { return e->obs_dense_on; }
 static int obs_nstage(const ca_env* e) { return obs_dense(e) ? 16 + 2 * e->cfg.n_agents : e->cfg.n_agents; }
+
+struct ObsLaunch {
+    obs_fn_t fn;
+    int block, apb, bpa;
+    unsigned grid;
+    size_t lds;
+};
+static bool obs_four(const ca_env* e) { return e->obs_four_on && !e->nidx16; }
+static ObsLaunch obs_launch(const ca_env* e) {
+    const int A = e->cfg.n_arenas, N = e->cfg.n_agents;
+    ObsLaunch o;
+    const bool four = obs_four(e);
+    o.block = four ? OBS4_BS : OBS16_BS;
+    o.apb = o.block / (four ? 4 : 16);
+    o.bpa = (N + o.apb - 1) / o.apb;
+    o.fn = obs_fn(four, e->nidx16 != 0, obs_dense(e));
+    o.grid = obs_dense(e) ? (unsigned)(((size_t)A * N + o.apb - 1) / o.apb) : (unsigned)((size_t)A * o.bpa);
+    o.lds = four ? obs4_lds_bytes(N, e->S) : obs_lds_bytes(obs_nstage(e), o.block, 16 * (e->K + e->S));
+    return o;
+}
 
 static hipError_t launch_obs(ca_env* e) {
     if (!e->orient_valid) {
@@ -338,8 +354,8 @@
     o.obs = e->obs;
     o.A = e->cfg.n_arenas; o.N = e->cfg.n_agents; o.S = e->S;
     o.K = e->K > 0 ? e->K : 1;
-    const int obs_bs = obs_block_threads(o.N), apb = obs_bs / 16;
-    o.bpa = (o.N + apb - 1) / apb;
+    const ObsLaunch L = obs_launch(e);
+    o.bpa = L.bpa;
     o.paircap = 16 * (e->K + e->S);
     o.a0 = 0; o.dbg = e->dbg_obs;
     o.dense = obs_dense(e) ? 1 : 0;
@@ -348,10 +364,8 @@
     o.radius = e->cfg.radius;
     memcpy(o.rays, e->rays, sizeof o.rays);
     memcpy(o.oct, e->oct, sizeof o.oct);
-    const dim3 grid(o.dense ? (unsigned)(((size_t)o.A * o.N + apb - 1) / apb) : (unsigned)((size_t)o.A * o.bpa)), block(obs_bs);
-    const size_t lds = obs_lds_bytes(o.nstage_max, obs_bs, o.paircap);
     ProfScope ps(e, KIND_OBS);
-    launch_k(ps, obs_fn(obs_bs, e->nidx16 != 0, o.dense != 0), grid, block, lds, e->stream, o);
+    launch_k(ps, L.fn, dim3(L.grid), dim3(L.block), L.lds, e->stream, o);
     return hipGetLastError();
 }
 
@@ -553,6 +567,8 @@
     {
         const char* v = getenv("CA_OBS_DENSE");
         e->obs_dense_on = cfg->n_agents < 16 && !(v && v[0] == '0');
+        const char* f = getenv("CA_OBS_FOUR");
+        e->obs_four_on = cfg->n_agents >= 17 && cfg->n_agents <= 64 && !(f && f[0] == '0');
     }
     {
         const char* v = getenv("CA_DENSE");
@@ -624,12 +640,9 @@
     bool lds_misfit = false;
     if (r == hipSuccess) r = apply_variant_attributes(e, &lds_misfit);
     if (r == hipSuccess) {
-        const int obs_bs = obs_block_threads(cfg->n_agents);
-        const size_t ol = obs_lds_bytes(obs_nstage(e), obs_bs, 16 * (e->K + e->S));
-        if (ol > 48 * 1024) {
-            r = hipFuncSetAttribute(reinterpret_cast<const void*>(obs_fn(obs_bs, e->nidx16 != 0, obs_dense(e))),
-                                    hipFuncAttributeMaxDynamicSharedMemorySize, (int)ol);
-        }
+        const ObsLaunch L = obs_launch(e);
+        if (L.lds > 48 * 1024)
+            r = hipFuncSetAttribute(reinterpret_cast<const void*>(L.fn), hipFuncAttributeMaxDynamicSharedMemorySize, (int)L.lds);
     }
     if (r == hipSuccess) {
         r = hipHostMalloc((void**)&e->ovf_host, sizeof(unsigned long long), hipHostMallocDefault);
@@ -1667,11 +1680,16 @@
     if (block) *block = (int32_t)s.block.x;
     if (grid) *grid = (int32_t)s.grid.x;
     if (lds_bytes) *lds_bytes = (int32_t)s.lds;
-    if (obs_grid) {
-        const int apb = obs_block_threads(e->cfg.n_agents) / 16;
-        *obs_grid = obs_dense(e) ? (int32_t)(((size_t)e->cfg.n_arenas * e->cfg.n_agents + apb - 1) / apb)
-                                 : (int32_t)((size_t)e->cfg.n_arenas * ((e->cfg.n_agents + apb - 1) / apb));
-    }
+    if (obs_grid) *obs_grid = (int32_t)obs_launch(e).grid;
+    return CA_OK;
+}
+
+int ca_obs_info(ca_env* e, int32_t* lanes_per_agent, int32_t* block, int32_t* lds_bytes) {
+    if (!e) return CA_EINVAL;
+    const ObsLaunch L = obs_launch(e);
+    if (lanes_per_agent) *lanes_per_agent = obs_four(e) ? 4 : 16;
+    if (block) *block = (int32_t)L.block;
+    if (lds_bytes) *lds_bytes = (int32_t)L.lds;
     return CA_OK;
 }
 
diff --git a/collision_avoidance_amd/csrc/ca_obs.h b/collision_avoidance_amd/csrc/ca_obs.h
--- a/collision_avoidance_amd/csrc/ca_obs.h
+++ b/collision_avoidance_amd/csrc/ca_obs.h
@@ -41,13 +41,7 @@
     const size_t apb = obs_bs / 16;
     return (size_t)nstage_max * 16 + 2 * apb * 16 * 8 + apb * 16 + apb * 16 * 4 + apb * 16 * 4 + 64 * 4 + 2 * apb * 4 + apb * (size_t)paircap * 2;
 }
-#ifndef CA_OBS_BS_MAX
-#define CA_OBS_BS_MAX 256
-#endif
-__host__ __device__ inline int obs_block_threads(int N) {
-    const int want = N > 32 ? 1024 : (N > 16 ? 512 : 256);
-    return want < CA_OBS_BS_MAX ? want : CA_OBS_BS_MAX;
-}
+constexpr int OBS16_BS = 256;
 
 struct SegGeom {
     float s02x, s02y;
@@ -69,6 +63,120 @@
     r = (yy < 0.0f) ? -r : r;
     const float u = r * 2.54647908947f;
     return (u < 0.0f) ? u + 16.0f : u;
+}
+
+
+__device__ __forceinline__ void obs_nb_window(float c, float s, float rx, float ry, float R, int& i0, int& w) {
+    const float d2 = rx * rx + ry * ry;
+    const float ax = c * rx - s * ry, ay = s * rx + c * ry;
+    const bool all = !(d2 > 1.0404f * R * R);
+    const float ua = ray_dial(ax, ay);
+    const float t = R * __builtin_amdgcn_rsqf(d2);
+    const float t2 = t * t;
+    const float hw = t * (1.0f + t2 * (0.16666667f + t2 * (0.075f + t2 * 0.32914f))) * 2.54647908947f + 0.002f;
+    int i1 = (int)floorf(ua + hw);
+    i0 = (int)ceilf(ua - hw);
+    if (all || i1 - i0 >= 15) { i0 = 0; i1 = 15; }
+    w = max(i1 - i0 + 1, 0);
+}
+
+__device__ __forceinline__ void obs_seg(float c, float s, float x1, float y1, float x2, float y2, SegGeom& sg) {
+    sg.r1x = c * x1 - s * y1; sg.r1y = s * x1 + c * y1;
+    sg.r2x = c * x2 - s * y2; sg.r2y = s * x2 + c * y2;
+    sg.s32x = sg.r2x - sg.r1x; sg.s32y = sg.r2y - sg.r1y;
+    sg.s02x = 0.0f - sg.r1x; sg.s02y = 0.0f - sg.r1y;
+    sg.t_numer = sg.s32x * sg.s02y - sg.s32y * sg.s02x;
+}
+__device__ __forceinline__ void obs_seg_vel(float c, float s, float x1, float y1, float vx, float vy, const SegGeom& sg, float& velx, float& vely) {
+    const float lvx = x1 + vx, lvy = y1 + vy;
+    const float rvx = c * lvx - s * lvy, rvy = s * lvx + c * lvy;
+    velx = rvx - sg.r1x; vely = rvy - sg.r1y;
+}
+__device__ __forceinline__ void obs_build_nb(const float* s_oct, const float2& fr, float rx, float ry, int e, SegGeom& sg) {
+    const float4 oc = reinterpret_cast<const float4*>(s_oct)[e];
+    obs_seg(fr.x, fr.y, oc.x + rx, oc.y + ry, oc.z + rx, oc.w + ry, sg);
+}
+__device__ __forceinline__ bool obs_hit(const SegGeom& sg, float s10x, float s10y, float& d, float& hx, float& hy) {
+    const float denom = s10x * sg.s32y - sg.s32x * s10y;
+    if (denom == 0.0f) return false;
+    const bool dpos = denom > 0.0f;
+    const float s_numer = s10x * sg.s02y - s10y * sg.s02x;
+    if ((s_numer < 0.0f) == dpos) return false;
+    if ((sg.t_numer < 0.0f) == dpos) return false;
+    if (((s_numer > denom) == dpos) || ((sg.t_numer > denom) == dpos)) return false;
+    const float t = div_ir(sg.t_numer, denom);
+    hx = 0.0f + t * s10x; hy = 0.0f + t * s10y;
+    d = sqrt_ir(hx * hx + hy * hy);
+    return true;
+}
+__device__ __forceinline__ bool obs_accept_nb(const SegGeom& sg, float s10x, float s10y, float& denom) {
+    denom = s10x * sg.s32y - sg.s32x * s10y;
+    const float s_numer = s10x * sg.s02y - s10y * sg.s02x;
+    const bool dpos = denom > 0.0f;
+    return (denom != 0.0f) && ((s_numer < 0.0f) != dpos) && ((sg.t_numer < 0.0f) != dpos) &&
+           ((s_numer > denom) != dpos) && ((sg.t_numer > denom) != dpos);
+}
+__device__ __forceinline__ float obs_hit_dist(float t_numer, float denom, float s10x, float s10y) {
+    const float t = div_ir(t_numer, denom);
+    const float hx = 0.0f + t * s10x, hy = 0.0f + t * s10y;
+    return sqrt_ir(hx * hx + hy * hy);
+}
+__device__ __forceinline__ void obs_merge(unsigned long long* s_key, int ga, int ray, float best, int best_m) {
+    if (best_m >= 0)
+        atomicMin(&s_key[ga * 16 + ray], ((unsigned long long)__float_as_uint(best) << 32) | (unsigned)best_m);
+}
+__device__ __forceinline__ float obs_chord_tol(float neighbor_dist, float radius) {
+    return 2e-5f * neighbor_dist * (neighbor_dist + 2.0f * radius + 1.0f);
+}
+
+__device__ __forceinline__ void obs_nb_pair(const float* s_oct, const float2& fr, float rx, float ry, float s10x, float s10y,
+                                            float R, float tol, int k, float& best, int& best_m) {
+    best = __int_as_float(0x7f800000);
+    best_m = -1;
+    const float wx = fr.x * s10x + fr.y * s10y, wy = fr.x * s10y - fr.y * s10x;
+    const float wb = wx * ry - wy * rx;
+    const float Rh = 0.70710678f * R;
+    const float c0 = R * wy, c2 = R * wx, c1 = Rh * (wx + wy), c3 = Rh * (wy - wx);
+    const float cr[8] = {wb - c0, wb - c1, wb - c2, wb + c3, wb + c0, wb + c1, wb + c2, wb - c3};
+    unsigned acc = 0;
+#pragma unroll
+    for (int e = 0; e < 8; ++e) {
+        const float ca = cr[e], cb = cr[(e + 1) & 7];
+        const bool same_side = (ca > tol && cb > tol) || (ca < -tol && cb < -tol);
+        acc |= same_side ? 0u : (1u << e);
+    }
+    while (acc) {
+        const int e1 = __ffs(acc) - 1;
+        acc &= acc - 1;
+        const bool two = acc != 0;
+        const int e2 = two ? __ffs(acc) - 1 : e1;
+        acc &= acc - 1;
+        SegGeom g1, g2;
+        obs_build_nb(s_oct, fr, rx, ry, e1, g1);
+        obs_build_nb(s_oct, fr, rx, ry, e2, g2);
+        float dn1, dn2;
+        const bool ok1 = obs_accept_nb(g1, s10x, s10y, dn1), ok2 = obs_accept_nb(g2, s10x, s10y, dn2) && two;
+        const float lhs = fabsf(g1.t_numer) * fabsf(dn2), rhs = fabsf(g2.t_numer) * fabsf(dn1);
+        const bool first = ok1 && (!ok2 || lhs < rhs);
+        const float tnw = first ? g1.t_numer : g2.t_numer, dnw = first ? dn1 : dn2;
+        const int ew = first ? e1 : e2;
+        const bool sure = fminf(lhs, rhs) < 0.99999f * fmaxf(lhs, rhs) && fmaxf(lhs, rhs) > 1e-30f &&
+                          fabsf(tnw) > 1e-12f * fabsf(dnw);
+        if (ok1 && ok2 && !sure) {
+            const float d1 = obs_hit_dist(g1.t_numer, dn1, s10x, s10y), d2 = obs_hit_dist(g2.t_numer, dn2, s10x, s10y);
+            if (d1 < best) { best = d1; best_m = 8 * k + e1; }
+            if (d2 < best) { best = d2; best_m = 8 * k + e2; }
+        } else {
+            const float dw = obs_hit_dist(tnw, dnw, s10x, s10y);
+            if ((ok1 || ok2) && dw < best) { best = dw; best_m = 8 * k + ew; }
+        }
+    }
+}
+__device__ __forceinline__ void obs_winner(const SegGeom& sg, float s10x, float s10y, float wx, float wy, float& bx, float& by, float& vx, float& vy) {
+    const float t = div_ir(sg.t_numer, s10x * sg.s32y - sg.s32x * s10y);
+    bx = 0.0f + t * s10x; by = 0.0f + t * s10y;
+    vx = 0.0f; vy = 0.0f;
+    if (!(bx == 0.0f && by == 0.0f)) { vx = wx; vy = wy; }
 }
 
 template <int OBS_BS, bool NW16, bool DENSE = false>
@@ -176,17 +284,7 @@
             const int nb = s_nb[g * 16 + k];
             const float rx = (GATHER ? gpx[nb] : s_px[nb]) - mx, ry = (GATHER ? gpy[nb] : s_py[nb]) - my;
             s_rel[g * 16 + k] = make_float2(rx, ry);
-            const float d2 = rx * rx + ry * ry, R = p.radius;
-            const float ax = c * rx - s * ry, ay = s * rx + c * ry;
-            const bool all = !(d2 > 1.0404f * R * R);
-            const float ua = ray_dial(ax, ay);
-            const float t = R * __builtin_amdgcn_rsqf(d2);
-            const float t2 = t * t;
-            const float hw = t * (1.0f + t2 * (0.16666667f + t2 * (0.075f + t2 * 0.32914f))) * 2.54647908947f + 0.002f;
-            int i1 = (int)floorf(ua + hw);
-            i0 = (int)ceilf(ua - hw);
-            if (all || i1 - i0 >= 15) { i0 = 0; i1 = 15; }
-            w = max(i1 - i0 + 1, 0);
+            obs_nb_window(c, s, rx, ry, p.radius, i0, w);
         }
         const int incl = wave_prefix_sum(w);
         int base = 0;
@@ -239,58 +337,11 @@
             x1 = o1.px - mx; y1 = o1.py - my;
             x2 = o1.qx - mx; y2 = o1.qy - my;
         }
-        sg.r1x = c * x1 - s * y1; sg.r1y = s * x1 + c * y1;
-        sg.r2x = c * x2 - s * y2; sg.r2y = s * x2 + c * y2;
-        sg.s32x = sg.r2x - sg.r1x; sg.s32y = sg.r2y - sg.r1y;
-        sg.s02x = 0.0f - sg.r1x; sg.s02y = 0.0f - sg.r1y;
-        sg.t_numer = sg.s32x * sg.s02y - sg.s32y * sg.s02x;
-        if (want_vel) {
-            const float lvx = x1 + vx, lvy = y1 + vy;
-            const float rvx = c * lvx - s * lvy, rvy = s * lvx + c * lvy;
-            velx = rvx - sg.r1x; vely = rvy - sg.r1y;
-        }
+        obs_seg(c, s, x1, y1, x2, y2, sg);
+        if (want_vel) obs_seg_vel(c, s, x1, y1, vx, vy, sg, velx, vely);
     };
-    auto build_nb = [&](const float2& fr, float rx, float ry, int e, SegGeom& sg) {
-        const float4 oc = reinterpret_cast<const float4*>(s_oct)[e];
-        const float x1 = oc.x + rx, y1 = oc.y + ry, x2 = oc.z + rx, y2 = oc.w + ry;
-        sg.r1x = fr.x * x1 - fr.y * y1; sg.r1y = fr.y * x1 + fr.x * y1;
-        sg.r2x = fr.x * x2 - fr.y * y2; sg.r2y = fr.y * x2 + fr.x * y2;
-        sg.s32x = sg.r2x - sg.r1x; sg.s32y = sg.r2y - sg.r1y;
-        sg.s02x = 0.0f - sg.r1x; sg.s02y = 0.0f - sg.r1y;
-        sg.t_numer = sg.s32x * sg.s02y - sg.s32y * sg.s02x;
-    };
-    auto hit = [&](const SegGeom& sg, float s10x, float s10y, float& d, float& hx, float& hy) -> bool {
-        const float denom = s10x * sg.s32y - sg.s32x * s10y;
-        if (denom == 0.0f) return false;
-        const bool dpos = denom > 0.0f;
-        const float s_numer = s10x * sg.s02y - s10y * sg.s02x;
-        if ((s_numer < 0.0f) == dpos) return false;
-        if ((sg.t_numer < 0.0f) == dpos) return false;
-        if (((s_numer > denom) == dpos) || ((sg.t_numer > denom) == dpos)) return false;
-        const float t = div_ir(sg.t_numer, denom);
-        hx = 0.0f + t * s10x; hy = 0.0f + t * s10y;
-        d = sqrt_ir(hx * hx + hy * hy);
-        return true;
-    };
-
-    auto accept_nb = [&](const SegGeom& sg, float s10x, float s10y, float& denom) -> bool {
-        denom = s10x * sg.s32y - sg.s32x * s10y;
-        const float s_numer = s10x * sg.s02y - s10y * sg.s02x;
-        const bool dpos = denom > 0.0f;
-        return (denom != 0.0f) && ((s_numer < 0.0f) != dpos) && ((sg.t_numer < 0.0f) != dpos) &&
-               ((s_numer > denom) != dpos) && ((sg.t_numer > denom) != dpos);
-    };
-    auto hit_dist = [&](float t_numer, float denom, float s10x, float s10y) -> float {
-        const float t = div_ir(t_numer, denom);
-        const float hx = 0.0f + t * s10x, hy = 0.0f + t * s10y;
-        return sqrt_ir(hx * hx + hy * hy);
-    };
-
-    const float tol = 2e-5f * p.rays[0] * (p.rays[0] + 2.0f * p.radius + 1.0f);
-    auto merge = [&](int ga, int ray, float best, int best_m) {
-        if (best_m >= 0)
-            atomicMin(&s_key[ga * 16 + ray], ((unsigned long long)__float_as_uint(best) << 32) | (unsigned)best_m);
-    };
+
+    const float tol = obs_chord_tol(p.rays[0], p.radius);
     const int ntot = s_cnt[0];
     for (int pi = tid; pi < ntot; pi += OBS_BS) {
         const int pr = s_pair[pi];
@@ -298,48 +349,10 @@
         const float2 fr = *reinterpret_cast<const float2*>(&s_frame[ga]);
         const float2 rel = s_rel[pr >> 4];
         const float s10x = s_rays[2 * ray] - 0.0f, s10y = s_rays[2 * ray + 1] - 0.0f;
-        float best = __int_as_float(0x7f800000);
-        int best_m = -1;
-        const float rx = rel.x, ry = rel.y;
-        const float wx = fr.x * s10x + fr.y * s10y, wy = fr.x * s10y - fr.y * s10x;
-        const float wb = wx * ry - wy * rx;
-        const float R = p.radius, Rh = 0.70710678f * R;
-        const float c0 = R * wy, c2 = R * wx, c1 = Rh * (wx + wy), c3 = Rh * (wy - wx);
-        const float cr[8] = {wb - c0, wb - c1, wb - c2, wb + c3, wb + c0, wb + c1, wb + c2, wb - c3};
-        unsigned acc = 0;
-#pragma unroll
-        for (int e = 0; e < 8; ++e) {
-            const float ca = cr[e], cb = cr[(e + 1) & 7];
-            const bool same_side = (ca > tol && cb > tol) || (ca < -tol && cb < -tol);
-            acc |= same_side ? 0u : (1u << e);
-        }
-        while (acc) {
-            const int e1 = __ffs(acc) - 1;
-            acc &= acc - 1;
-            const bool two = acc != 0;
-            const int e2 = two ? __ffs(acc) - 1 : e1;
-            acc &= acc - 1;
-            SegGeom g1, g2;
-            build_nb(fr, rx, ry, e1, g1);
-            build_nb(fr, rx, ry, e2, g2);
-            float dn1, dn2;
-            const bool ok1 = accept_nb(g1, s10x, s10y, dn1), ok2 = accept_nb(g2, s10x, s10y, dn2) && two;
-            const float lhs = fabsf(g1.t_numer) * fabsf(dn2), rhs = fabsf(g2.t_numer) * fabsf(dn1);
-            const bool first = ok1 && (!ok2 || lhs < rhs);
-            const float tnw = first ? g1.t_numer : g2.t_numer, dnw = first ? dn1 : dn2;
-            const int ew = first ? e1 : e2;
-            const bool sure = fminf(lhs, rhs) < 0.99999f * fmaxf(lhs, rhs) && fmaxf(lhs, rhs) > 1e-30f &&
-                              fabsf(tnw) > 1e-12f * fabsf(dnw);
-            if (ok1 && ok2 && !sure) {
-                const float d1 = hit_dist(g1.t_numer, dn1, s10x, s10y), d2 = hit_dist(g2.t_numer, dn2, s10x, s10y);
-                if (d1 < best) { best = d1; best_m = 8 * k + e1; }
-                if (d2 < best) { best = d2; best_m = 8 * k + e2; }
-            } else {
-                const float dw = hit_dist(tnw, dnw, s10x, s10y);
-                if ((ok1 || ok2) && dw < best) { best = dw; best_m = 8 * k + ew; }
-            }
-        }
-        merge(ga, ray, best, best_m);
+        float best;
+        int best_m;
+        obs_nb_pair(s_oct, fr, rel.x, rel.y, s10x, s10y, p.radius, tol, k, best, best_m);
+        obs_merge(s_key, ga, ray, best, best_m);
     }
     const int no = s_cnt2[g];
     for (int pi = r; pi < no; pi += 16) {
@@ -350,7 +363,7 @@
         float dum0, dum1, d, hx, hy;
         const int m = 8 * nn + (k - nn);
         build(m, sg, dum0, dum1, false);
-        if (hit(sg, s10x, s10y, d, hx, hy)) merge(g, ray, d, m);
+        if (obs_hit(sg, s10x, s10y, d, hx, hy)) obs_merge(s_key, g, ray, d, m);
     }
     CA_OSTAMP(5);
     __syncthreads();
@@ -363,9 +376,7 @@
         float wx, wy;
         build((int)(unsigned)key, sg, wx, wy, true);
         const float s10x = s_rays[2 * r] - 0.0f, s10y = s_rays[2 * r + 1] - 0.0f;
-        const float t = div_ir(sg.t_numer, s10x * sg.s32y - sg.s32x * s10y);
-        bx = 0.0f + t * s10x; by = 0.0f + t * s10y;
-        if (!(bx == 0.0f && by == 0.0f)) { vx = wx; vy = wy; }
+        obs_winner(sg, s10x, s10y, wx, wy, bx, by, vx, vy);
     }
     CA_OSTAMP(7);
     {
@@ -377,4 +388,173 @@
     CA_OSTAMP(8);
 }
 
-}
+constexpr int OBS4_BS = 64;
+constexpr int OBS4_TRIPS = 6;
+__host__ __device__ inline size_t obs4_lds_bytes(int n_agents, int S) {
+    const size_t apb = OBS4_BS / 4;
+    return (size_t)n_agents * 16 + apb * 16 * 8 + apb * 16 + 64 * 4 + (size_t)OBS4_TRIPS * OBS4_BS * 2 + apb * (size_t)S * 2 + apb * 16;
+}
+
+__global__ __launch_bounds__(OBS4_BS) __attribute__((amdgpu_waves_per_eu(8))) void obs_kernel4(const ObsArgs p) {
+    constexpr int OBS_BS = OBS4_BS;
+    constexpr int APB = OBS_BS / 4;
+    constexpr int CAP = OBS4_TRIPS * OBS_BS;
+    extern __shared__ float4 smem4[];
+    const int tid = threadIdx.x;
+    const int g = tid >> 2, l = tid & 3;
+    const int N = p.N, K = p.K, S = p.S;
+    int bid = blockIdx.x;
+    if (p.xcd) { const int x = bid & 7, idx = bid >> 3, q8 = idx / p.bpa; bid = (x + 8 * q8) * p.bpa + (idx - q8 * p.bpa); }
+    const int ab = bid / p.bpa;
+    const int a = p.a0 + ab;
+    const int i = (bid - ab * p.bpa) * APB + g;
+    const bool active = i < N;
+    const size_t aoff = (size_t)a * N;
+    const unsigned ii = active ? (unsigned)i : 0u;
+    const ObstDev* tab = p.obst + (p.tab_off ? p.tab_off[a] : 0);
+
+    float2* s_pos = reinterpret_cast<float2*>(smem4);
+    float2* s_vel = s_pos + N;
+    unsigned long long* s_key = reinterpret_cast<unsigned long long*>(s_vel + N);
+    float4* s_frame = reinterpret_cast<float4*>(s_key + APB * 16);
+    float* s_rays = reinterpret_cast<float*>(s_frame + APB);
+    float* s_oct = s_rays + 32;
+    unsigned short* s_pair = reinterpret_cast<unsigned short*>(s_oct + 32);
+    unsigned short* s_ob = s_pair + CAP;
+    unsigned char* s_nb = reinterpret_cast<unsigned char*>(s_ob + APB * S);
+    CA_OSTAMP(0);
+    if (tid < 32) { s_rays[tid] = p.rays[tid]; s_oct[tid] = p.oct[tid]; }
+    for (unsigned t = tid; t < (unsigned)N; t += OBS_BS) {
+        s_pos[t] = make_float2((p.pos_x + aoff)[t], (p.pos_y + aoff)[t]);
+        s_vel[t] = make_float2((p.vel_x + aoff)[t], (p.vel_y + aoff)[t]);
+    }
+    int nn = 0, ns = 0;
+    float c = 1.0f, s = 0.0f, mx = 0.0f, my = 0.0f;
+    if (active) {
+        const int cnts = (p.counts + aoff)[ii];
+        nn = cnts & 0xFF; ns = cnts >> 8;
+        c = (p.orient_x + aoff)[ii]; s = -(p.orient_y + aoff)[ii];
+        mx = (p.pos_x + aoff)[ii]; my = (p.pos_y + aoff)[ii];
+        const unsigned char* nbase = (const unsigned char*)p.nb_idx + aoff * (size_t)K;
+#pragma unroll
+        for (int t = 0; t < 4; ++t) {
+            const int k = l + 4 * t;
+            if (k < nn) s_nb[g * 16 + k] = (unsigned char)ld_idx_t<false>(nbase, (unsigned)k * (unsigned)N + ii);
+        }
+        for (int k = l; k < ns; k += 4) s_ob[g * S + k] = (p.obst_idx + aoff * (size_t)S)[(unsigned)k * (unsigned)N + ii];
+        if (l == 0) s_frame[g] = make_float4(c, s, mx, my);
+    }
+    {
+        uint4* kk = reinterpret_cast<uint4*>(s_key) + 2 * tid;
+        kk[0] = make_uint4(~0u, ~0u, ~0u, ~0u); kk[1] = make_uint4(~0u, ~0u, ~0u, ~0u);
+    }
+    CA_OSTAMP(1);
+    __syncthreads();
+    CA_OSTAMP(2);
+
+    int win[4];
+#pragma unroll
+    for (int t = 0; t < 4; ++t) {
+        const int k = l + 4 * t;
+        win[t] = 0;
+        if (k < nn) {
+            const float2 pn = s_pos[s_nb[g * 16 + k]];
+            int i0, w;
+            obs_nb_window(c, s, pn.x - mx, pn.y - my, p.radius, i0, w);
+            win[t] = (i0 & 15) | (w << 4);
+        }
+    }
+    for (int sidx = 0; sidx < ns; ++sidx) {
+        const ObstDev o1 = load_obst(tab, s_ob[g * S + sidx]);
+        SegGeom sg;
+        obs_seg(c, s, o1.px - mx, o1.py - my, o1.qx - mx, o1.qy - my, sg);
+#pragma unroll
+        for (int t = 0; t < 4; ++t) {
+            const int ray = l + 4 * t;
+            const float s10x = s_rays[2 * ray] - 0.0f, s10y = s_rays[2 * ray + 1] - 0.0f;
+            float d, hx, hy;
+            if (obs_hit(sg, s10x, s10y, d, hx, hy)) obs_merge(s_key, g, ray, d, 8 * nn + sidx);
+        }
+    }
+    const float tol = obs_chord_tol(p.rays[0], p.radius);
+    int wl = (win[0] >> 4) + (win[1] >> 4) + (win[2] >> 4) + (win[3] >> 4);
+    for (;;) {
+        const int incl = wave_prefix_sum(wl);
+        const bool fits = incl <= CAP;
+        const int ntot = __builtin_amdgcn_readlane(incl, __popcll(__ballot(fits)) - 1);
+        if (fits) {
+            int at = incl - wl;
+#pragma unroll
+            for (int t = 0; t < 4; ++t) {
+                const int w = win[t] >> 4, i0 = win[t] & 15;
+                const unsigned short hd = (unsigned short)((g << 8) | ((l + 4 * t) << 4));
+#pragma unroll
+                for (int t2 = 0; t2 < 4; ++t2)
+                    if (t2 < w) s_pair[at + t2] = (unsigned short)(hd | ((i0 + t2) & 15));
+                if (__builtin_expect(__ballot(w > 4) != 0ull, 0)) {
+#pragma clang loop vectorize(disable) unroll(disable)
+                    for (int t2 = 4; t2 < w; ++t2) s_pair[at + t2] = (unsigned short)(hd | ((i0 + t2) & 15));
+                }
+                at += w;
+                win[t] = 0;
+            }
+            wl = 0;
+        }
+        CA_OSTAMP(3);
+        __syncthreads();
+        CA_OSTAMP(4);
+        const bool more = __ballot(wl > 0) != 0ull;
+        for (int pi = tid; pi < ntot; pi += OBS_BS) {
+            const int pr = s_pair[pi];
+            const int ga = pr >> 8, k = (pr >> 4) & 15, ray = pr & 15;
+            const float4 fr4 = s_frame[ga];
+            const float2 fr = make_float2(fr4.x, fr4.y);
+            const float2 pn = s_pos[s_nb[pr >> 4]];
+            const float s10x = s_rays[2 * ray] - 0.0f, s10y = s_rays[2 * ray + 1] - 0.0f;
+            float best;
+            int best_m;
+            obs_nb_pair(s_oct, fr, pn.x - fr4.z, pn.y - fr4.w, s10x, s10y, p.radius, tol, k, best, best_m);
+            obs_merge(s_key, ga, ray, best, best_m);
+        }
+        if (__builtin_expect(!more, 1)) break;
+        __syncthreads();
+    }
+    CA_OSTAMP(5);
+    __syncthreads();
+    CA_OSTAMP(6);
+    if (!active) return;
+    typedef float v4f __attribute__((ext_vector_type(4)));
+    v4f* row = (reinterpret_cast<v4f*>(p.obs) + aoff * 16) + ii * 16u;
+#pragma unroll
+    for (int t = 0; t < 4; ++t) {
+        const int ray = l + 4 * t;
+        const unsigned long long key = s_key[g * 16 + ray];
+        float bx = 0.0f, by = 0.0f, vx = 0.0f, vy = 0.0f;
+        if (key != ~0ull) {
+            const int m = (int)(unsigned)key;
+            float x1, y1, x2, y2, nvx = 0.0f, nvy = 0.0f;
+            if (m < 8 * nn) {
+                const int nb = s_nb[g * 16 + (m >> 3)];
+                const float2 pn = s_pos[nb], vn = s_vel[nb];
+                const float4 oc = reinterpret_cast<const float4*>(s_oct)[m & 7];
+                const float rx = pn.x - mx, ry = pn.y - my;
+                x1 = oc.x + rx; y1 = oc.y + ry; x2 = oc.z + rx; y2 = oc.w + ry;
+                nvx = vn.x; nvy = vn.y;
+            } else {
+                const ObstDev o1 = load_obst(tab, s_ob[g * S + (m - 8 * nn)]);
+                x1 = o1.px - mx; y1 = o1.py - my; x2 = o1.qx - mx; y2 = o1.qy - my;
+            }
+            SegGeom sg;
+            float wx, wy;
+            obs_seg(c, s, x1, y1, x2, y2, sg);
+            obs_seg_vel(c, s, x1, y1, nvx, nvy, sg, wx, wy);
+            obs_winner(sg, s_rays[2 * ray] - 0.0f, s_rays[2 * ray + 1] - 0.0f, wx, wy, bx, by, vx, vy);
+        }
+        const v4f out = {bx, by, vx, vy};
+        __builtin_nontemporal_store(out, row + ray);
+    }
+    CA_OSTAMP(7);
+    CA_OSTAMP(8);
+}
+
+}
diff --git a/collision_avoidance_amd/vec_env.py b/collision_avoidance_amd/vec_env.py
--- a/collision_avoidance_amd/vec_env.py
+++ b/collision_avoidance_amd/vec_env.py
@@ -270,8 +270,11 @@
         self._call("ca_launch_info", self.h, *[C.byref(x) for x in v])
         lanes, roll = C.c_int32(), C.c_int32()
         self._call("ca_solver_info", self.h, C.byref(lanes), C.byref(roll))
+        ob = [C.c_int32() for _ in range(3)]
+        self._call("ca_obs_info", self.h, *[C.byref(x) for x in ob])
         return dict(block=v[0].value, grid=v[1].value, lds_bytes=v[2].value, obs_grid=v[3].value,
-                    lanes_per_agent=lanes.value, rollout_one_launch=roll.value)
+                    lanes_per_agent=lanes.value, rollout_one_launch=roll.value,
+                    obs_lanes_per_agent=ob[0].value, obs_block=ob[1].value, obs_lds_bytes=ob[2].value)
 
     def _on_device(self, t, dtype):
         if not t.is_cuda:
diff --git a/include/ca_env.h b/include/ca_env.h
--- a/include/ca_env.h
+++ b/include/ca_env.h
@@ -155,6 +155,7 @@
 
 int ca_launch_info(ca_env* env, int32_t* block, int32_t* grid, int32_t* lds_bytes, int32_t* obs_grid);
 int ca_solver_info(ca_env* env, int32_t* lanes_per_agent, int32_t* rollout_one_launch);
+int ca_obs_info(ca_env* env, int32_t* lanes_per_agent, int32_t* block, int32_t* lds_bytes);
 const char* ca_source_sha(void);
 
 #ifdef __cplusplus
```

Result: faster. 2.751 billion, median of 6 (+13.8%).
